# EI-CoreBioinformatics/portcullis

Measured on AMD Instinct MI355X. Metric: junc_reads_per_sec, higher is better.
Workload: dtype int32; 1 GPU; BASELINE configs[2]: synthetic 199999998 paired-end 150-bp reads, 25 contigs of GRCh38 lengths (3088286401 bp), 249999 junctions, orientation FR; reads_total=199999998, junctions_total=249999, contigs=25, reads_rank0=199999998, pairs_rank0=66692850

## Files before the change

### portcullis_amd/csrc/pjb_api.hip

```cpp
#include "pjb_host.hip.h"
#include "pjb_kernels.hip.h"

static int slot_init(pjb_ctx *c, int k);
static void aux_streams(pjb_ctx *c) {
    if (!c->stream3) (void)hipStreamCreateWithFlags(&c->stream3, hipStreamNonBlocking);
    if (!c->stream4) (void)hipStreamCreateWithFlags(&c->stream4, hipStreamNonBlocking);
}

extern "C" {

namespace {
std::mutex g_host_mu;
std::map<void *, size_t> g_host_registered;
}
void *pjb_host_alloc(size_t bytes) {
    if (bytes >= ((size_t)8 << 20)) {
        const size_t huge = (size_t)2 << 20, len = (bytes + huge - 1) & ~(huge - 1);
        void *p = mmap(nullptr, len, PROT_READ | PROT_WRITE, MAP_PRIVATE | MAP_ANONYMOUS, -1, 0);
        if (p != MAP_FAILED) {
            (void)madvise(p, len, MADV_HUGEPAGE);
            const size_t nt = std::min<size_t>(4, len >> 24);
            auto touch = [&](size_t t) {
                const size_t per = ((len / std::max<size_t>(nt, 1)) + huge - 1) & ~(huge - 1), a = std::min(len, per * t), b = std::min(len, a + per);
                for (size_t o = a; o < b; o += 4096) ((volatile uint8_t *)p)[o] = 0;
// ... 489 lines not shown
    c->mirror_acc[0] += (int64_t)R.spliced;
    c->mirror_acc[1] += (int64_t)R.unspliced;
    c->mirror_acc[2] += (int64_t)R.sum_len;
    c->mirror_acc[3] = std::min<int64_t>(c->mirror_acc[3], R.min_len);
    c->mirror_acc[4] = std::max<int64_t>(c->mirror_acc[4], R.max_len);
    int64_t *h = c->mirror_hdr;
    h[0] = (int64_t)c->mirror_rows;
    for (int k = 0; k < 5; k++) h[1 + k] = c->mirror_acc[k];
    h[6] = h[7] = 0;
}
static void mirror_reset(pjb_ctx *c) {
    c->mirror_rows = 0;
    c->mirror_acc[0] = c->mirror_acc[1] = c->mirror_acc[2] = 0;
    c->mirror_acc[3] = INT32_MAX;
    c->mirror_acc[4] = 0;
}
static int mirror_header_only(pjb_ctx *c, const pjb_region_result &R) {
    if (!c->mirror) return PJB_OK;
    aux_streams(c);
    mirror_fold(c, R, 0);
    HIP_TRY(c, hipMemcpyAsync(c->mirror, c->mirror_hdr, PJB_MIRROR_HEADER_BYTES, hipMemcpyHostToDevice, c->stream4));
    HIP_TRY(c, hipStreamSynchronize(c->stream4));
    return PJB_OK;
}

static void wait_flight(pjb_ctx *c, Flight &f);


static int rows_pinned_reserve(pjb_ctx *c, size_t need) {
    if (need <= c->rows_pinned_cap && c->rows_pinned) return PJB_OK;
    int rc = rows_sync(c);
    if (rc) return rc;
    const size_t ncap = std::max<size_t>(need * 3 / 2, 1024);
    pjb_junction_row *np = nullptr;
    const hipError_t e = hipHostMalloc((void **)&np, ncap * sizeof(pjb_junction_row), hipHostMallocPortable);
    if (e != hipSuccess) return fail(c, PJB_ERR_NOMEM, "hipHostMalloc(rows): %s", hipGetErrorString(e));
    if (c->rows_pinned && c->rows_n) memcpy(np, c->rows_pinned, std::min(c->rows_n, c->rows_pinned_cap) * sizeof(pjb_junction_row));
    if (c->rows_pinned) (void)hipHostFree(c->rows_pinned);
    c->rows_pinned = np;
    c->rows_pinned_cap = ncap;
    return PJB_OK;
}

static size_t rows_upper_bound(const pjb_ctx *c) {
    size_t n = c->rows_n;
    for (int k = 0; k < c->n_fl; k++)
        if (c->fl[k].queued) n += c->fl[k].lim.junc_limit;
    return n;
}

constexpr unsigned K6_BLOCKS = 128;
static int queue_contig(pjb_ctx *c, Flight &f) {
    std::vector<DevBatch> &batches = f.batches;
    CtlSlot &S = c->sl[f.slot];
    const hipStream_t service = c->stream, st = c->side_stream ? S.main : c->stream;
    struct ChainScope {
        pjb_ctx *c;
        hipStream_t service;
        ~ChainScope() {
            c->stream = service;
            c->scan_tiles = &c->b_scan_tiles;
        }
    } chain_scope{c, service};
    c->stream = st;
    c->scan_tiles = &S.scan_tiles;
    const u32 n_tiles = f.n_tiles;
    const ContigLimits &lim = f.lim;
    const int n_members = (int)f.tids.size();
    const bool group = n_members > 1;
    const int32_t ref_len = group ? (int32_t)f.vlen : c->ref_len[(size_t)f.tid];
    GroupTab GT;
    memset(&GT, 0, sizeof GT);
    GT.n = n_members;
    bool all_codes = true, any_x = false;
    for (int m = 0; m < n_members; m++) {
        const Contig &g = c->contigs[(size_t)f.tids[(size_t)m]];
        GT.voff[m] = f.voff[(size_t)m];
        GT.len[m] = (int32_t)g.len;
        GT.tid[m] = f.tids[(size_t)m];
        GT.d[m] = g.d;
        GT.codes[m] = g.codes;
        GT.codes2[m] = g.codes2;
        if (g.any_exc) GT.exc_members |= 1u << m;
        all_codes = all_codes && g.codes != nullptr;
        any_x = any_x || g.has_x;
    }
    const KeyFmt kf = lim.kf;
    const u32 PL = lim.pair_limit, JL = lim.junc_limit;
    const u32 SL = lim.sort_limit && lim.sort_limit < JL ? lim.sort_limit : JL;
    int rc;
    bool ahead = false;
    for (int k = 0; k < c->n_fl; k++) ahead |= c->fl[k].queued && &c->fl[k] != &f;
    const int64_t row_base = ahead ? -1 : (int64_t)c->rows_n, mirror_base = ahead ? -1 : (int64_t)c->mirror_rows;
    struct PoolScope {
        pjb_ctx *c;
        ~PoolScope() { c->cur_pool = MISC_POOL; }
    } pool_scope{c};
    c->cur_pool = f.slot;
    c->cur_slot = f.slot;
    ev_drop(c, f.slot);
    if ((rc = ensure(c, S.batches, batches.size() * sizeof(DevBatch)))) return rc;
    if (batches.size() + 2 > S.batches_pinned_cap) {
        if (S.batches_pinned) (void)hipHostFree(S.batches_pinned);
        S.batches_pinned = nullptr;
        S.batches_pinned_cap = 0;
        const size_t cap = std::max<size_t>(batches.size() * 2 + 2, 16);
        HIP_TRY(c, hipHostMalloc((void **)&S.batches_pinned, cap * sizeof(DevBatch), hipHostMallocDefault));
        S.batches_pinned_cap = cap;
    }
    memcpy(S.batches_pinned, batches.data(), batches.size() * sizeof(DevBatch));
    if ((rc = ensure(c, S.cstats, sizeof(ContigStats)))) return rc;
    if (!S.scan_parts.p) {
        if ((rc = ensure(c, S.scan_parts, sizeof(ScanPart) * K1S_BLOCKS))) return rc;
        HIP_TRY(c, hipMemset(S.scan_parts.p, 0, sizeof(ScanPart) * K1S_BLOCKS));
        HIP_TRY(c, hipStreamSynchronize(nullptr));
    }
    if ((rc = ensure(c, S.err, 8))) return rc;
    if (!c->b_cursor.p) {
        if ((rc = ensure(c, c->b_cursor, sizeof(RowCursor)))) return rc;
        HIP_TRY(c, hipMemset(c->b_cursor.p, 0, sizeof(RowCursor)));
        HIP_TRY(c, hipStreamSynchronize(nullptr));
    }
    if ((rc = ensure(c, S.tile_cnt, (size_t)n_tiles * 4))) return rc;
    if ((rc = ensure(c, S.tile_stats, (size_t)n_tiles * sizeof(TileStats)))) return rc;
    if ((rc = ensure(c, S.tile_soff, ((size_t)n_tiles + 1) * 4))) return rc;
    if ((rc = ensure(c, S.chunk_tile, ((size_t)n_tiles * (K1_TILE / 256) + 4) * 4))) return rc;
    if ((rc = ensure(c, S.splidx, (size_t)n_tiles * K1_TILE * 4))) return rc;
    if ((rc = ensure(c, S.splpoff, (size_t)n_tiles * K1_TILE * 4))) return rc;
    if ((rc = ensure(c, S.splrec, (size_t)n_tiles * K1_TILE * 16))) return rc;
    if (!S.members.p) {
        if ((rc = ensure(c, S.members, GROUP_MAX * sizeof(MemberStats) + GROUP_MAX * 4 + (GROUP_MAX + 1) * 4))) return rc;
        HIP_TRY(c, hipMemset(S.members.p, 0, S.members.cap));
        HIP_TRY(c, hipStreamSynchronize(nullptr));
    }
    MemberStats *d_members = (MemberStats *)S.members.p;
    u32 *d_member_junc = (u32 *)(d_members + GROUP_MAX);
    u32 *d_tile_lo = d_member_junc + GROUP_MAX;
    if ((rc = ensure(c, S.total, 8))) return rc;
    if ((rc = ensure(c, S.okey, ((size_t)PL + RS_TILE) * 8))) return rc;
    if ((rc = ensure(c, S.key[0], ((size_t)PL + RS_TILE) * 8))) return rc;
    if ((rc = ensure(c, S.key[1], ((size_t)PL + RS_TILE) * 8))) return rc;
    if ((rc = ensure(c, S.idx[0], ((size_t)PL + RS_TILE) * 4))) return rc;
    if ((rc = ensure(c, S.idx[1], ((size_t)PL + RS_TILE) * 4))) return rc;
    if ((rc = ensure(c, S.rec, ((size_t)PL + 1) * sizeof(PairRec)))) return rc;
    if ((rc = ensure(c, S.jid, (size_t)PL * 4 + 16))) return rc;
    if ((rc = ensure(c, S.jidbam, ((size_t)PL + RS_TILE) * 4))) return rc;
    if (c->extra && (rc = ensure(c, S.g, (size_t)PL * 4 + 16))) return rc;
    if ((rc = ensure(c, S.seg, ((size_t)PL + 1) * 4))) return rc;
    if ((rc = ensure(c, S.runfirst, ((size_t)PL + 1) * 4))) return rc;
    if ((rc = ensure(c, S.runstart, ((size_t)PL + 1) * 4))) return rc;
    if ((rc = ensure(c, S.ent, (size_t)PL * 8 + 16))) return rc;
    const u32 pair_blocks = std::max<u32>(1, (PL + 255) / 256);
    const u32 gen_cap = lim.list_cap ? lim.list_cap : (c->list_cap_forced ? c->list_cap_forced : gen_list_cap(PL));
    const u32 pack_nn = (u64)f.n_reads < (1ull << 28) ? 1u : 0u;
    if ((rc = ensure(c, S.genlist, (size_t)gen_cap * GEN_SHARDS * 8 * 3))) return rc;
    if ((rc = ensure(c, S.gencount, GEN_SHARDS * GEN_CNT_STRIDE * 4))) return rc;
    const u32 slots_lim = JL + (PL + 63) / 64 + 1;
    if ((rc = ensure(c, S.frag, (size_t)slots_lim * F_WORDS * 4))) return rc;
    if ((rc = ensure(c, S.fragj, (size_t)slots_lim * 4))) return rc;
    if ((rc = ensure(c, S.acc, (size_t)JL * F_WORDS * 4 + 16))) return rc;
    if ((rc = ensure(c, S.ancl, (size_t)JL * 4 + 16))) return rc;
    if ((rc = ensure(c, S.ancr, (size_t)JL * 4 + 16))) return rc;
    if ((rc = ensure(c, S.jkey, (size_t)JL * 8 + 16))) return rc;
    if ((rc = ensure(c, S.rows, (size_t)JL * sizeof(pjb_junction_row) + 16))) return rc;
    size_t old = rows_upper_bound(c);
    if (old + JL > c->rows_cap) {
        for (int k = 0; k < c->n_fl; k++)
            if (c->fl[k].queued && &c->fl[k] != &f) wait_flight(c, c->fl[k]);
        if ((rc = rows_sync(c))) return rc;
        old = std::min(old, c->rows_cap);
        const size_t ncap = std::max<size_t>((old + JL) * 3 / 2, 1024);
        pjb_junction_row *nd = nullptr;
        hipError_t e = hipMalloc((void **)&nd, ncap * sizeof(pjb_junction_row));
        if (e != hipSuccess) return fail(c, PJB_ERR_NOMEM, "hipMalloc(row table): %s", hipGetErrorString(e));
        if (old) {
            HIP_TRY(c, hipMemcpyAsync(nd, c->rows_table, old * sizeof(pjb_junction_row), hipMemcpyDeviceToDevice, c->stream4));
            HIP_TRY(c, hipStreamSynchronize(c->stream4));
        }
        if (c->rows_table) bury(c, c->rows_table);
        c->rows_table = nd;
        c->rows_cap = ncap;
    }
    if (!S.pub) {
        HIP_TRY(c, hipHostMalloc((void **)&S.pub, PUB_BYTES, hipHostMallocMapped | hipHostMallocPortable));
        void *dp = nullptr;
        if (hipHostGetDevicePointer(&dp, S.pub, 0) != hipSuccess || !dp) return fail(c, PJB_ERR_HIP, "hipHostGetDevicePointer(control block) failed");
        S.pub_dev = (uint8_t *)dp;
    }

    const hipStream_t front = st;
    {
        bool on_service = false;
        for (int32_t t : f.tids) {
            auto oit = c->open.find(t);
            on_service = on_service || (oit != c->open.end() && oit->second.on_main_stream);
        }
        if (st != service && on_service) {
            HIP_TRY(c, hipEventRecord(c->ev_front, service));
            HIP_TRY(c, hipStreamWaitEvent(st, c->ev_front, 0));
        }
    }
    HIP_TRY(c, hipMemcpyAsync(S.batches.p, S.batches_pinned, batches.size() * sizeof(DevBatch), hipMemcpyHostToDevice, front));
    if (group) {
        u32 *h_lo = (u32 *)(S.batches_pinned + batches.size());
        for (int m = 0; m <= n_members; m++) h_lo[m] = f.tile_lo[(size_t)m];
        HIP_TRY(c, hipMemcpyAsync(d_tile_lo, h_lo, (size_t)(n_members + 1) * 4, hipMemcpyHostToDevice, front));
    }
    if (!S.at_rest) {
        HIP_TRY(c, hipMemsetAsync(S.err.p, 0xff, 8, front));
        HIP_TRY(c, hipMemsetAsync(S.gencount.p, 0, GEN_SHARDS * GEN_CNT_STRIDE * 4, front));
        HIP_TRY(c, hipMemsetAsync(d_member_junc, 0, GROUP_MAX * 4, front));
    }
    S.at_rest = false;
    u64 *d_err = (u64 *)S.err.p;
    ContigStats *d_cs = (ContigStats *)S.cstats.p;
    const u32 *d_P = &d_cs->P, *d_J = &d_cs->J, *d_slots = &d_cs->n_slots;
    const bool stage_events = c->ktime && c->ktime_only.empty();
#define STAGE_EVENT(k)                                            \
    do {                                                          \
        if (stage_events) HIP_TRY(c, hipEventRecord(S.ev[k], st));  \
    } while (0)
    HIP_TRY(c, hipEventRecord(S.ev[0], front));
    const size_t n_words = ((size_t)std::max(ref_len, 1) + 63) / 64;
    if (lim.dense) {
        const void *was[2] = {S.bitmap.p, S.ends.p};
        if ((rc = ensure(c, S.bitmap, n_words * 8 + 16))) return rc;
        if ((rc = ensure(c, S.wrank, n_words * 4 + 16))) return rc;
        const void *was_pc = S.pagecnt.p;
        if ((rc = ensure(c, S.pagecnt, ((n_words >> KD_PAGE_SHIFT) + 1) * 4 + 16))) return rc;
        if ((rc = ensure(c, S.pagerank, ((n_words >> KD_PAGE_SHIFT) + 1) * 4 + 16))) return rc;
        if ((rc = ensure(c, S.ends, (size_t)JL * DENSE_ENDS * 4 + 32))) return rc;
        if ((rc = ensure(c, S.firstid, (size_t)JL * 4 + 16))) return rc;
        if (!S.dense_at_rest || was[0] != S.bitmap.p || was[1] != S.ends.p || was_pc != S.pagecnt.p) {
            HIP_TRY(c, hipMemsetAsync(S.bitmap.p, 0, S.bitmap.cap, front));
            HIP_TRY(c, hipMemsetAsync(S.pagecnt.p, 0, S.pagecnt.cap, front));
            HIP_TRY(c, hipMemsetAsync(S.ends.p, 0xff, S.ends.cap, front));
        }
        S.dense_at_rest = false;
    }
    Pairs pr;
    pr.key = (u64 *)S.okey.p;
    pr.rec = (PairRec *)S.rec.p;
    pr.g = c->extra ? (u32 *)S.g.p : (u32 *)nullptr;
    f.pr = pr;
    u32 *d_gen_cnt = (u32 *)S.gencount.p;
    const bool fast_codes = all_codes && !any_x;
    {
        const bool xk1 = c->extra && !c->extra_dense_only && !group && !f.x_k1 && !f.x_pre;
        XOut xo = {nullptr, nullptr, nullptr, nullptr, 0, nullptr};
        if (xk1) {
            const size_t N = (size_t)f.n_reads;
            if ((rc = ensure(c, S.x_q, N + 16)) || (rc = ensure(c, S.x_spos, N * 4 + 16)) || (rc = ensure(c, S.x_send, N * 4 + 16)) ||
                (rc = ensure(c, S.x_zlist, (size_t)X_ZCAP * 4)) || (rc = ensure(c, S.x_scnt, X_SCNT_BYTES)))
                return rc;
            HIP_TRY(c, hipMemsetAsync((uint8_t *)S.x_q.p + N, 0, 1, c->stream));
            HIP_TRY(c, hipMemsetAsync(S.x_scnt.p, 0, sizeof(SparseCounters) + sizeof(ExtraCounters), c->stream));
            xo = XOut{(int32_t *)S.x_spos.p, (int32_t *)S.x_send.p, (uint8_t *)S.x_q.p, (u32 *)S.x_zlist.p, X_ZCAP, (SparseCounters *)S.x_scnt.p};
        }
        if (c->k1_serial && c->last_k1_ev) HIP_TRY(c, hipStreamWaitEvent(st, c->last_k1_ev, 0));
        if (xk1)
            LAUNCH(c, "k1_count", k1_count<true>, dim3(n_tiles), dim3(K1C_T), (const DevBatch *)S.batches.p, (int)batches.size(), (u32 *)S.tile_cnt.p, (TileStats *)S.tile_stats.p,
                   (u32 *)S.splidx.p, (u32 *)S.splpoff.p, (uint4 *)S.splrec.p, d_err, GT, 0, xo);
        else
            LAUNCH(c, "k1_count", k1_count<false>, dim3(n_tiles), dim3(K1C_T), (const DevBatch *)S.batches.p, (int)batches.size(), (u32 *)S.tile_cnt.p, (TileStats *)S.tile_stats.p,
                   (u32 *)S.splidx.p, (u32 *)S.splpoff.p, (uint4 *)S.splrec.p, d_err, GT, group ? 1 : 0, xo);
        if (xk1) {
            HIP_TRY(c, hipEventRecord(S.ev_xk1, c->stream));
            f.x_k1 = true;
        }
        LAUNCH(c, "k1_scan_tiles", k1_scan_tiles, dim3(c->k1s_blocks_forced ? (u32)c->k1s_blocks_forced : k1s_blocks(n_tiles)), dim3(K1S_THREADS), (u32 *)S.tile_cnt.p, (const TileStats *)S.tile_stats.p,
               n_tiles, d_cs, PL, kf, group ? INT32_MAX - 1 : ref_len, (const u64 *)nullptr, (u32 *)S.tile_soff.p, (u32 *)S.chunk_tile.p,
               (ScanPart *)S.scan_parts.p, ++S.scan_epoch);
        EmitLists el;
        el.cand = lim.dense ? (u64 *)S.key[1].p : (u64 *)nullptr;
        el.bitmap = lim.dense ? (u64 *)S.bitmap.p : (u64 *)nullptr;
        el.page_cnt = lim.dense ? (u32 *)S.pagecnt.p : (u32 *)nullptr;
        el.cand_anc = (u64 *)S.ent.p;
        el.gen_list = (u64 *)S.genlist.p;
        el.gen_cnt = d_gen_cnt;
        el.gen_cap = gen_cap;
        el.pack_nn = pack_nn;
        for (size_t b0 = 0; b0 < batches.size(); b0 += K1E_MAXB) {
            const size_t nb = std::min<size_t>(K1E_MAXB, batches.size() - b0);
            u64 reads = 0;
            for (size_t bi = b0; bi < b0 + nb; bi++) reads += (u64)batches[bi].n;
            const u32 nt = (u32)std::min<u64>((reads + K1_TILE - 1) / K1_TILE + nb, 0x7fffffffu);
            static const u32 tiles_per_block = getenv("PJB_K1E_TILES") ? (u32)std::max(1, atoi(getenv("PJB_K1E_TILES"))) : 8u;
            const u32 grid = std::max<u32>(1, std::min<u32>(nt, std::max<u32>(1024, nt / tiles_per_block)));
            LAUNCH(c, "k1_emit", k1_emit, dim3(grid), dim3(256), (const DevBatch *)S.batches.p + b0, (int)nb, n_tiles, (const u32 *)S.tile_cnt.p,
                   (const u32 *)S.tile_soff.p, (const u32 *)S.chunk_tile.p, (const u32 *)S.splidx.p, (const u32 *)S.splpoff.p, (const uint4 *)S.splrec.p, pr, el, kf,
                   GT, fast_codes ? 1 : 0, (int)c->cfg.orientation, d_err, d_cs);
        }
        if (c->k1_serial && !getenv("PJB_K1_SERIAL_LATE")) {
            HIP_TRY(c, hipEventRecord(S.ev_k1, st));
            c->last_k1_ev = S.ev_k1;
        }
        if (group)
            LAUNCH(c, "kg_member_stats", kg_member_stats, dim3((unsigned)n_members), dim3(256), (const u32 *)S.tile_cnt.p, (const TileStats *)S.tile_stats.p,
                   (const u32 *)d_tile_lo, n_members, d_members, n_tiles, (const ContigStats *)d_cs);
        LAUNCH(c, "k1_generic", k1_generic, dim3(std::min<u32>(std::max<u32>(1, (u32)(((u64)gen_cap * GEN_SHARDS + K1E_T - 1) / K1E_T)), 1536u )), dim3(K1E_T),
               (const DevBatch *)S.batches.p, (int)batches.size(), (const u32 *)S.splidx.p, (const uint4 *)S.splrec.p, pr, el, kf, GT, fast_codes ? 1 : 0,
               (int)c->cfg.orientation, d_err, d_cs);
    }
    if (c->k1_serial && getenv("PJB_K1_SERIAL_LATE")) {
        HIP_TRY(c, hipEventRecord(S.ev_k1, st));
        c->last_k1_ev = S.ev_k1;
    }
    STAGE_EVENT(1);
    const u32 gen_grid = std::min<u32>(2 * (u32)(((u64)gen_cap * GEN_SHARDS + 255) / 256), 2560u);
    auto launch_k4b = [&]() -> int {
        LAUNCH(c, "k4b_generic", k4b_generic, dim3(gen_grid), dim3(256), (const u64 *)S.genlist.p, (const u32 *)d_gen_cnt, gen_cap, (const u64 *)pr.key,
               pr.rec, (const u32 *)S.jidbam.p, kf, (const DevBatch *)S.batches.p, (int)batches.size(), (const int32_t *)S.ancl.p, (const int32_t *)S.ancr.p,
               GT, any_x ? 1 : 0, any_x ? 0 : 1, d_err, (const ContigStats *)d_cs, pack_nn);
        return PJB_OK;
    };
    auto fork_k4b = [&]() -> int {
        if (!c->side_stream) return launch_k4b();
        HIP_TRY(c, hipEventRecord(S.ev_fork, st));
        HIP_TRY(c, hipStreamWaitEvent(S.side, S.ev_fork, 0));
        c->stream = S.side;
        f.forked = true;
        const int rc2 = launch_k4b();
        c->stream = st;
        if (rc2) return rc2;
        HIP_TRY(c, hipEventRecord(S.ev_join, S.side));
        return PJB_OK;
    };

    int sort_bits = kf.total_bits;
    const u32 rs_tiles = std::max<u32>(1, (PL + RS_TILE - 1) / RS_TILE);
    int n_pass = 1;
    std::vector<int> pass_bits;
    bool first_hist_done = false;
    auto plan_passes = [&]() -> int {
        n_pass = (sort_bits + c->radix_max_bits - 1) / c->radix_max_bits;
        if (n_pass < 1) n_pass = 1;
        pass_bits.assign((size_t)n_pass, sort_bits / n_pass);
        for (int p = 0; p < sort_bits % n_pass; p++) pass_bits[(size_t)p]++;
        const int dbits = pass_bits[0];
        int rc2;
        if ((rc2 = ensure(c, S.hist, (size_t)rs_tiles * (1u << dbits) * 4))) return rc2;
        if ((rc2 = ensure(c, S.hist_scan, (size_t)rs_tiles * (1u << dbits) * 4))) return rc2;
        if ((rc2 = ensure(c, S.bintotal, (size_t)4 << dbits))) return rc2;
        if ((rc2 = ensure(c, S.hist_part, (size_t)((rs_tiles + RSP_TILES - 1) / RSP_TILES) * (1u << dbits) * 4))) return rc2;
        return PJB_OK;
    };
    if (lim.dense) {
        const u32 cand_blocks = std::min<u32>(pair_blocks, 1024u);
        const u64 *okey = (const u64 *)pr.key;
        u64 *cand = (u64 *)S.key[1].p;
        const u32 n_pages = (u32)((n_words + ((size_t)1 << KD_PAGE_SHIFT) - 1) >> KD_PAGE_SHIFT);
        if ((rc = run_scan(c, "kd_rank", ArrU32Fn{(const u32 *)S.pagecnt.p}, ExclusiveU32Sink{(u32 *)S.pagerank.p}, (u64)n_pages, (u64 *)S.total.p)))
            return rc;
        LAUNCH(c, "kd_rank_pages", kd_rank_pages, dim3((n_pages + 3) / 4), dim3(256), (const u64 *)S.bitmap.p, (const u32 *)S.pagecnt.p, (const u32 *)S.pagerank.p,
               (u32 *)S.wrank.p, n_pages, (u32)n_words);
        u32 *cand_rank = (u32 *)S.idx[1].p;
        LAUNCH(c, "kd_ends", kd_ends, dim3(cand_blocks), dim3(256), (const u64 *)cand, kf, (const u64 *)S.bitmap.p, (const u32 *)S.wrank.p, JL,
               (u32 *)S.ends.p, cand_rank, d_cs);
        if ((rc = run_scan(c, "kd_first", EndsCountFn{(const u32 *)S.ends.p}, FirstIdSink{(u32 *)S.firstid.p, (int32_t *)S.ancl.p, (int32_t *)S.ancr.p},
                           (u64)JL, (u64 *)S.total.p)))
            return rc;
        LAUNCH(c, "kd_table", kd_table, dim3(cand_blocks), dim3(256), (const u64 *)cand, (const u64 *)S.ent.p, (const u32 *)cand_rank, kf, JL,
               (const u32 *)S.ends.p, (const u32 *)S.firstid.p, (const u64 *)S.total.p, (u64 *)S.jkey.p, (int32_t *)S.ancl.p, (int32_t *)S.ancr.p, d_cs,
               (const u32 *)d_gen_cnt, gen_cap, SL);
        sort_bits = std::max(1, bits_of((uint64_t)SL));
        if ((rc = plan_passes())) return rc;
        LAUNCH(c, "kd_assign", kd_assign, dim3(rs_tiles), dim3(256), okey, d_P, kf, (const u64 *)S.bitmap.p, (const u32 *)S.wrank.p,
               (const u32 *)S.ends.p, (const u32 *)S.firstid.p, JL, (const u64 *)S.total.p, (u32 *)S.jidbam.p, (u32 *)S.acc.p, (const u64 *)S.jkey.p,
               (const int32_t *)S.ancl.p, (const int32_t *)S.ancr.p, d_err, d_cs, pass_bits[0], (u32 *)S.hist.p);
        first_hist_done = true;
        if ((rc = fork_k4b())) return rc;
        LAUNCH(c, "kd_reset", kd_reset, dim3(cand_blocks), dim3(256), (const u64 *)cand, (const u32 *)cand_rank, kf, JL, (const ContigStats *)d_cs,
               (u64 *)S.bitmap.p, (u32 *)S.ends.p, (u32 *)S.pagecnt.p);
        S.dense_at_rest = true;
    } else if ((rc = plan_passes()))
        return rc;
    int cur = 0, shift = 0;
    auto sort_pass = [&](auto key_tag, const void *kin_v, void *kout_v, const u32 *vin, u32 *vout, int bits) -> int {
        using K = decltype(key_tag);
        const K *kin = (const K *)kin_v;
        K *kout = (K *)kout_v;
        if (!(shift == 0 && first_hist_done))
            LAUNCH(c, "rs_hist", rs_hist<K>, dim3(rs_tiles), dim3(256), kin, d_P, shift, bits, (u32 *)S.hist.p, rs_tiles);
        {
            const u32 nb = 1u << bits, n_panels = (rs_tiles + RSP_TILES - 1) / RSP_TILES;
            LAUNCH(c, "rs_panel_sums", rs_panel_sums, dim3(n_panels, (nb + 255) / 256), dim3(256), (const u32 *)S.hist.p, rs_tiles, nb, (u32 *)S.hist_part.p);
            LAUNCH(c, "rs_panel_scan", rs_panel_scan, dim3(n_panels, (nb + 255) / 256), dim3(256), (const u32 *)S.hist.p, (const u32 *)S.hist_part.p, rs_tiles, nb,
                   (u32 *)S.hist_scan.p, (u32 *)S.bintotal.p);
        }
#define RS_SCATTER(B)                                                                                                                          \
    LAUNCH_LDS(c, "rs_scatter", (rs_scatter<B, K>), dim3(rs_tiles), dim3(256), rs_scatter_lds_bytes(bits, sizeof(K)), kin, vin, kout, vout, d_P, \
               shift, bits, (const u32 *)S.hist_scan.p, (const u32 *)S.bintotal.p, rs_tiles)
        switch (bits) {
        case 9: RS_SCATTER(9); break;
        case 10: RS_SCATTER(10); break;
        case 11: RS_SCATTER(11); break;
        default: RS_SCATTER(0); break;
        }
#undef RS_SCATTER
        return PJB_OK;
    };
    for (int p = 0; p < n_pass; p++) {
        const int bits = pass_bits[(size_t)p];
        if (bits <= 0) break;
        const u32 *vin = p == 0 ? nullptr : (const u32 *)S.idx[cur].p;
        u32 *vout = (u32 *)S.idx[cur ^ 1].p;
        if (lim.dense) rc = sort_pass((u32)0, p == 0 ? S.jidbam.p : S.key[cur].p, S.key[cur ^ 1].p, vin, vout, bits);
        else rc = sort_pass((u64)0, p == 0 ? S.okey.p : S.key[cur].p, S.key[cur ^ 1].p, vin, vout, bits);
        if (rc) return rc;
        cur ^= 1;
        shift += bits;
    }
    f.n_pass = n_pass;
    const u32 *sidx = (const u32 *)S.idx[cur].p;
    f.sidx = sidx;
    const u32 *jid_sorted = lim.dense ? (const u32 *)S.key[cur].p : (const u32 *)S.jid.p;
    f.jid_sorted = jid_sorted;
    STAGE_EVENT(2);
    if ((rc = ensure(c, S.entsum, (size_t)JL * 8 + 16))) return rc;
    const u32 n_slices_lim = (PL + 63) / 64 + 1;
    const hipStream_t tl = st;
    auto entropy_kernels = [&]() -> int {
        LAUNCH(c, "k5_entropy_sum", k5_entropy_sum, dim3(std::max<u32>(1, (JL + 15) / 16)), dim3(256), (const u32 *)S.seg.p, (const u32 *)S.runfirst.p,
               (const u32 *)S.runstart.p, d_J, (double *)S.entsum.p);
        return PJB_OK;
    };
    bool entropy_forked = false;
    auto fork_entropy = [&]() -> int {
        if (!c->side_stream) return entropy_kernels();
        HIP_TRY(c, hipEventRecord(S.ev_fork2, st));
        HIP_TRY(c, hipStreamWaitEvent(S.side, S.ev_fork2, 0));
        c->stream = S.side;
        entropy_forked = true;
        const int rc2 = entropy_kernels();
        c->stream = st;
        if (rc2) return rc2;
        HIP_TRY(c, hipEventRecord(S.ev_join2, S.side));
        return PJB_OK;
    };
    if (lim.dense) {
        if ((rc = ensure(c, S.masks, (size_t)n_slices_lim * 8 * 2 + (size_t)n_slices_lim * 4))) return rc;
        u64 *head_mask = (u64 *)S.masks.p, *run_mask = head_mask + n_slices_lim;
        u32 *run_base = (u32 *)(run_mask + n_slices_lim);
        STAGE_EVENT(3);
        STAGE_EVENT(4);
        if (f.forked) HIP_TRY(c, hipStreamWaitEvent(tl, S.ev_join, 0));
#ifdef PJB_DEBUG_LAUNCH
        fprintf(stderr, "[k4_pairs] tid %d PL %u JL %u slots_lim %u n_slices_lim %u frag cap %zu fragj cap %zu masks cap %zu rec cap %zu idx cap %zu key cap %zu jkey cap %zu cur %d n_pass %d\n",
                f.tid, PL, JL, slots_lim, n_slices_lim, S.frag.cap, S.fragj.cap, S.masks.cap, S.rec.cap, S.idx[cur].cap, S.key[cur].cap, S.jkey.cap, cur, n_pass);
        {
            ContigStats hcs;
            (void)hipDeviceSynchronize();
            (void)hipMemcpy(&hcs, d_cs, sizeof hcs, hipMemcpyDeviceToHost);
            u64 htot = 0;
            (void)hipMemcpy(&htot, S.total.p, 8, hipMemcpyDeviceToHost);
            fprintf(stderr, "[k4_pairs] cs: P %u n_pairs %llu J %u n_junc %u n_slots %u n_slices %u n_cand %u overflow %u R %u total %llu slot %d attempt %d\n", hcs.P,
                    (unsigned long long)hcs.n_pairs, hcs.J, hcs.n_junc, hcs.n_slots, hcs.n_slices, hcs.n_cand, hcs.overflow, hcs.R, (unsigned long long)htot, f.slot, f.attempt);
            std::vector<u32> hs(hcs.P), hj(hcs.P), hb(hcs.P);
            (void)hipMemcpy(hs.data(), sidx, (size_t)hcs.P * 4, hipMemcpyDeviceToHost);
            (void)hipMemcpy(hj.data(), jid_sorted, (size_t)hcs.P * 4, hipMemcpyDeviceToHost);
            (void)hipMemcpy(hb.data(), S.jidbam.p, (size_t)hcs.P * 4, hipMemcpyDeviceToHost);
            std::vector<char> seen(hcs.P, 0);
            size_t bad_idx = 0, dup = 0, bad_order = 0, bad_in = 0, mism = 0;
            long first_bad = -1;
            for (size_t i = 0; i < hcs.P; i++) {
                if (hb[i] >= hcs.J) bad_in++;
// ... 521 lines not shown

int pjb_collect_device(pjb_ctx *c, const pjb_junction_row **rows, int64_t *n) {
    if (!c || !rows || !n) return PJB_ERR_ARG;
    *rows = (const pjb_junction_row *)c->sl[c->last_slot].rows.p;
    *n = (int64_t)c->last_rows_n;
    return PJB_OK;
}

int pjb_set_row_mirror(pjb_ctx *c, void *device_buffer, int64_t cap_bytes) {
    if (!c) return PJB_ERR_ARG;
    if (device_buffer && cap_bytes < PJB_MIRROR_HEADER_BYTES) return fail(c, PJB_ERR_ARG, "set_row_mirror: buffer smaller than its header");
    if (c->n_fl) return fail(c, PJB_ERR_STATE, "set_row_mirror: target %d is still queued", c->fl[0].tid);
    c->mirror = (uint8_t *)device_buffer;
    c->mirror_cap = device_buffer ? (size_t)cap_bytes : 0;
    mirror_reset(c);
    if (c->mirror && !c->mirror_hdr) {
        HIP_TRY(c, hipSetDevice(c->cfg.device));
        HIP_TRY(c, hipHostMalloc((void **)&c->mirror_hdr, PJB_MIRROR_HEADER_BYTES, hipHostMallocDefault));
    }
    return PJB_OK;
}

int pjb_plan_groups(const int32_t *ref_len, const int32_t *tids, int32_t n_tids, int64_t max_bases, int32_t *group_of) {
    if (n_tids < 0 || (n_tids > 0 && (!ref_len || !tids || !group_of))) return PJB_ERR_ARG;
    if (max_bases <= 0) max_bases = (int64_t)1 << 30;
    auto span = [&](int32_t k) { return (((int64_t)std::max(ref_len[tids[k]], 1) + GROUP_GAP) + 63) & ~(int64_t)63; };
    auto plan = [&](int64_t cap) {
        int32_t g = 0, members = 0;
        int64_t tot = 0;
        for (int32_t k = 0; k < n_tids; k++) {
            const int64_t s = span(k);
            if (members && (tot + s > cap || members >= GROUP_MAX)) g++, members = 0, tot = 0;
            group_of[k] = g;
            members++;
            tot += s;
        }
        return n_tids ? g + 1 : 0;
    };
    for (int32_t k = 0; k < n_tids; k++)
        if (tids[k] < 0) return PJB_ERR_ARG;
    int32_t n = plan(max_bases);
    if (n == 1 && n_tids > 1) {
        int64_t total = 0;
        for (int32_t k = 0; k < n_tids; k++) total += span(k);
        if (total > 600000000) n = plan((int64_t)((double)total * 0.55));
    }
    return n;
}

int pjb_merge_rows(const void *gathered, int32_t n_ranks, int64_t slot_stride_bytes, pjb_junction_row *rows_out, int64_t cap_rows, int64_t *n_rows,
                   pjb_region_result *totals) {
    if (n_rows) *n_rows = 0;
    if (!gathered || n_ranks < 1 || slot_stride_bytes < PJB_MIRROR_HEADER_BYTES || !n_rows || !totals || cap_rows < 0 || (cap_rows > 0 && !rows_out))
        return PJB_ERR_ARG;
    struct Run {
        int32_t refid;
        const pjb_junction_row *first;
        int64_t n;
    };
    std::vector<Run> runs;
    pjb_region_result T;
    memset(&T, 0, sizeof T);
    T.min_len = INT32_MAX;
    int64_t total = 0;
    for (int32_t r = 0; r < n_ranks; r++) {
        const uint8_t *slot = (const uint8_t *)gathered + (size_t)r * (size_t)slot_stride_bytes;
        int64_t h[6];
        memcpy(h, slot, sizeof h);
        if (h[0] < 0 || h[0] > (slot_stride_bytes - PJB_MIRROR_HEADER_BYTES) / (int64_t)sizeof(pjb_junction_row)) return PJB_ERR_ARG;
        T.spliced += (uint64_t)h[1];
        T.unspliced += (uint64_t)h[2];
        T.sum_len += (uint64_t)h[3];
        T.min_len = std::min<int32_t>(T.min_len, (int32_t)std::min<int64_t>(h[4], INT32_MAX));
        T.max_len = std::max<int32_t>(T.max_len, (int32_t)h[5]);
        const pjb_junction_row *rows = (const pjb_junction_row *)(slot + PJB_MIRROR_HEADER_BYTES);
        for (int64_t i = 0; i < h[0];) {
            int64_t j = i + 1;
            while (j < h[0] && rows[j].refid == rows[i].refid) j++;
            runs.push_back(Run{rows[i].refid, rows + i, j - i});
            i = j;
        }
        total += h[0];
    }
    T.n_reads = (int64_t)(T.spliced + T.unspliced);
    T.n_junctions = total;
    *totals = T;
    *n_rows = total;
    if (total > cap_rows) return PJB_ERR_ARG;
    std::stable_sort(runs.begin(), runs.end(), [](const Run &a, const Run &b) { return a.refid < b.refid; });
    pjb_junction_row *out = rows_out;
    for (const Run &u : runs) {
        memcpy(out, u.first, (size_t)u.n * sizeof(pjb_junction_row));
        out += u.n;
    }
    return PJB_OK;
}

int pjb_clear_rows(pjb_ctx *c) {
    if (!c) return PJB_ERR_ARG;
    if (c->n_fl) return fail(c, PJB_ERR_STATE, "clear_rows: target %d is still queued", c->fl[0].tid);
    (void)rows_sync(c);
    c->rows_n = 0;
    (void)exhume(c);
    mirror_reset(c);
    if (c->extra) {
        (void)hipSetDevice(c->cfg.device);
        (void)hipStreamSynchronize(c->stream);
        extra_clear(c);
    }
    return PJB_OK;
}

int pjb_get_kernel_timing(const pjb_ctx *c, pjb_kernel_time *out, int32_t cap, int32_t *n) {
    if (!c || !n) return PJB_ERR_ARG;
    *n = (int32_t)c->knames.size();
    for (int32_t i = 0; out && i < cap && i < *n; i++) {
        memset(&out[i], 0, sizeof out[i]);
        strncpy(out[i].name, c->knames[(size_t)i].c_str(), sizeof(out[i].name) - 1);
        out[i].launches = c->kcount[(size_t)i];
        out[i].total_ms = c->kms[(size_t)i];
    }
    return PJB_OK;
}

int pjb_select_timed_kernels(pjb_ctx *c, const char *comma_separated_names) {
    if (!c) return PJB_ERR_ARG;
    c->ktime_only.clear();
    std::string s = comma_separated_names ? comma_separated_names : "";
    size_t a = 0;
    while (a < s.size()) {
        size_t b = s.find(',', a);
        if (b == std::string::npos) b = s.size();
        if (b > a) c->ktime_only.push_back(s.substr(a, b - a));
        a = b + 1;
    }
    return PJB_OK;
}

int pjb_reset_kernel_timing(pjb_ctx *c) {
    if (!c) return PJB_ERR_ARG;
    std::fill(c->kcount.begin(), c->kcount.end(), 0);
    std::fill(c->kms.begin(), c->kms.end(), 0.0);
    return PJB_OK;
}

int pjb_set_option(pjb_ctx *c, const char *name, int64_t value) {
    if (!c || !name) return PJB_ERR_ARG;
    if (c->n_fl) return fail(c, PJB_ERR_STATE, "set_option: target %d is still queued", c->fl[0].tid);
    const std::string n = name;
    if (n == "overlap") c->side_stream = value != 0;
    else if (n == "dense_ids") c->dense_ids = value != 0;
    else if (n == "extra_dense") c->extra_dense_only = value != 0;
    else if (n == "sort_floor") c->sort_floor = (u32)std::max<int64_t>(1, std::min<int64_t>(value, 1 << 30));
    else if (n == "list_cap") c->list_cap_forced = (u32)std::max<int64_t>(0, std::min<int64_t>(value, 1 << 30));
    else return fail(c, PJB_ERR_ARG, "set_option: unknown option '%s'", name);
    return PJB_OK;
}

int pjb_get_timing(const pjb_ctx *c, pjb_timing *out) {
    if (!c || !out) return PJB_ERR_ARG;
    if (c->cfg.abi_version >= 4) *out = c->timing;
    else memcpy(out, &c->timing, offsetof(pjb_timing, repeats));
    return PJB_OK;
}

}
```

### portcullis_amd/csrc/pjb_device.hip.h

```cpp
#pragma once

#include <hip/hip_runtime.h>
#include <stdint.h>

#include "../../include/portcullis_amd.h"

namespace pjb {

typedef unsigned long long u64;
typedef unsigned int u32;

struct DevBatch {
    const int32_t *pos;
    const uint16_t *flag;
    const uint8_t *mapq;
    const uint8_t *xs;
    const int32_t *l_qseq;
    const int32_t *mtid;
    const int32_t *mpos;
    const uint32_t *cig_off;
    const uint32_t *cigar;
    const uint32_t *seq_off;
    const uint8_t *seq4;
    const u64 *name_hash;
    int64_t n;
    uint32_t base;
    uint32_t tile_base;
    int32_t prev_pos;
    int32_t member;
    const int32_t *prev_pos_ptr;
    const uint32_t *seq2;
    const uint32_t *seq_exc;
};

__device__ inline void set_error(u64 *err, u32 ordinal, int code) {
    atomicMin(err, ((u64)ordinal << 8) | (u64)(u32)(-code));
}

struct TileStats {
    u32 spliced, unspliced;
    u64 sum_len;
    int32_t min_len, max_len;
    int32_t max_end;
    int32_t max_nlen;
    int32_t min_pos;
    int32_t _pad;
};

enum : u32 { OVF_PAIRS = 1u, OVF_KEYFMT = 2u, OVF_JUNC = 4u, OVF_DENSE = 8u, OVF_LISTS = 16u };
struct ContigStats {
    u64 spliced, unspliced, sum_len;
    int32_t min_len, max_len;
    int32_t max_end, max_nlen, min_pos;
    u32 n_tiles;
    u64 n_pairs;
    u64 err;
    u32 n_junc, n_runs;
    u32 P;
    u32 J, R;
    u32 n_slots;
    u32 overflow;
    u32 n_cand;
    u32 n_slices;
    u32 list_need;
};

struct __attribute__((aligned(16))) PairRec {
    u64 aux;
    int32_t lstart;
    int32_t rend;
    int32_t pos;
    int32_t aend;
    u32 meta;
    u32 updown;
};
static_assert(sizeof(PairRec) == 32, "PairRec is one 32-byte sector");
struct Pairs {
    u64 *key;
    PairRec *rec;
    u32 *g;
};
__device__ __forceinline__ void rec_store(PairRec *dst, const PairRec &r) {
    uint4 *q = reinterpret_cast<uint4 *>(dst);
    q[0] = make_uint4((u32)r.aux, (u32)(r.aux >> 32), (u32)r.lstart, (u32)r.rend);
    q[1] = make_uint4((u32)r.pos, (u32)r.aend, r.meta, r.updown);
}
__device__ __forceinline__ PairRec rec_load(const PairRec *src) {
    const uint4 *q = reinterpret_cast<const uint4 *>(src);
    const uint4 a = q[0], b = q[1];
    PairRec r;
    r.aux = (u64)a.x | ((u64)a.y << 32);
    r.lstart = (int32_t)a.z;
    r.rend = (int32_t)a.w;
    r.pos = (int32_t)b.x;
    r.aend = (int32_t)b.y;
    r.meta = b.z;
    r.updown = b.w;
    return r;
}

enum : u32 {
    META_CAT_MASK = 3u,
    META_MULTI = 1u << 2,
    META_XS_SHIFT = 3,
    META_UM = 1u << 5,
    META_BPP = 1u << 6,
    META_PPP = 1u << 7,
    META_REL = 1u << 8,
    META_SIMPLE = 1u << 9,
};
__device__ __forceinline__ u64 pack_res(u32 minMatch, u32 mmes, u32 mis) {
    return (u64)(minMatch & 0xfffffu) | ((u64)(mmes & 0xfffffu) << 20) | ((u64)mis << 40);
}
constexpr u32 RES_FIELD_MAX = 0xfffffu;

constexpr int GROUP_MAX = 32;
constexpr int32_t GROUP_GAP = 4096;
struct GroupTab {
    int32_t n;
    int32_t voff[GROUP_MAX];
    int32_t len[GROUP_MAX];
    int32_t tid[GROUP_MAX];
    const uint8_t *d[GROUP_MAX];
    const u32 *codes[GROUP_MAX];
    const u32 *codes2[GROUP_MAX];
    u32 exc_members;
};
struct Member {
    int32_t idx, voff, len, tid;
    const uint8_t *d;
    const u32 *codes;
};
__device__ __forceinline__ Member member_of(const GroupTab &T, int32_t vpos) {
    int m = 0;
    if (T.n > 1) {
#pragma unroll
        for (int s = GROUP_MAX / 2; s >= 1; s >>= 1)
            if (m + s < T.n && T.voff[m + s] <= vpos) m += s;
    }
    Member M;
    M.idx = m;
    M.voff = T.voff[m];
    M.len = T.len[m];
    M.tid = T.tid[m];
    M.d = T.d[m];
    M.codes = T.codes[m];
    return M;
}
struct MemberStats {
    u64 spliced, unspliced, sum_len, n_pairs;
    int32_t min_len, max_len;
    u32 n_junc, _pad;
};

struct KeyFmt {
    int raw;
    int lbits;
    int total_bits;
};
__device__ __host__ inline u64 make_key(const KeyFmt &f, int32_t istart, int32_t iend) {
    if (f.raw) return ((u64)(u32)istart << 32) | (u64)(u32)iend;
    return ((u64)(u32)istart << f.lbits) | (u64)(u32)(iend - istart + 1);
}
__device__ __host__ inline void unpack_key(const KeyFmt &f, u64 k, int32_t &istart, int32_t &iend) {
    if (f.raw) {
        istart = (int32_t)(u32)(k >> 32);
        iend = (int32_t)(u32)k;
    } else {
        istart = (int32_t)(u32)(k >> f.lbits);
        iend = istart + (int32_t)(u32)(k & ((1ull << f.lbits) - 1)) - 1;
    }
}

__device__ __forceinline__ bool op_consumes_ref(u32 op) { return (0x18Du >> op) & 1u; }
__device__ __forceinline__ bool op_consumes_query(u32 op) { return (0x193u >> op) & 1u; }
enum : u32 { OP_M = 0, OP_I = 1, OP_D = 2, OP_N = 3, OP_S = 4, OP_H = 5, OP_P = 6, OP_EQ = 7, OP_X = 8 };

__device__ __forceinline__ int lane_id() { return threadIdx.x & 63; }
__device__ __forceinline__ void lds_barrier() {
    asm volatile("s_waitcnt lgkmcnt(0)" ::: "memory");
    __builtin_amdgcn_s_barrier();
    asm volatile("" ::: "memory");
}

template <class T>
__device__ __forceinline__ T gload(const T *p) {
    T v;
    __builtin_memcpy(&v, (const __attribute__((address_space(1))) void *)p, sizeof(T));
    return v;
}
#define PJB_GLOBAL __attribute__((address_space(1)))
template <class T>
__device__ __forceinline__ const PJB_GLOBAL T *as_global(const T *p) {
    return (const PJB_GLOBAL T *)p;
}
template <class T, class U>
__device__ __forceinline__ T gload_as(const PJB_GLOBAL U *p) {
    T v;
    __builtin_memcpy(&v, (const PJB_GLOBAL void *)p, sizeof(T));
    return v;
}
struct GBatch {
    const PJB_GLOBAL int32_t *pos;
    const PJB_GLOBAL uint16_t *flag;
    const PJB_GLOBAL uint8_t *mapq;
    const PJB_GLOBAL uint8_t *xs;
    const PJB_GLOBAL int32_t *l_qseq;
    const PJB_GLOBAL int32_t *mtid;
    const PJB_GLOBAL int32_t *mpos;
    const PJB_GLOBAL uint32_t *cig_off;
    const PJB_GLOBAL uint32_t *cigar;
    const PJB_GLOBAL uint32_t *seq_off;
    const PJB_GLOBAL uint8_t *seq4;
    int64_t n;
    uint32_t base, tile_base;
    int32_t prev_pos, member;
    const PJB_GLOBAL int32_t *prev_pos_ptr;
    const PJB_GLOBAL uint32_t *seq2, *seq_exc;
// ... 324 lines not shown
```

### portcullis_amd/csrc/pjb_host.hip.h

```cpp
#pragma once
#include "pjb_device.hip.h"
#include "pjb_extra_types.hip.h"

#include <algorithm>
#include <sys/mman.h>
#include <thread>
#include <chrono>
#include <cstdarg>
#include <cstdio>
#include <cstdlib>
#include <cstring>
#include <map>
#include <memory>
#include <mutex>
#include <string>
#include <thread>
#include <vector>

using namespace pjb;


inline thread_local std::string g_create_error;
inline thread_local std::string g_thread_error;
inline thread_local const void *g_thread_error_ctx = nullptr;
// ... 71 lines not shown
    int32_t tid = -1;
    int32_t len = 0;
    u32 *cover = nullptr;
    bool has_unspliced = false;
    size_t row_base = 0, n_rows = 0;
    ExtraRow *xr = nullptr;
    u64 *pair_code = nullptr;
    u32 *pair_row = nullptr;
    u32 n_pairs = 0;
    u64 *spl_codes = nullptr;
    u32 n_spl = 0;
    bool dense = false;
    bool codes_in_table = false;
    SparseDepth sparse = {nullptr, nullptr, nullptr, nullptr, 0, 0, 0, 0};
    int32_t voff = 0;
};

struct XArena {
    struct Chunk {
        uint8_t *p;
        size_t cap;
    };
    std::vector<Chunk> chunks;
    size_t cur = 0, used = 0;
};

struct ContigLimits {
    u32 pair_limit = 0, junc_limit = 0;
    u32 list_cap = 0;
    u32 sort_limit = 0;
    KeyFmt kf;
    bool dense = false;
};

struct CtlSlot {
    Buf cstats, err, gencount, batches, rows;
    Buf x_q, x_spos, x_send, x_gapoff, x_zlist, x_scnt, x_codes;
    Buf tile_cnt, tile_stats, splidx, splpoff, splrec, tile_soff, chunk_tile;
    Buf scan_parts;
    u32 scan_epoch = 0;
    Buf members;
    Buf okey, rec, g, jidbam;
    hipEvent_t ev_k1 = nullptr;
    hipEvent_t ev_xk1 = nullptr;
    Buf total, bitmap, wrank, ends, firstid, key[2], idx[2], hist, hist_scan, hist_part, bintotal, scan_tiles;
    Buf pagecnt, pagerank;
    Buf jid, seg, runfirst, runstart, ent, entsum, frag, fragj, acc, ancl, ancr, jkey, genlist, masks;
    bool dense_at_rest = false;
    hipStream_t main = nullptr, side = nullptr;
    hipEvent_t ev_fork = nullptr, ev_join = nullptr, ev_fork2 = nullptr, ev_join2 = nullptr;
    uint8_t *pub = nullptr, *pub_dev = nullptr;
    DevBatch *batches_pinned = nullptr;
    size_t batches_pinned_cap = 0;
    bool at_rest = false;
    hipEvent_t ev[PJB_N_STAGES + 2] = {};
    hipEvent_t ev_rows = nullptr, ev_done = nullptr;
};
struct EvPool {
    std::vector<hipEvent_t> ev;
    size_t used = 0;
    std::vector<int> name;
};
constexpr int MISC_POOL = PJB_MAX_QUEUED;

struct Flight {
    int32_t tid = -1;
    std::vector<int32_t> tids;
    std::vector<int32_t> voff;
    int64_t vlen = 0;
    std::vector<u32> tile_lo;
    std::vector<int64_t> m_reads;
    std::vector<DevBatch> batches;
    std::vector<int> batch_member;
    int slot = 0;
    bool queued = false;
    bool empty = false;
    bool forked = false;
    ContigLimits lim;
    int64_t n_reads = 0;
    u32 n_tiles = 0;
    int attempt = 0, list_attempt = 0;
    int n_pass = 0;
    const u32 *sidx = nullptr;
    const u32 *jid_sorted = nullptr;
    Pairs pr;
    bool x_pre = false;
    bool x_k1 = false;
    int32_t *x_spos = nullptr, *x_send = nullptr;
    u32 *x_gapoff = nullptr;
    Gap *x_gaps = nullptr;
    u32 x_gap_cap = 0;
};

constexpr size_t PJB_UP_EVENTS = 64;
struct pjb_ctx {
    pjb_config cfg;
    hipStream_t stream = nullptr;
    hipStream_t stream3 = nullptr;
    hipStream_t stream4 = nullptr;
    hipEvent_t ev_front = nullptr;
    CtlSlot sl[PJB_MAX_QUEUED];
    bool slot_busy[PJB_MAX_QUEUED] = {};
    Flight fl[PJB_MAX_QUEUED];
    int n_fl = 0;
    int cur_slot = 0;
    EvPool pools[PJB_MAX_QUEUED + 1];
    int cur_pool = MISC_POOL;
    Buf b_cursor;
    std::map<int32_t, struct BamStage *> bam_stage;
    std::mutex bam_mu, err_mu;
    std::vector<Buf> genome_pool;
    std::vector<Buf> stage_pool;
    std::vector<Buf> out_pool, misc_pool;
    hipStream_t inf_streams[4] = {};
    unsigned inf_next = 0;
    hipStream_t stream_up = nullptr;
    hipEvent_t ev_up = nullptr;
    hipEvent_t up_events[64] = {};
    int64_t up_ticket = 0, up_done = 0;
    std::string err;
    std::vector<int32_t> ref_len;
    std::vector<Contig> contigs;
    int32_t cur_tid = -1;
    std::map<int32_t, OpenContig> open;
    std::vector<Slab> slab_pool;
    uint8_t *stage[2] = {nullptr, nullptr};
    size_t stage_cap[2] = {0, 0};
    hipEvent_t stage_ev[2] = {nullptr, nullptr};
    bool stage_busy[2] = {false, false};
    unsigned stage_next = 0;
    pjb_junction_row *rows_pinned = nullptr;
    pjb_junction_row *rows_table = nullptr;
    bool rows_copy_pending = false;
    int last_slot = 0;
    int inflate_lanes = 512 * 64;
    bool side_stream = true;
    bool dense_ids = true;
    u32 junc_seen = 0;
    int lbits_seen = 18;
    size_t rows_n = 0, rows_cap = 0;
    size_t rows_pinned_cap = 0;
    std::vector<void *> graveyard;
    std::mutex grave_mu;
    size_t last_rows_n = 0;
    uint8_t *mirror = nullptr;
    size_t mirror_cap = 0;
    int64_t *mirror_hdr = nullptr;
    size_t mirror_rows = 0;
    int64_t mirror_acc[5] = {0, 0, 0, INT32_MAX, 0};
    pjb_timing timing;
    int radix_max_bits = 11;
    double junc_per_read = 0;
    u32 sort_floor = 1u << 16;
    u32 list_cap_forced = 0;
    bool k1_serial = true;
    hipEvent_t last_k1_ev = nullptr;
    int k1s_blocks_forced = 0;
    bool ktime = false;
    std::vector<std::string> knames;
    std::vector<int64_t> kcount;
    std::vector<double> kms;
    std::vector<std::string> ktime_only;
    Buf *scan_tiles = nullptr;
    Buf b_scan_tiles;
    Buf b_inf_comp, b_inf_out, b_inf_blocks, b_inf_status, b_inf_scratch, b_inf_bitmap;
    Buf b_dfl_in, b_dfl_sym, b_dfl_slots, b_dfl_size, b_dfl_off, b_dfl_packed;
    Buf b_bam_seg, b_bam_rec, b_bam_ctl;
    bool extra = false;
    std::vector<ExtraContig> xc;
    std::map<int32_t, std::pair<u64 *, u32>> filter_keys;
    Buf f_pos, f_cigoff, f_cigar, f_codes;
    Buf g_rows, g_models, g_refs, g_out, g_bad;
    Buf x_pos, x_endx, x_q, x_prefq, x_ce, x_bound, x_de, x_dropped, x_zlist, x_cnt, x_tabk, x_tabc, x_rs, x_re, x_rr, x_tileoff;
    Buf x_xrall, x_tab;
    size_t x_tab_slots = 0, x_tab_n = 0;
    XArena xarena;
    pjb_extra_row *xrows_pinned = nullptr;
    size_t xrows_pinned_cap = 0;
    bool extra_dense_only = false;
    Buf b_hasx, b_xtotal;
    Buf b_fasta_raw;
};


inline int fail(pjb_ctx *c, int code, const char *fmt, ...) {
    char tmp[1024];
    va_list ap;
    va_start(ap, fmt);
    vsnprintf(tmp, sizeof tmp, fmt, ap);
    va_end(ap);
    if (c) {
        g_thread_error = tmp;
        g_thread_error_ctx = c;
        std::lock_guard<std::mutex> lk(c->err_mu);
        c->err = tmp;
    } else
        g_create_error = tmp;
    return code;
}

#define HIP_TRY(c, call)                                                                                   \
    do {                                                                                                   \
        hipError_t e_ = (call);                                                                            \
        if (e_ != hipSuccess)                                                                              \
            return fail((c), PJB_ERR_HIP, "%s failed: %s (%s:%d)", #call, hipGetErrorString(e_), __FILE__, \
                        __LINE__);                                                                         \
    } while (0)

inline void bury(pjb_ctx *c, void *p) {
    std::lock_guard<std::mutex> lk(c->grave_mu);
    c->graveyard.push_back(p);
}
inline bool exhume(pjb_ctx *c) {
    std::vector<void *> g;
    {
        std::lock_guard<std::mutex> lk(c->grave_mu);
        g.swap(c->graveyard);
    }
    for (void *p : g) (void)hipFree(p);
    return !g.empty();
}
#ifdef PJB_DEBUG_ALLOC
#define ensure(c, b, bytes) ensure_named((c), (b), (bytes), #b, __LINE__)
inline int ensure_named(pjb_ctx *c, Buf &b, size_t bytes, const char *what, int line);
inline int ensure_impl(pjb_ctx *c, Buf &b, size_t bytes);
inline int ensure_named(pjb_ctx *c, Buf &b, size_t bytes, const char *what, int line) {
    const void *was = b.p;
    const int rc = ensure_impl(c, b, bytes);
    if (b.p != was) fprintf(stderr, "[alloc] %s (line %d): %p .. %p (%zu bytes, asked %zu)\n", what, line, b.p, (void *)((char *)b.p + b.cap), b.cap, bytes);
    return rc;
}
inline int ensure_impl(pjb_ctx *c, Buf &b, size_t bytes) {
#else
inline int ensure(pjb_ctx *c, Buf &b, size_t bytes) {
#endif
    if (bytes <= b.cap && b.p) return PJB_OK;
    if (b.p) bury(c, b.p);
    b.p = nullptr;
    b.cap = 0;
    size_t want = std::max<size_t>(bytes + bytes / 4, 256);
    hipError_t e = hipMalloc(&b.p, want);
    if (e != hipSuccess) {
        (void)hipGetLastError();
        if (exhume(c)) e = hipMalloc(&b.p, want);
    }
    if (e != hipSuccess) {
        want = std::max<size_t>(bytes, 256);
        e = hipMalloc(&b.p, want);
        if (e != hipSuccess) return fail(c, PJB_ERR_NOMEM, "hipMalloc(%zu) failed: %s", want, hipGetErrorString(e));
    }
    b.cap = want;
    static const bool poison = getenv("PJB_POISON") != nullptr && strcmp(getenv("PJB_POISON"), "0") != 0;
    if (poison) {
        (void)hipMemset(b.p, 0xCD, want);
        (void)hipDeviceSynchronize();
    }
    return PJB_OK;
}

inline void release(Buf &b) {
    if (b.p) (void)hipFree(b.p);
    b.p = nullptr;
    b.cap = 0;
}

inline const char *err_text(int code) {
    switch (code) {
    case PJB_ERR_BAD_XS: return "Unknown strand: XS tag is not one of + - ? .";
    case PJB_ERR_NO_PRESENCE: return "Found an alignment that does not have a presence in the requested region";
    case PJB_ERR_ZERO_LEN_OP: return "Can't extract cigar op sequence from query string when length has been calculated as 0";
    case PJB_ERR_QUERY_RANGE: return "Can't extract cigar op sequence from query string";
    case PJB_ERR_GENOME_RANGE: return "Can't extract cigar op sequence from extracted genome region";
    case PJB_ERR_QREGION: return "Query region is outside the genomic region";
    case PJB_ERR_ANCHOR_MISMATCH: return "Anchor region for query and genome are not the same size";
    case PJB_ERR_SPLICE_SITE_LEN: return "Retrieved sequence for splice site of junction is not the expected length";
    case PJB_ERR_ANCHOR_LEN: return "Retrieved sequence for anchor of junction is not the expected length";
    case PJB_ERR_INTRON_FLANK_LEN: return "Retrieved sequence for intron region of junction is not the expected length";
    case PJB_ERR_MIN_ANCHOR: return "The intron must lie inside its anchors (Intron::minAnchorLength)";
    case PJB_ERR_HAMMING_LEN: return "Can't find hamming distance of strings that are not the same length";
    case PJB_ERR_CLIP_RANGE: return "Soft clip longer than the read (basic_string::substr)";
    case PJB_ERR_UNSORTED: return "Alignments are not coordinate sorted";
    case PJB_ERR_DIVERGENT: return "Malformed CIGAR: padded query and genome walks disagree";
    case PJB_ERR_NO_SEQ: return "A spliced alignment was submitted without its sequence";
    default: return "unknown error";
    }
}

inline int check_device_error(pjb_ctx *c, u64 e) {
    if (e == ~0ull) return PJB_OK;
    const int code = -(int)(e & 0xff);
    const unsigned long long ord = e >> 8;
    return fail(c, code, "%s (alignment ordinal %llu on target %d)", err_text(code), ord, c->cur_tid);
}

inline void parallel_copy(void *dst, const void *src, size_t bytes) {
    const size_t MIN_SLICE = (size_t)4 << 20;
    const unsigned hw = std::max(1u, std::thread::hardware_concurrency());
    const size_t nthr = std::min<size_t>(std::min<size_t>(8, hw), bytes / MIN_SLICE);
    if (nthr <= 1) {
        memcpy(dst, src, bytes);
        return;
    }
    std::vector<std::thread> th;
    const size_t per = ((bytes + nthr - 1) / nthr + 63) & ~(size_t)63;
    for (size_t t = 0; t < nthr; t++) {
        const size_t a = std::min(bytes, per * t), b = std::min(bytes, a + per);
// ... 201 lines not shown
```

### portcullis_amd/csrc/pjb_kernels.hip.h

```cpp
#pragma once

#include "pjb_device.hip.h"

namespace pjb {

__global__ __launch_bounds__(256) void k0_upper(uint8_t *g, int64_t n, int do_upper, int *has_x) {
    int64_t i = ((int64_t)blockIdx.x * 256 + threadIdx.x) * 16;
    bool x = false;
    for (int64_t j = i; j < n && j < i + 16; j++) {
        uint8_t c = g[j];
        x |= (c == 'X' || (do_upper && c == 'x'));
    }
    if (__ballot(x) && lane_id() == 0) atomicOr(has_x, 1);
    if (!do_upper) return;
    if (i + 16 <= n && ((uintptr_t)(g + i) & 15) == 0) {
        uint4 v = *reinterpret_cast<uint4 *>(g + i);
        u32 *w = reinterpret_cast<u32 *>(&v);
#pragma unroll
        for (int k = 0; k < 4; k++) {
            u32 x = w[k], r = 0;
#pragma unroll
            for (int b = 0; b < 4; b++) {
                u32 c = (x >> (8 * b)) & 0xff;
                if (c >= 'a' && c <= 'z') c -= 32;
                r |= c << (8 * b);
            }
            w[k] = r;
        }
        *reinterpret_cast<uint4 *>(g + i) = v;
    } else {
        for (int64_t j = i; j < n && j < i + 16; j++) {
            uint8_t c = g[j];
            if (c >= 'a' && c <= 'z') g[j] = c - 32;
        }
    }
}

__global__ __launch_bounds__(256) void k0_fasta(const uint8_t *raw, int64_t raw_bytes, int64_t n, int32_t line_blen, int32_t line_len,
                                                 uint8_t *out, int *bad) {
    const int64_t i0 = ((int64_t)blockIdx.x * 256 + threadIdx.x) * 16;
    if (i0 >= n) return;
    int64_t line = i0 / line_blen;
    int32_t col = (int32_t)(i0 - line * line_blen);
    int64_t src = line * line_len + col;
    bool wrong = false;
    const int64_t i1 = i0 + 16 < n ? i0 + 16 : n;
    for (int64_t i = i0; i < i1; i++) {
        uint8_t ch = 0;
        if (src < raw_bytes) ch = raw[src];
        else wrong = true;
        wrong |= ch <= 32 || ch >= 127;
        out[i] = ch;
        src++;
        if (++col == line_blen) {
            if (i + 1 < n)
                for (int32_t k = 0; k < line_len - line_blen; k++) {
                    const uint8_t t = src + k < raw_bytes ? raw[src + k] : (uint8_t)'?';
                    wrong |= t > 32 && t < 127;
                }
            src += line_len - line_blen;
            col = 0;
        }
    }
    if (__ballot(wrong) && lane_id() == 0) atomicOr(bad, 1);
}

__device__ __forceinline__ u32 nt16_code(u32 c, bool &exotic) {
    switch (c) {
    case '=': return 0;
    case 'A': return 1;
    case 'C': return 2;
    case 'M': return 3;
    case 'G': return 4;
    case 'R': return 5;
    case 'S': return 6;
    case 'V': return 7;
    case 'T': return 8;
    case 'W': return 9;
    case 'Y': return 10;
    case 'H': return 11;
    case 'K': return 12;
    case 'D': return 13;
    case 'B': return 14;
    case 'N': return 15;
    default: exotic = true; return 0;
    }
}
__global__ __launch_bounds__(256) void k0_encode(const uint8_t *g, int64_t n, u32 *codes, int64_t n_words, int *exotic_flag) {
    const int64_t w = (int64_t)blockIdx.x * 256 + threadIdx.x;
    bool exotic = false;
    if (w < n_words) {
        u32 out = 0;
        const int64_t b0 = w * 8;
#pragma unroll
        for (int k = 0; k < 8; k++) {
            const int64_t i = b0 + k;
            if (i < n) out |= nt16_code(g[i], exotic) << (4 * k);
        }
        codes[w] = out;
    }
    if (__ballot(exotic) && lane_id() == 0) atomicOr(exotic_flag, 1);
}

constexpr int K0_CODES2_PAD = 8, K0_GEXC_PAD = 4;
__host__ __device__ inline int64_t codes2_words(int64_t n) { return ((n + 63) / 64) * 4; }
__host__ __device__ inline int64_t gexc_words(int64_t n) { return (((n + 63) / 64 + 63) / 64) * 2; }
__host__ __device__ inline int64_t codes2_alloc_words(int64_t n) { return codes2_words(n) + K0_CODES2_PAD + gexc_words(n) + K0_GEXC_PAD; }
__global__ __launch_bounds__(256) void k0_encode2(const uint8_t *g, int64_t n, u32 *codes2, u32 *gexc, int *any_exc) {
    const int64_t s = (int64_t)blockIdx.x * 256 + threadIdx.x;
    const int64_t n_str = (n + 63) / 64;
    bool exc = false;
    if (s < n_str) {
        u32 w[4] = {0, 0, 0, 0};
        const int64_t b0 = s * 64;
        if (b0 + 64 <= n && ((uintptr_t)(g + b0) & 15) == 0) {
#pragma unroll
            for (int q = 0; q < 4; q++) {
                const uint4 v = *reinterpret_cast<const uint4 *>(g + b0 + 16 * q);
                const u32 x[4] = {v.x, v.y, v.z, v.w};
#pragma unroll
                for (int k = 0; k < 16; k++) {
                    const u32 c = (x[k >> 2] >> (8 * (k & 3))) & 0xffu;
                    const u32 code = c == 'C' ? 1u : c == 'G' ? 2u : c == 'T' ? 3u : 0u;
                    exc |= !(c == 'A' || c == 'C' || c == 'G' || c == 'T');
                    w[q] |= code << (2 * k);
                }
            }
        } else {
            for (int k = 0; k < 64; k++) {
                const int64_t i = b0 + k;
                if (i < n) {
                    const u32 c = g[i];
                    const u32 code = c == 'C' ? 1u : c == 'G' ? 2u : c == 'T' ? 3u : 0u;
                    exc |= !(c == 'A' || c == 'C' || c == 'G' || c == 'T');
                    w[k >> 4] |= code << (2 * (k & 15));
                }
            }
        }
        *reinterpret_cast<uint4 *>(codes2 + 4 * s) = make_uint4(w[0], w[1], w[2], w[3]);
    }
    const u64 m = __ballot(exc);
    if (lane_id() == 0 && s < ((n_str + 63) / 64) * 64) reinterpret_cast<u64 *>(gexc)[s >> 6] = m;
    if (m && lane_id() == 0) atomicOr(any_exc, 1);
}


__device__ __forceinline__ u32 spl_nlq(u32 n, bool seq_ok, int32_t lq) {
    return (n < 0x7fffu ? n : 0x7fffu) | (seq_ok ? 0x8000u : 0u) | ((u32)lq < 0xffffu ? (u32)lq << 16 : 0xffff0000u);
}
#ifndef K1C_T
#define K1C_T 256
#endif
#ifndef K1C_WAVES
#define K1C_WAVES 7
#endif
__device__ __forceinline__ int batch_of_tile(const DevBatch *batches, int n_batches, u32 tile) {
    int found = 0;
    for (int base = 0; base < n_batches; base += 64) {
        const int k = base + lane_id();
        const u32 tb = k < n_batches ? gload(&batches[k].tile_base) : 0xffffffffu;
        const u64 m = __ballot(tb <= tile);
        if (m == 0) break;
        found = base + 63 - __clzll((long long)m);
    }
    return __builtin_amdgcn_readfirstlane(found);
}
template <int CTRL, int ROW_MASK, int BANK_MASK>
__device__ __forceinline__ u32 dpp_shift0(u32 v) {
    return (u32)__builtin_amdgcn_update_dpp(0, (int)v, CTRL, ROW_MASK, BANK_MASK, false);
}
__device__ __forceinline__ u32 wave_iscan_dpp(u32 v) {
    u32 o = v + dpp_shift0<0x111, 0xf, 0xf>(v) + dpp_shift0<0x112, 0xf, 0xf>(v) + dpp_shift0<0x113, 0xf, 0xf>(v);
    o += dpp_shift0<0x114, 0xf, 0xe>(o);
    o += dpp_shift0<0x118, 0xf, 0xc>(o);
    o += dpp_shift0<0x142, 0xa, 0xf>(o);
    o += dpp_shift0<0x143, 0xc, 0xf>(o);
    return o;
}
#define PJB_LDS __attribute__((address_space(3)))
#ifndef K1C_OPSW
#define K1C_OPSW 3072
#endif
template <bool EXTRA>
__device__ __forceinline__ void k1_count_rows(const GBatch &b, const u32 tile_local, const u32 cA, const u32 n_ops, u32 *tile_cnt, TileStats *tile_stats, u32 *spl_idx,
                                              u32 *spl_poff, uint4 *spl_rec, u64 *err, const int32_t chk_ref_len, const XOut &X) {
    constexpr int NW = K1C_T / 64;
    static_assert(K1C_T * 4 == K1_TILE, "four reads a thread");
    __shared__ __attribute__((aligned(16))) u32 s_ops[K1C_OPSW + 8];
    __shared__ u32 s_scan[2][NW];
    __shared__ u64 r64[NW][2];
    __shared__ int32_t r32[NW][6];
    const int t = threadIdx.x, w = t >> 6;
    const int64_t r0 = (int64_t)tile_local * K1_TILE + 4 * t;
    const uintptr_t a0 = (uintptr_t)(b.cigar + cA);
    const u32 shift = (u32)(a0 >> 2) & 3u;
    {
        const PJB_GLOBAL uint4 *p = (const PJB_GLOBAL uint4 *)(a0 - 4u * shift);
        const u32 total = n_ops + shift;
        const u32 exist = b.cig_off[b.n] - cA + shift;
#pragma unroll
        for (int it = 0; it < (K1C_OPSW + 3 + K1C_T * 4 - 1) / (K1C_T * 4); it++) {
            if ((u32)it * (K1C_T * 4) < total) {
                const u32 i = (u32)it * (K1C_T * 4) + (u32)t * 4u;
                if (i + 4u <= exist) {
                    if (i < total) __builtin_amdgcn_global_load_lds(p + (i >> 2), (PJB_LDS void *)(s_ops + it * (K1C_T * 4) + w * 256), 16, 0, 0);
                } else if (i < exist) {
                    const PJB_GLOBAL u32 *q = (const PJB_GLOBAL u32 *)p + i;
                    s_ops[i] = q[0];
                    if (i + 1u < exist) s_ops[i + 1] = q[1];
                    if (i + 2u < exist) s_ops[i + 2] = q[2];
                }
            }
        }
    }
    const Words4 co = gload_as<Words4>(b.cig_off + r0);
    const u32 co4 = b.cig_off[r0 + 4];
    const Words4 po = gload_as<Words4>(b.pos + r0);
    const int32_t pprev = r0 > 0 ? b.pos[r0 - 1] : (b.prev_pos_ptr ? *b.prev_pos_ptr : b.prev_pos);
    const Words4 lqv = gload_as<Words4>(b.l_qseq + r0);
    const Words4 sov = gload_as<Words4>(b.seq_off + r0);
    const u32 so4 = b.seq_off[r0 + 4];
    const u32 xs4 = gload_as<u32>(b.xs + r0);
    u64 fl4 = 0;
    if (EXTRA) fl4 = gload_as<u64>(b.flag + r0);
    const u32 c[5] = {co.x, co.y, co.z, co.w, co4}, so[5] = {sov.x, sov.y, sov.z, sov.w, so4};
    const int32_t pos[4] = {(int32_t)po.x, (int32_t)po.y, (int32_t)po.z, (int32_t)po.w}, lq[4] = {(int32_t)lqv.x, (int32_t)lqv.y, (int32_t)lqv.z, (int32_t)lqv.w};
    asm volatile("s_waitcnt vmcnt(0)" ::: "memory");
    __syncthreads();
    u32 cnt = 0, spl = 0, uns = 0;
    u64 sum = 0;
    int32_t mn = INT32_MAX, mx = 0, max_end = 0, max_nlen = 0, min_pos = INT32_MAX;
    u32 cN[4], nlq[4];
    u32 xspan = 0, xgapmax = 0;
    bool xmany = false;
#pragma unroll
    for (int i = 0; i < 4; i++) {
        const int64_t r = r0 + i;
        const int32_t p = pos[i], lenv = lq[i];
        const int32_t prv = i == 0 ? pprev : pos[i > 0 ? i - 1 : 0];
        if (p < prv) set_error(err, b.base + (u32)r, PJB_ERR_UNSORTED);
        if (((xs4 >> (8 * i)) & 0xffu) > 2u) set_error(err, b.base + (u32)r, PJB_ERR_BAD_XS);
        mn = lenv < mn ? lenv : mn;
        mx = lenv > mx ? lenv : mx;
        sum += (u64)(int64_t)lenv;
        const u32 n = c[i + 1] - c[i];
        nlq[i] = spl_nlq(n, (u64)(so[i + 1] - so[i]) * 8ull >= (u64)(int64_t)lenv, lenv);
        const u32 *ops = s_ops + (c[i] - cA + shift);
        u32 cc = 0, ngap = 0, gmax = 0;
        int32_t al = 0;
        auto count_op = [&](u32 op) {
            const u32 ty = op & 15u;
            const int32_t ln = (int32_t)(op >> 4);
            if (op_consumes_ref(ty)) al += ln;
            if (ty == OP_N) {
                cc++;
                max_nlen = ln > max_nlen ? ln : max_nlen;
            }
            if (EXTRA && ty == OP_D && ln) {
                ngap++;
                gmax = max(gmax, (u32)ln);
            }
        };
        const u32 o0 = ops[0], o1 = ops[1], o2 = ops[2], o3 = ops[3];
        count_op(0u < n ? o0 : 0u);
        count_op(1u < n ? o1 : 0u);
        count_op(2u < n ? o2 : 0u);
        count_op(3u < n ? o3 : 0u);
        for (u32 k = 4; k < n; k++) count_op(ops[k]);
        cnt += cc;
        if (cc) {
            spl++;
            const int32_t e = p + al;
            max_end = e > max_end ? e : max_end;
            min_pos = p < min_pos ? p : min_pos;
        } else
            uns++;
        cN[i] = cc;
        if (EXTRA) {
            const u32 g = b.base + (u32)r;
            const u32 fv = (u32)(fl4 >> (16 * i)) & 0xffffu;
            const bool unspliced = cc == 0 && !(fv & 0x4u);
            const bool spans = unspliced && al > 0 && p >= 0;
            X.s_pos[g] = p;
            X.s_end[g] = spans ? p + al : p;
            if (!spans) ngap = 0, gmax = 0;
            if (ngap > SPARSE_GAP_MAX) xmany = true, ngap = SPARSE_GAP_MAX;
            X.q[g] = (uint8_t)((spans ? 1u : 0u) | (ngap << 1));
            if (spans) xspan = max(xspan, (u32)al);
            xgapmax = max(xgapmax, gmax);
            if (unspliced && al == 0) {
                const u32 z = atomicAdd(&X.cnt->n_zero, 1u);
                if (z < X.zcap) X.zlist[z] = (u32)p;
            }
        }
    }
    if (EXTRA) {
        xspan = wave_max(xspan);
        xgapmax = wave_max(xgapmax);
        if (lane_id() == 0) {
            if (xspan > X.cnt->max_span) atomicMax(&X.cnt->max_span, xspan);
            if (xgapmax > X.cnt->max_gap) atomicMax(&X.cnt->max_gap, xgapmax);
        }
        if (xmany) atomicOr(&X.cnt->need_dense, 2u);
    }
    {
        const u32 inc_s = wave_iscan_dpp(spl), inc_p = wave_iscan_dpp(cnt);
        if (lane_id() == 63) {
            s_scan[0][w] = inc_s;
            s_scan[1][w] = inc_p;
        }
        __syncthreads();
        u32 ex_s = inc_s - spl, ex_p = inc_p - cnt;
#pragma unroll
        for (int k = 0; k < NW; k++)
            if (k < w) {
                ex_s += s_scan[0][k];
                ex_p += s_scan[1][k];
            }
#pragma unroll
        for (int i = 0; i < 4; i++)
            if (cN[i]) {
                const size_t slot = (size_t)blockIdx.x * K1_TILE + ex_s;
                spl_idx[slot] = (u32)(r0 + i);
                spl_poff[slot] = ex_p;
                spl_rec[slot] = make_uint4(c[i], (u32)pos[i], so[i], nlq[i]);
                ex_s++;
                ex_p += cN[i];
            }
    }
    const u32 w_cnt = wave_total<DppAdd>(cnt), w_su = wave_total<DppAdd>((spl << 16) | uns);
    sum = (u64)wave_total<DppAdd>((u32)(sum & 0xffffu)) + ((u64)wave_total<DppAdd>((u32)((sum >> 16) & 0xffffu)) << 16) +
          ((u64)wave_total<DppAdd>((u32)(sum >> 32)) << 32);
    auto smin = [](int32_t v) { return (int32_t)(wave_total<DppMin>((u32)v ^ 0x80000000u) ^ 0x80000000u); };
    auto smax = [](int32_t v) { return (int32_t)(wave_total<DppMax>((u32)v ^ 0x80000000u) ^ 0x80000000u); };
    mn = smin(mn);
    mx = smax(mx);
    max_end = smax(max_end);
    max_nlen = smax(max_nlen);
    min_pos = smin(min_pos);
    if (lane_id() == 0) {
        r64[w][0] = ((u64)w_cnt << 32) | w_su;
        r64[w][1] = sum;
        r32[w][0] = mn;
        r32[w][1] = mx;
        r32[w][2] = max_end;
        r32[w][3] = max_nlen;
        r32[w][4] = min_pos;
    }
    __syncthreads();
    if (threadIdx.x == 0) {
        u64 pk = 0;
        TileStats ts;
        ts.sum_len = 0;
        ts.min_len = INT32_MAX, ts.max_len = 0, ts.max_end = 0, ts.max_nlen = 0, ts.min_pos = INT32_MAX;
        for (int i = 0; i < NW; i++) {
            pk += r64[i][0];
            ts.sum_len += r64[i][1];
            ts.min_len = min(ts.min_len, r32[i][0]);
            ts.max_len = max(ts.max_len, r32[i][1]);
            ts.max_end = max(ts.max_end, r32[i][2]);
            ts.max_nlen = max(ts.max_nlen, r32[i][3]);
            ts.min_pos = min(ts.min_pos, r32[i][4]);
        }
        ts.spliced = (u32)((pk >> 16) & 0xffff);
        ts.unspliced = (u32)(pk & 0xffff);
        if (chk_ref_len > 0 && ts.max_end > chk_ref_len) ts.max_end = INT32_MAX;
        ts._pad = 0;
        tile_stats[blockIdx.x] = ts;
        tile_cnt[blockIdx.x] = (u32)(pk >> 32);
    }
}
template <bool EXTRA>
__global__ __launch_bounds__(K1C_T) __attribute__((amdgpu_waves_per_eu(K1C_WAVES, K1C_WAVES))) void k1_count(const DevBatch *batches, int n_batches, u32 *tile_cnt, TileStats *tile_stats, u32 *spl_idx,
                                                 u32 *spl_poff, uint4 *spl_rec, u64 *err, GroupTab G, int chk_members, XOut X) {
    constexpr int NW = K1C_T / 64, RPT = K1_TILE / K1C_T;
    __shared__ u64 sm64[NW];
    __shared__ u64 sm_scan4[RPT][NW];
    __shared__ int32_t smi[NW][6];
    const GBatch b = load_batch(batches + batch_of_tile(batches, n_batches, blockIdx.x));
    const u32 tile_local = blockIdx.x - b.tile_base;
    const int32_t chk_ref_len = chk_members ? max(G.len[b.member], 1) : 0;
    int64_t base = (int64_t)tile_local * K1_TILE;
    if (base + K1_TILE <= b.n) {
        const u32 cA = b.cig_off[base], cB = b.cig_off[base + K1_TILE];
        if (cB - cA + 3u <= (u32)K1C_OPSW) {
            k1_count_rows<EXTRA>(b, tile_local, cA, cB - cA, tile_cnt, tile_stats, spl_idx, spl_poff, spl_rec, err, chk_ref_len, X);
            return;
        }
    }
    u32 cnt = 0, spl = 0, uns = 0;
    u64 sum = 0;
    int32_t mn = INT32_MAX, mx = 0, max_end = 0, max_nlen = 0, min_pos = INT32_MAX;
    constexpr int K1_OPS = 4;
    u32 c0[RPT], nop[RPT], ops[RPT][K1_OPS];
    int32_t pos4[RPT];
    u32 c4[RPT], so4[RPT], nlq4[RPT];
    u32 bad = 0;
    u32 xflag4[RPT] = {}, xspan = 0, xgapmax = 0;
    bool xmany = false;
#pragma unroll
    for (int it = 0; it < RPT; it++) {
        const int64_t r = base + it * K1C_T + threadIdx.x;
        const bool on = r < b.n;
        const int64_t rr = on ? r : b.n - 1, rp = rr > 0 ? rr - 1 : 0;
        const u32 c0v = b.cig_off[rr], c1v = b.cig_off[rr + 1];
        const int32_t posv = b.pos[rr], prevv = b.pos[rp], lenv = b.l_qseq[rr];
        const u32 xsv = (u32)b.xs[rr], sov = b.seq_off[rr], so1v = b.seq_off[rr + 1];
        so4[it] = sov;
        c0[it] = on ? c0v : 0u;
        nop[it] = on ? c1v - c0v : 0u;
        pos4[it] = on ? posv : 0;
        const int32_t prv = r > 0 ? prevv : (b.prev_pos_ptr ? *b.prev_pos_ptr : b.prev_pos);
        if (on && posv < prv) bad |= 1u << it;
        if (on && xsv > 2) bad |= 16u << it;
        if (on) {
            mn = lenv < mn ? lenv : mn;
            mx = lenv > mx ? lenv : mx;
            sum += (u64)(int64_t)lenv;
        }
        nlq4[it] = spl_nlq(c1v - c0v, (u64)(so1v - sov) * 8ull >= (u64)(int64_t)lenv, lenv);
        if (EXTRA) {
            const u32 fv = (u32)b.flag[rr];
            xflag4[it] = on ? fv : 0u;
        }
    }
#pragma unroll
    for (int it = 0; it < RPT; it++)
#pragma unroll
        for (int k = 0; k < K1_OPS; k++) {
            const bool has = (u32)k < nop[it];
            const u32 v = *(has ? b.cigar + c0[it] + k : b.cig_off);
            ops[it][k] = has ? v : 0u;
        }
#pragma unroll
    for (int it = 0; it < RPT; it++) {
        const int64_t r = base + it * K1C_T + threadIdx.x;
        u32 cthis = 0;
        if (r < b.n) {
            const int32_t p = pos4[it];
            if (bad & (1u << it)) set_error(err, b.base + (u32)r, PJB_ERR_UNSORTED);
            if (bad & (16u << it)) set_error(err, b.base + (u32)r, PJB_ERR_BAD_XS);
            u32 c = 0, ngap = 0, gmax = 0;
            int32_t al = 0;
            auto count_op = [&](u32 op) {
                const u32 ty = op & 15u;
                const int32_t ln = (int32_t)(op >> 4);
                if (op_consumes_ref(ty)) al += ln;
                if (ty == OP_N) {
                    c++;
                    max_nlen = ln > max_nlen ? ln : max_nlen;
                }
                if (EXTRA && ty == OP_D && ln) {
                    ngap++;
                    gmax = max(gmax, (u32)ln);
                }
            };
#pragma unroll
            for (int k = 0; k < K1_OPS; k++) count_op(ops[it][k]);
            for (u32 k = K1_OPS; k < nop[it]; k++) count_op(b.cigar[c0[it] + k]);
            cnt += c;
            if (c) {
                spl++;
                int32_t e = p + al;
                max_end = e > max_end ? e : max_end;
                min_pos = p < min_pos ? p : min_pos;
            } else
                uns++;
            cthis = c;
            if (EXTRA) {
                const u32 g = b.base + (u32)r;
                const bool unspliced = c == 0 && !(xflag4[it] & 0x4u);
                const bool spans = unspliced && al > 0 && p >= 0;
                X.s_pos[g] = p;
                X.s_end[g] = spans ? p + al : p;
                if (!spans) ngap = 0, gmax = 0;
                if (ngap > SPARSE_GAP_MAX) xmany = true, ngap = SPARSE_GAP_MAX;
                X.q[g] = (uint8_t)((spans ? 1u : 0u) | (ngap << 1));
                if (spans) xspan = max(xspan, (u32)al);
                xgapmax = max(xgapmax, gmax);
                if (unspliced && al == 0) {
                    const u32 z = atomicAdd(&X.cnt->n_zero, 1u);
                    if (z < X.zcap) X.zlist[z] = (u32)p;
                }
            }
        }
        c4[it] = cthis;
    }
    if (EXTRA) {
        xspan = wave_max(xspan);
        xgapmax = wave_max(xgapmax);
        if (lane_id() == 0) {
            if (xspan > X.cnt->max_span) atomicMax(&X.cnt->max_span, xspan);
            if (xgapmax > X.cnt->max_gap) atomicMax(&X.cnt->max_gap, xgapmax);
        }
        if (xmany) atomicOr(&X.cnt->need_dense, 2u);
    }
    {
        u64 inc[RPT];
        const int w = threadIdx.x >> 6;
#pragma unroll
        for (int it = 0; it < RPT; it++) {
            inc[it] = wave_iscan<u64>(((u64)c4[it] << 16) | (u64)(c4[it] ? 1u : 0u));
            if (lane_id() == 63) sm_scan4[it][w] = inc[it];
        }
        __syncthreads();
        u64 run = 0;
#pragma unroll
        for (int it = 0; it < RPT; it++) {
            u64 before = run;
#pragma unroll
            for (int i = 0; i < NW; i++) {
                const u64 t = sm_scan4[it][i];
                if (i < w) before += t;
                run += t;
            }
            if (c4[it]) {
                const u64 ex = before + inc[it] - (((u64)c4[it] << 16) | 1u);
                const size_t slot = (size_t)blockIdx.x * K1_TILE + (u32)(ex & 0xffffu);
                spl_idx[slot] = (u32)(base + it * K1C_T + threadIdx.x);
                spl_poff[slot] = (u32)(ex >> 16);
                spl_rec[slot] = make_uint4(c0[it], (u32)pos4[it], so4[it], nlq4[it]);
            }
        }
    }
    u64 packed = ((u64)wave_total<DppAdd>(cnt) << 32) | (u64)wave_total<DppAdd>((spl << 16) | uns);
    sum = (u64)wave_total<DppAdd>((u32)(sum & 0xffffu)) + ((u64)wave_total<DppAdd>((u32)((sum >> 16) & 0xffffu)) << 16) +
          ((u64)wave_total<DppAdd>((u32)(sum >> 32)) << 32);
    auto smin = [](int32_t v) { return (int32_t)(wave_total<DppMin>((u32)v ^ 0x80000000u) ^ 0x80000000u); };
    auto smax = [](int32_t v) { return (int32_t)(wave_total<DppMax>((u32)v ^ 0x80000000u) ^ 0x80000000u); };
    mn = smin(mn);
    mx = smax(mx);
    max_end = smax(max_end);
    max_nlen = smax(max_nlen);
    min_pos = smin(min_pos);
    int w = threadIdx.x >> 6;
    __shared__ u64 smp[NW];
    if (lane_id() == 0) {
        smp[w] = packed;
        sm64[w] = sum;
        smi[w][0] = mn;
        smi[w][1] = mx;
        smi[w][2] = max_end;
        smi[w][3] = max_nlen;
        smi[w][4] = min_pos;
    }
    __syncthreads();
    if (threadIdx.x == 0) {
        u64 p = 0;
        TileStats t;
        t.sum_len = 0;
        t.min_len = INT32_MAX, t.max_len = 0, t.max_end = 0, t.max_nlen = 0, t.min_pos = INT32_MAX;
        for (int i = 0; i < NW; i++) {
            p += smp[i];
            t.sum_len += sm64[i];
            t.min_len = min(t.min_len, smi[i][0]);
            t.max_len = max(t.max_len, smi[i][1]);
            t.max_end = max(t.max_end, smi[i][2]);
            t.max_nlen = max(t.max_nlen, smi[i][3]);
            t.min_pos = min(t.min_pos, smi[i][4]);
        }
        t.spliced = (u32)((p >> 16) & 0xffff);
        t.unspliced = (u32)(p & 0xffff);
        if (chk_ref_len > 0 && t.max_end > chk_ref_len) t.max_end = INT32_MAX;
        t._pad = 0;
        tile_stats[blockIdx.x] = t;
        tile_cnt[blockIdx.x] = (u32)(p >> 32);
    }
}

constexpr int K1S_THREADS = 256, K1S_PER = 16, K1S_BLOCKS = 64;
struct ScanPart {
    u64 pairs, spl, uns, sum;
    int32_t mn, mx, max_end, max_nlen, min_pos;
    u32 flag;
    u32 _pad[2];
};
static_assert(sizeof(ScanPart) == 64, "ScanPart layout");
__host__ __device__ inline u32 k1s_blocks(u32 n_tiles) {
    const u32 g = (n_tiles + 1023u) / 1024u;
    return g < 1u ? 1u : (g > (u32)K1S_BLOCKS ? (u32)K1S_BLOCKS : g);
}
__global__ __launch_bounds__(K1S_THREADS) void k1_scan_tiles(u32 *tile_cnt, const TileStats *ts, u32 n_tiles, ContigStats *out, u32 pair_limit,
                                                              KeyFmt kf, int32_t ref_len, const u64 *tile_desc, u32 *tile_soff, u32 *chunk_tile,
                                                              ScanPart *parts, u32 epoch) {
    constexpr int NW = K1S_THREADS / 64;
    __shared__ u64 wsum[NW];
    __shared__ u32 wsum2[NW];
    __shared__ u32 carry2_s;
    __shared__ u64 carry_s;
    __shared__ u64 r_pairs[NW], r_spl[NW], r_uns[NW], r_sum[NW];
    __shared__ int32_t r_i[NW][5];
    __shared__ ScanPart total_s;
    const u32 nblk = gridDim.x, blk = blockIdx.x;
    const u32 per_blk = ((n_tiles + nblk - 1) / nblk + (u32)K1S_PER - 1) / (u32)K1S_PER * (u32)K1S_PER;
    const u32 lo = min(n_tiles, blk * per_blk), hi = min(n_tiles, lo + per_blk);
    const int w = threadIdx.x >> 6;
    u64 pairs = 0, spl = 0, uns = 0, sum = 0;
    int32_t mn = INT32_MAX, mx = 0, max_end = 0, max_nlen = 0, min_pos = INT32_MAX;
    for (u32 base = lo; base < hi; base += K1S_THREADS * K1S_PER) {
        const u32 i0 = base + K1S_PER * threadIdx.x;
#pragma unroll 4
        for (int q = 0; q < K1S_PER; q++) {
            const u32 i = i0 + q, ic = i < hi ? i : hi - 1;
            const u64 cnt = tile_desc ? (tile_desc[ic] & ((1ull << 40) - 1)) : (u64)tile_cnt[ic];
            const TileStats t = ts[ic];
            if (i < hi) {
                pairs += cnt;
                spl += t.spliced;
                uns += t.unspliced;
                sum += t.sum_len;
                mn = min(mn, t.min_len);
                mx = max(mx, t.max_len);
                max_end = max(max_end, t.max_end);
                max_nlen = max(max_nlen, t.max_nlen);
                min_pos = min(min_pos, t.min_pos);
            }
        }
    }
    pairs = wave_sum(pairs);
    spl = wave_sum(spl);
    uns = wave_sum(uns);
    sum = wave_sum(sum);
    mn = wave_min(mn);
    mx = wave_max(mx);
    max_end = wave_max(max_end);
    max_nlen = wave_max(max_nlen);
    min_pos = wave_min(min_pos);
    if (lane_id() == 0) {
        r_pairs[w] = pairs;
        r_spl[w] = spl;
        r_uns[w] = uns;
        r_sum[w] = sum;
        r_i[w][0] = mn;
        r_i[w][1] = mx;
        r_i[w][2] = max_end;
        r_i[w][3] = max_nlen;
        r_i[w][4] = min_pos;
    }
    __syncthreads();
    ScanPart mine;
    mine.pairs = mine.spl = mine.uns = mine.sum = 0;
    mine.mn = INT32_MAX, mine.mx = 0, mine.max_end = 0, mine.max_nlen = 0, mine.min_pos = INT32_MAX;
    for (int k = 0; k < NW; k++) {
        mine.pairs += r_pairs[k];
        mine.spl += r_spl[k];
        mine.uns += r_uns[k];
        mine.sum += r_sum[k];
        mine.mn = min(mine.mn, r_i[k][0]);
        mine.mx = max(mine.mx, r_i[k][1]);
        mine.max_end = max(mine.max_end, r_i[k][2]);
        mine.max_nlen = max(mine.max_nlen, r_i[k][3]);
        mine.min_pos = min(mine.min_pos, r_i[k][4]);
    }
    if (threadIdx.x == 0 && blk + 1 < nblk) {
        ScanPart *o = parts + blk;
        o->pairs = mine.pairs;
        o->spl = mine.spl;
        o->uns = mine.uns;
        o->sum = mine.sum;
        o->mn = mine.mn;
        o->mx = mine.mx;
        o->max_end = mine.max_end;
        o->max_nlen = mine.max_nlen;
        o->min_pos = mine.min_pos;
        __hip_atomic_store(&o->flag, epoch, __ATOMIC_RELEASE, __HIP_MEMORY_SCOPE_AGENT);
    }
    if (w == 0) {
        const u32 l = lane_id();
        ScanPart b;
        b.pairs = b.spl = b.uns = b.sum = 0;
        b.mn = INT32_MAX, b.mx = 0, b.max_end = 0, b.max_nlen = 0, b.min_pos = INT32_MAX;
        if (l < blk) {
            const ScanPart *o = parts + l;
            while (__hip_atomic_load(&o->flag, __ATOMIC_ACQUIRE, __HIP_MEMORY_SCOPE_AGENT) != epoch) __builtin_amdgcn_s_sleep(1);
            b.pairs = __hip_atomic_load(&o->pairs, __ATOMIC_RELAXED, __HIP_MEMORY_SCOPE_AGENT);
            b.spl = __hip_atomic_load(&o->spl, __ATOMIC_RELAXED, __HIP_MEMORY_SCOPE_AGENT);
            if (blk + 1 == nblk) {
                b.uns = __hip_atomic_load(&o->uns, __ATOMIC_RELAXED, __HIP_MEMORY_SCOPE_AGENT);
                b.sum = __hip_atomic_load(&o->sum, __ATOMIC_RELAXED, __HIP_MEMORY_SCOPE_AGENT);
                b.mn = __hip_atomic_load(&o->mn, __ATOMIC_RELAXED, __HIP_MEMORY_SCOPE_AGENT);
                b.mx = __hip_atomic_load(&o->mx, __ATOMIC_RELAXED, __HIP_MEMORY_SCOPE_AGENT);
                b.max_end = __hip_atomic_load(&o->max_end, __ATOMIC_RELAXED, __HIP_MEMORY_SCOPE_AGENT);
                b.max_nlen = __hip_atomic_load(&o->max_nlen, __ATOMIC_RELAXED, __HIP_MEMORY_SCOPE_AGENT);
                b.min_pos = __hip_atomic_load(&o->min_pos, __ATOMIC_RELAXED, __HIP_MEMORY_SCOPE_AGENT);
            }
        }
        b.pairs = wave_sum(b.pairs);
        b.spl = wave_sum(b.spl);
        if (blk + 1 == nblk) {
            b.uns = wave_sum(b.uns);
            b.sum = wave_sum(b.sum);
            b.mn = wave_min(b.mn);
            b.mx = wave_max(b.mx);
            b.max_end = wave_max(b.max_end);
            b.max_nlen = wave_max(b.max_nlen);
            b.min_pos = wave_min(b.min_pos);
        }
        if (l == 0) {
            carry_s = b.pairs;
            carry2_s = (u32)b.spl;
            total_s = b;
        }
    }
    __syncthreads();
    for (u32 base = lo; base < hi; base += K1S_THREADS * K1S_PER) {
        const u32 i0 = base + K1S_PER * threadIdx.x;
        u64 v[K1S_PER];
        u32 v2[K1S_PER];
        u64 vs = 0;
        u32 vs2 = 0;
#pragma unroll
        for (int q = 0; q < K1S_PER; q++) {
            const u32 i = i0 + q, ic = i < hi ? i : hi - 1;
            const u64 cnt = tile_desc ? (tile_desc[ic] & ((1ull << 40) - 1)) : (u64)tile_cnt[ic];
            const u32 sp = ts[ic].spliced;
            v[q] = i < hi ? cnt : 0;
            v2[q] = i < hi ? sp : 0u;
            vs += v[q];
            vs2 += v2[q];
        }
        const u64 inc = wave_iscan(vs);
        const u32 inc2 = wave_iscan(vs2);
        if (lane_id() == 63) {
            wsum[w] = inc;
            wsum2[w] = inc2;
        }
        __syncthreads();
        u64 wb = 0, tot = 0;
        u32 wb2 = 0, tot2 = 0;
        for (int k = 0; k < NW; k++) {
            const u64 s = wsum[k];
            const u32 s2 = wsum2[k];
            if (k < w) {
                wb += s;
                wb2 += s2;
            }
            tot += s;
            tot2 += s2;
        }
        const u64 carry = carry_s;
        const u32 carry2 = carry2_s;
        u64 ex = carry + wb + inc - vs;
        u32 so = carry2 + wb2 + inc2 - vs2;
#pragma unroll
        for (int q = 0; q < K1S_PER; q++) {
            const u32 i = i0 + q;
            if (i < hi) {
                if (!tile_desc) tile_cnt[i] = (u32)ex;
                if (tile_soff) {
                    tile_soff[i] = so;
                    for (u32 c = (so + 255u) >> 8; (c << 8) < so + v2[q]; c++) chunk_tile[c] = i;
                }
            }
            ex += v[q];
            so += v2[q];
        }
        __syncthreads();
        if (threadIdx.x == 0) {
            carry_s = carry + tot;
            carry2_s = carry2 + tot2;
        }
        __syncthreads();
    }
    if (blk + 1 != nblk) return;
    if (threadIdx.x == 0) {
        if (tile_soff) tile_soff[n_tiles] = carry2_s;
        const ScanPart b = total_s;
        const u64 n_pairs = carry_s;
        const int32_t m0 = min(b.mn, mine.mn), m1 = max(b.mx, mine.mx), m2 = max(b.max_end, mine.max_end), m3 = max(b.max_nlen, mine.max_nlen),
                      m4 = min(b.min_pos, mine.min_pos);
        out->spliced = b.spl + mine.spl;
        out->unspliced = b.uns + mine.uns;
        out->sum_len = b.sum + mine.sum;
        out->min_len = m0;
        out->max_len = m1;
        out->max_end = m2;
        out->max_nlen = m3;
        out->min_pos = m4;
        out->n_tiles = n_tiles;
        out->n_pairs = n_pairs;
        u32 ovf = 0;
        if (n_pairs > (u64)pair_limit) ovf |= OVF_PAIRS;
        if (n_pairs > 0) {
            const bool weird = m4 < 0 || m2 > ref_len || m2 < 0;
            if (!kf.raw) {
                int need = 0;
                for (u32 v = (u32)m3; v; v >>= 1) need++;
                if (weird || need > kf.lbits) ovf |= OVF_KEYFMT;
            }
        }
        out->overflow = ovf;
        out->P = ovf ? 0u : (u32)n_pairs;
        out->J = out->R = out->n_slots = out->n_slices = 0;
        out->n_junc = out->n_runs = 0;
        out->list_need = 0;
        out->n_cand = 0;
    }
}

__device__ __forceinline__ u32 nt16_ascii(u32 c) {
    const u64 t0 = 0x565352474D43413DULL;
    const u64 t1 = 0x4E42444B48595754ULL;
    const u64 t = (c & 8u) ? t1 : t0;
    return (u32)(t >> ((c & 7u) * 8)) & 0xffu;
}

__device__ __forceinline__ u32 swap_nibbles(u32 x) { return ((x & 0x0F0F0F0Fu) << 4) | ((x >> 4) & 0x0F0F0F0Fu); }
template <int NW>
struct CmpChunkT {
    u32 qw[NW], gg[NW];
};
template <int NW>
__device__ __forceinline__ void load_words(u32 (&d)[NW], const u32 *p, int32_t first, int32_t last) {
    static_assert(NW == 9 || NW == 8 || NW == 5, "chunk width");
    if (first >= 0 && first + NW - 1 <= last) {
        const Words4 a = gload(reinterpret_cast<const Words4 *>(p + first));
        d[0] = a.x, d[1] = a.y, d[2] = a.z, d[3] = a.w;
        if constexpr (NW >= 8) {
            const Words4 b = gload(reinterpret_cast<const Words4 *>(p + first + 4));
            d[4] = b.x, d[5] = b.y, d[6] = b.z, d[7] = b.w;
        }
        if constexpr (NW != 8) d[NW - 1] = gload(p + first + NW - 1);
    } else {
#pragma unroll
        for (int k = 0; k < NW; k++) d[k] = (first + k >= 0 && first + k <= last) ? gload(p + first + k) : 0u;
    }
}
template <int NW, bool TO_BUFFER_END = false>
__device__ __forceinline__ void chunk_load(CmpChunkT<NW> &C, const u32 *seqw, int32_t qi, int32_t q_last, const u32 *gw, int32_t gi, int32_t g_words,
                                           int32_t l, int32_t t) {
    const int32_t lastg = (gi + l - 1) >> 3;
    load_words<NW>(C.qw, seqw, (qi + t) >> 3, q_last);
    load_words<NW>(C.gg, gw, (gi + t) >> 3, !TO_BUFFER_END && lastg < g_words - 1 ? lastg : g_words - 1);
}
template <int NW>
__device__ __forceinline__ void chunk_cmp(CmpChunkT<NW> &C, int32_t qi, int32_t gi, int32_t l, int32_t t, int32_t out_base, int32_t &mism,
                                          int32_t &first_mis, int32_t &last_mis) {
    const u32 shq = (u32)(qi & 7) * 4u, shg = (u32)(gi & 7) * 4u;
#pragma unroll
    for (int k = 0; k < NW; k++) C.qw[k] = swap_nibbles(C.qw[k]);
#pragma unroll
    for (int c = 0; c < NW - 1; c++) {
        const int32_t rem = l - t - 8 * c;
        if (rem > 0) {
            const u32 q = __builtin_amdgcn_alignbit(C.qw[c + 1], C.qw[c], shq);
            const u32 g = __builtin_amdgcn_alignbit(C.gg[c + 1], C.gg[c], shg);
            const u32 x = q ^ g;
            u32 m = (((x & 0x77777777u) + 0x77777777u) | x) & 0x88888888u;
            if (rem < 8) m &= (1u << (4 * rem)) - 1u;
            if (m) {
                mism += __popc(m);
                if (first_mis < 0) first_mis = out_base + t + 8 * c + ((__ffs((int)m) - 1) >> 2);
                last_mis = out_base + t + 8 * c + ((31 - __clz((int)m)) >> 2);
            }
        }
    }
}
__device__ __forceinline__ u32 ffbl_hw(u32 x) {
    u32 r;
    asm("v_ffbl_b32 %0, %1" : "=v"(r) : "v"(x));
    return r;
}
__device__ __forceinline__ u32 ffbh_hw(u32 x) {
    u32 r;
    asm("v_ffbh_u32 %0, %1" : "=v"(r) : "v"(x));
    return r;
}
template <int NW>
__device__ __forceinline__ void chunk_cmp_bits(CmpChunkT<NW> &C, int32_t qi, int32_t gi, int32_t l, int32_t t, u32 &mism, u32 &fbit, u32 &lbit1) {
    const u32 shq = (u32)(qi & 7) * 4u, shg = (u32)(gi & 7) * 4u;
#pragma unroll
    for (int k = 0; k < NW; k++) C.qw[k] = swap_nibbles(C.qw[k]);
    const int32_t rem2 = 2 * (l - t);
    u32 fw = 0xffffffffu, lw = 0;
#pragma unroll
    for (int c = 0; c < NW - 1; c++) {
        int32_t w2 = rem2 - 16 * c;
        w2 = w2 < 0 ? 0 : (w2 > 16 ? 16 : w2);
        const u32 inval = (0xffffffffu << (u32)w2) << (u32)w2;
        const u32 q = __builtin_amdgcn_alignbit(C.qw[c + 1], C.qw[c], shq);
        const u32 g = __builtin_amdgcn_alignbit(C.gg[c + 1], C.gg[c], shg);
        const u32 x = q ^ g;
        const u32 m = (((x & 0x77777777u) + 0x77777777u) | x) & (0x88888888u & ~inval);
        mism += (u32)__popc(m);
        fw = min(fw, __builtin_elementwise_add_sat(ffbl_hw(m), 32u * (u32)c));
        lw = max(lw, __builtin_elementwise_sub_sat(32u * (u32)c + 32u, ffbh_hw(m)));
    }
    fbit = min(fbit, __builtin_elementwise_add_sat(fw, 4u * (u32)t));
    lbit1 = lw ? lw + 4u * (u32)t : lbit1;
}
template <int NW, bool TO_BUFFER_END = false>
__device__ __forceinline__ void cmp_words(const u32 *seqw, int32_t qi, int32_t q_last, const u32 *gw, int32_t gi, int32_t g_words, int32_t l,
                                          int32_t out_base, int32_t &mism, int32_t &first_mis, int32_t &last_mis) {
    for (int32_t t = 0; t < l; t += 8 * (NW - 1)) {
        CmpChunkT<NW> C;
        chunk_load<NW, TO_BUFFER_END>(C, seqw, qi, q_last, gw, gi, g_words, l, t);
        chunk_cmp<NW>(C, qi, gi, l, t, out_base, mism, first_mis, last_mis);
    }
}

constexpr int OPS_LDS = 8;
template <int STRIDE, int NLDS>
struct OpsViewT {
    const uint32_t *g;
    const u32 *lds;
    __device__ __forceinline__ u32 operator[](u32 k) const { return k < (u32)NLDS ? lds[k * STRIDE] : gload(g + k); }
};
typedef OpsViewT<256, OPS_LDS> OpsView;

struct NCursor {
    u32 i;
    int32_t acc;
    bool has;
    int32_t peek;
};
template <typename Ops>
__device__ __forceinline__ void ncursor_advance(NCursor &c, const Ops cig, u32 n) {
    c.has = false;
    while (c.i < n) {
        u32 op = cig[c.i++];
        u32 ty = op & 15u;
        if (op_consumes_ref(ty)) c.acc += (int32_t)(op >> 4);
        if (ty == OP_N) {
            c.has = true;
            c.peek = c.acc;
            return;
        }
    }
}

constexpr int SIMPLE_NW = 8;
struct CmpBlock {
    int32_t len, mism, first, last;
};
__device__ __forceinline__ u64 cmp_blocks_res(const CmpBlock &L, const CmpBlock &R) {
    const u32 upM = L.last < 0 ? (u32)L.len : (u32)(L.len - 1 - L.last);
    const u32 downM = R.first < 0 ? (u32)R.len : (u32)R.first;
    const u32 tu = (u32)(L.len - L.mism), td = (u32)(R.len - R.mism);
    return pack_res(upM < downM ? upM : downM, tu < td ? tu : td, (u32)(L.mism + R.mism));
}
struct EmitRead {
    u32 n;
    int32_t pos;
    u32 g;
    u32 meta;
    u32 nN;
    int32_t aend;
    int32_t lq;
    bool seq_ok;
    u32 off;
    const u32 *closed_seqw;
    int32_t q_limit;
    const u32 *gcodes;
    int32_t glen, voff;
};
template <typename Ops, typename PairFn>
__device__ __forceinline__ void emit_read_pairs(const Ops cig, const EmitRead R, const Pairs P, const KeyFmt kf, const int32_t ref_len,
                                                u64 *err, PairFn &&on_pair) {
    const u32 n = R.n, g = R.g, nN = R.nN;
    const int32_t pos = R.pos, aend = R.aend;
    u32 meta = R.meta;
    NCursor U = {0, pos, false, 0}, D = {0, pos, false, 0};
    ncursor_advance(U, cig, n);
    ncursor_advance(D, cig, n);
    u32 cntU = 0, cntD = 0;
    int32_t lStart = pos, lEndExc = pos, sumAfter = 0, prevRStartU = 0, prevIend = 0, prevIstart = 0;
    int32_t qAcc = 0, prevQ = 0;
    int64_t prev = -1;
    u64 prev_key = 0;
    const bool closed = R.closed_seqw != nullptr;
    PairRec pend;
    pend.aux = 0;
    pend.lstart = pend.rend = 0;
    pend.pos = pos;
    pend.aend = aend;
    pend.meta = closed ? meta | META_SIMPLE : meta;
    pend.updown = 0;
    typedef CmpBlock Block;
    Block blkL = {0, 0, -1, -1}, blk = {0, 0, -1, -1};
    auto closed_stats = [&]() { return cmp_blocks_res(blkL, blk); };
    (void)prevIstart;
    (void)prevQ;
    u32 k = 0;
    for (u32 i = 0; i < n; i++) {
        const u32 op = cig[i];
        const u32 ty = op & 15u;
        const int32_t ln = (int32_t)(op >> 4);
        if (ty == OP_N) {
            if (prev >= 0) {
                int32_t rEndExc = prevRStartU + sumAfter;
                if (rEndExc - 1 >= ref_len) rEndExc = ref_len;
                pend.rend = rEndExc - 1;
                if (closed) pend.aux = closed_stats();
                rec_store(P.rec + prev, pend);
                on_pair(prev_key, pend.lstart, pend.rend);
                if (rEndExc - 1 < prevIend) set_error(err, g, PJB_ERR_MIN_ANCHOR);
            }
            const int32_t istart = lEndExc;
            const int32_t rStartU = lEndExc + ln;
            int32_t rStart = rStartU;
            if (rStart - 1 >= ref_len) rStart = ref_len - 1;
            const int32_t iend = rStart - 1;
            while (U.has && U.peek < istart) {
                cntU++;
                ncursor_advance(U, cig, n);
            }
            while (D.has && D.peek <= iend + 1) {
                cntD++;
                ncursor_advance(D, cig, n);
            }
            const int64_t idx = (int64_t)R.off + k;
            const u64 key = make_key(kf, istart, iend);
            P.key[idx] = key;
            if (P.g) P.g[idx] = g;
            pend.lstart = lStart;
            pend.updown = cntU | ((nN - cntD) << 16);
            if (lStart > istart) set_error(err, g, PJB_ERR_MIN_ANCHOR);
            prev = idx;
            prev_key = key;
            blkL = blk;
            blk = Block{0, 0, -1, -1};
            prevIstart = istart;
            prevQ = qAcc;
            prevIend = iend;
            prevRStartU = rStartU;
            sumAfter = 0;
            lStart = rStart;
            lEndExc = rStart;
            k++;
        } else {
            if (closed && ty != OP_S) {
                const bool cq = op_consumes_query(ty), cr = op_consumes_ref(ty);
                if (cq && cr)
                    cmp_words<SIMPLE_NW, true>(R.closed_seqw, qAcc, R.q_limit, R.gcodes, lEndExc - R.voff, (R.glen + 7) / 8 + 1, ln, blk.len, blk.mism, blk.first, blk.last);
                else {
                    blk.mism += ln;
                    if (blk.first < 0) blk.first = blk.len;
                    blk.last = blk.len + ln - 1;
                }
                blk.len += ln;
            }
            if (op_consumes_ref(ty)) {
                lEndExc += ln;
                sumAfter += ln;
            }
        }
        if (op_consumes_query(ty)) qAcc += ln;
    }
    if (prev >= 0) {
        int32_t rEndExc = prevRStartU + sumAfter;
        if (rEndExc - 1 >= ref_len) rEndExc = ref_len;
        pend.rend = rEndExc - 1;
        if (closed) pend.aux = closed_stats();
        rec_store(P.rec + prev, pend);
        on_pair(prev_key, pend.lstart, pend.rend);
        if (rEndExc - 1 < prevIend) set_error(err, g, PJB_ERR_MIN_ANCHOR);
    }
}

__device__ __forceinline__ u32 read_meta(u32 flag, u32 xs, u32 mapq, int32_t pos, int32_t mtid, int32_t mpos, int32_t tid, int orientation) {
    const bool pp_check = orientation == PJB_OR_FR || orientation == PJB_OR_RF || orientation == PJB_OR_FF;
// ... 86 lines not shown
                old = atomicCAS((unsigned long long *)&sh.set[h], (unsigned long long)KD_EMPTY, (unsigned long long)k);
                if (old == KD_EMPTY) {
                    atomicAdd(&sh.set_n, 1u);
                    old = k;
                }
            }
            if (old == k) {
                if (lstart < sh.lo[h]) atomicMin(&sh.lo[h], lstart);
                if (rend > sh.hi[h]) atomicMax(&sh.hi[h], rend);
                return;
            }
            h = (h + 1) & (KC_SLOTS - 1);
        }
        const u32 at = atomicAdd(&cs->n_cand, 1u);
        E.cand[at] = k;
        E.cand_anc[at] = (u64)(u32)lstart | ((u64)(u32)rend << 32);
        cand_mark(E, k);
    }
    __device__ __forceinline__ u32 list_reserve(u32 kind, bool mine, u32 pairs, u32 shard) const {
        const u64 gm2 = __ballot(mine);
        if (!gm2) return 0u;
        const u32 pairs_w = pairs * (u32)__popcll(gm2);
        const int leader = __ffsll((long long)gm2) - 1;
        const u32 w0 = shard * GEN_CNT_STRIDE + (kind - 1) * 2;
        u32 base = 0;
        if (lane_id() == leader) {
            base = atomicAdd(&E.gen_cnt[w0], (u32)__popcll(gm2));
            if (pairs_w) atomicAdd(&E.gen_cnt[w0 + 1], pairs_w);
        }
        return base;
    }
    __device__ __forceinline__ void list_write(u32 kind, bool mine, u32 base, u64 entry, u32 shard) const {
        const u64 gm2 = __ballot(mine);
        if (!gm2) return;
        base = (u32)__builtin_amdgcn_readlane((int)base, __ffsll((long long)gm2) - 1);
        const u32 at = base + (u32)__popcll(gm2 & ((1ull << lane_id()) - 1));
        if (mine && at < E.gen_cap) E.gen_list[((size_t)(kind - 1) * GEN_SHARDS + shard) * E.gen_cap + at] = entry;
    }
    __device__ __forceinline__ void list_append(u32 kind, bool mine, u32 pairs, u64 entry, u32 shard) const {
        const u64 gm2 = __ballot(mine);
        if (!gm2) return;
        const u32 pairs_w = wave_total<DppAdd>(mine ? pairs : 0u);
        const int leader = __ffsll((long long)gm2) - 1;
        const u32 w0 = shard * GEN_CNT_STRIDE + (kind - 1) * 2;
        u32 base = 0;
        if (lane_id() == leader) {
            base = atomicAdd(&E.gen_cnt[w0], (u32)__popcll(gm2));
            atomicAdd(&E.gen_cnt[w0 + 1], pairs_w);
        }
        base = (u32)__builtin_amdgcn_readlane((int)base, leader);
        const u32 at = base + (u32)__popcll(gm2 & ((1ull << lane_id()) - 1));
        if (mine && at < E.gen_cap) E.gen_list[((size_t)(kind - 1) * GEN_SHARDS + shard) * E.gen_cap + at] = entry;
    }
    __device__ __forceinline__ void cand_flush(bool force) const {
        if (!want_cand) return;
        lds_barrier();
        if (sh.set_n > (u32)KC_SLOTS / 4 || force) {
            u64 mine[KC_SLOTS / K1E_T], anc[KC_SLOTS / K1E_T];
            u32 cnt = 0;
#pragma unroll
            for (int i = 0; i < KC_SLOTS / K1E_T; i++) {
                const int at = i * K1E_T + threadIdx.x;
                mine[i] = sh.set[at];
                anc[i] = (u64)(u32)sh.lo[at] | ((u64)(u32)sh.hi[at] << 32);
                cnt += mine[i] != KD_EMPTY;
                sh.set[at] = KD_EMPTY;
                sh.lo[at] = INT32_MAX;
                sh.hi[at] = INT32_MIN;
            }
            u32 total;
            const u32 excl = block_escan<K1E_T / 64, u32, true>(cnt, sh.scan, &total);
            if (threadIdx.x == 0) {
                sh.base = total ? atomicAdd(&cs->n_cand, total) : 0u;
                sh.set_n = 0;
            }
            lds_barrier();
            u32 o = sh.base + excl;
#pragma unroll
            for (int i = 0; i < KC_SLOTS / K1E_T; i++)
                if (mine[i] != KD_EMPTY) {
                    E.cand[o] = mine[i];
                    E.cand_anc[o++] = anc[i];
                    cand_mark(E, mine[i]);
                }
        }
    }
};

struct __attribute__((packed, aligned(4))) Words2 {
    u32 x, y;
};
constexpr int C2_NW = 8;
constexpr int32_t C2_ROUND = 16 * (C2_NW - 1);
constexpr int32_t C2_MAX_BLOCK = 1900;
template <int NW>
__device__ __forceinline__ void chunk2_cmp_bits(const u32 (&qw)[NW], const u32 (&gw)[NW], u32 shq, u32 shg, int32_t l, int32_t t, u32 &mism, u32 &fbit,
                                                u32 &lbit1) {
    const int32_t rem = l - t;
    u32 fw = 0xffffffffu, lw = 0;
#pragma unroll
    for (int c = 0; c < NW - 1; c++) {
        int32_t v = rem - 16 * c;
        v = v < 0 ? 0 : (v > 16 ? 16 : v);
        const u32 inval = (0xffffffffu << (u32)v) << (u32)v;
        const u32 x = __builtin_amdgcn_alignbit(qw[c + 1], qw[c], shq) ^ __builtin_amdgcn_alignbit(gw[c + 1], gw[c], shg);
        const u32 m = (x | (x >> 1)) & (0x55555555u & ~inval);
        mism += (u32)__popc(m);
        fw = min(fw, __builtin_elementwise_add_sat(ffbl_hw(m), 32u * (u32)c));
        lw = max(lw, __builtin_elementwise_sub_sat(32u * (u32)c + 32u, ffbh_hw(m)));
    }
    fbit = min(fbit, __builtin_elementwise_add_sat(fw, 2u * (u32)t));
    lbit1 = lw ? lw + 2u * (u32)t : lbit1;
}

#ifdef K1E_PROF
__device__ unsigned long long g_k1e_prof[16];
#define K1E_T0() unsigned long long prof_t = __builtin_amdgcn_s_memtime()
#define K1E_MARK(i)                                                                  \
    do {                                                                             \
        const unsigned long long now_ = __builtin_amdgcn_s_memtime();                \
        if (lane_id() == 0) atomicAdd(&g_k1e_prof[i], now_ - prof_t);                \
        prof_t = now_;                                                               \
    } while (0)
#else
#define K1E_T0() do {} while (0)
#define K1E_MARK(i) do {} while (0)
#endif
constexpr int K1E_MAXB = 64;
struct EmitRec {
    bool on;
    u32 slot, r, toff, poff;
    uint4 sr;
};
struct EmitOps {
    u32 op[OPS_LDS];
    u32 n, flag, xs, mapq;
    u32 excw;
    int32_t mtid, mpos, lq;
};
struct EmitTrip {
    int bi;
    u32 chunk, s_begin, s_end;
};
__global__ __launch_bounds__(K1E_T) __attribute__((amdgpu_waves_per_eu(K1E_WAVES, K1E_WAVES))) void k1_emit(const DevBatch *batches, int n_batches, u32 n_tiles_total, const u32 *tile_off, const u32 *tile_soff,
                                                const u32 *chunk_tile, const u32 *spl_idx, const u32 *spl_poff, const uint4 *spl_rec, Pairs P, EmitLists E, KeyFmt kf,
                                                GroupTab G, int use_codes, int orientation, u64 *err, ContigStats *cs) {
    __shared__ u32 s_soff[K1E_LOOK];
    __shared__ EmitShared sh;
    __shared__ u32 s_cfirst[K1E_MAXB + 1];
    __shared__ u32 s_sbegin[K1E_MAXB + 1];
    __shared__ u32 s_seqw[K1E_MAXB], s_cigw[K1E_MAXB], s_tbase[K1E_MAXB];
    __shared__ u32 s_wsum[4];
    if (cs->P == 0) return;
    K1E_T0();
    const bool want_g = P.g != nullptr;
    const bool want_cand = E.cand != nullptr;
    EmitCtx ctx{sh, E, kf, cs, want_cand};
    ctx.init();
    auto cand_insert = [&](u64 k, int32_t lstart, int32_t rend) { ctx.cand_insert(k, lstart, rend); };
    {
        u32 trips = 0;
        if ((int)threadIdx.x < n_batches) {
            const PJB_GLOBAL DevBatch *d = as_global(batches + threadIdx.x);
            const u32 tb = d->tile_base, nt = (u32)((d->n + K1_TILE - 1) / K1_TILE);
            const u32 sb = tile_soff[tb], se = tile_soff[tb + nt];
            trips = sb == se ? 0u : ((se + (u32)K1E_T - 1u) >> K1E_SHIFT) - (sb >> K1E_SHIFT);
            s_sbegin[threadIdx.x] = sb;
            if ((int)threadIdx.x == n_batches - 1) s_sbegin[n_batches] = se;
            s_seqw[threadIdx.x] = as_global(d->seq_off)[d->n];
            s_cigw[threadIdx.x] = as_global(d->cig_off)[d->n];
            s_tbase[threadIdx.x] = tb;
        }
        u32 total;
        const u32 ex = block_escan<K1E_T / 64>(trips, s_wsum, &total);
        if (threadIdx.x < (u32)K1E_MAXB) s_cfirst[threadIdx.x] = ex;
        if (threadIdx.x == K1E_T - 1) s_cfirst[K1E_MAXB] = total;
        __syncthreads();
    }
    const u32 n_trips = s_cfirst[K1E_MAXB];
    const u32 per_block = (n_trips + gridDim.x - 1) / gridDim.x;
    const u32 v_lo = min(n_trips, blockIdx.x * per_block), v_hi = min(n_trips, v_lo + per_block);
    if (v_lo >= v_hi) return;
    u32 win_t0 = 0xffffffffu;
    int win_bi = -1;
    auto locate = [&](u32 v) {
        static_assert(K1E_MAXB <= 64, "one ballot");
        const int k = lane_id();
        const u64 m = __ballot(k < n_batches && s_cfirst[k] <= v);
        EmitTrip T;
        T.bi = __builtin_amdgcn_readfirstlane(63 - __clzll((long long)m));
        T.s_begin = s_sbegin[T.bi];
        T.s_end = s_sbegin[T.bi + 1];
        T.chunk = (T.s_begin >> K1E_SHIFT) + (v - s_cfirst[T.bi]);
        return T;
    };
    auto fetch_rec = [&](const EmitTrip &T) {
        const u32 s_last = min((T.chunk + 1u) << K1E_SHIFT, T.s_end) - 1u;
        const bool reload = win_bi != T.bi || win_t0 == 0xffffffffu || s_last >= s_soff[K1E_LOOK - 1];
        if (reload) {
            win_t0 = (T.chunk << K1E_SHIFT) < T.s_begin ? s_tbase[T.bi] : chunk_tile[T.chunk >> (8 - K1E_SHIFT)];
            win_bi = T.bi;
            const u32 mine = threadIdx.x < K1E_LOOK && win_t0 + threadIdx.x <= n_tiles_total ? tile_soff[win_t0 + threadIdx.x] : 0xffffffffu;
            lds_barrier();
            if (threadIdx.x < K1E_LOOK) s_soff[threadIdx.x] = mine;
            lds_barrier();
        }
        const u32 s = (T.chunk << K1E_SHIFT) + threadIdx.x;
        EmitRec R;
        R.on = s >= T.s_begin && s < T.s_end;
        R.slot = R.r = R.toff = R.poff = 0;
        R.sr = make_uint4(0, 0, 0, 0);
        const u32 w_first = (T.chunk << K1E_SHIFT) + (threadIdx.x & ~63u);
        const u32 off_m = lane_id() < K1E_LOOK ? s_soff[lane_id() & (K1E_LOOK - 1)] : 0xffffffffu;
        const u32 m_lo = (u32)__popcll(__ballot(off_m <= w_first)), m_hi = (u32)__popcll(__ballot(off_m <= w_first + 63u));
        if (R.on) {
            u32 k = m_lo ? m_lo - 1u : 0u;
            for (u32 m = m_lo ? m_lo : 1u; m < m_hi; m++) k += s >= (u32)__builtin_amdgcn_readlane((int)off_m, (int)m) ? 1u : 0u;
            u32 tile = win_t0 + k, soff = s_soff[k];
            if (k + 1 == (u32)K1E_LOOK && s >= soff) {
                u32 lo = tile, hi = n_tiles_total;
                while (hi - lo > 1) {
                    const u32 mid = (lo + hi) >> 1;
                    if (tile_soff[mid] <= s) lo = mid;
                    else hi = mid;
                }
                tile = lo;
                soff = tile_soff[lo];
            }
            R.slot = tile * (u32)K1_TILE + (s - soff);
            R.sr = spl_rec[R.slot];
            R.r = spl_idx[R.slot];
            R.toff = tile_off[tile];
            R.poff = spl_poff[R.slot];
        }
        return R;
    };
    auto fetch_ops = [&](const EmitTrip &T, const EmitRec &R) {
        EmitOps O;
#pragma unroll
        for (int q = 0; q < OPS_LDS; q++) O.op[q] = 0;
        O.n = O.flag = O.xs = O.mapq = 0;
        O.excw = 0xffffffffu;
        O.mtid = O.mpos = O.lq = 0;
        if (R.on) {
            const GBatch b = load_batch(batches + T.bi);
            const u32 c0 = R.sr.x, cig_words = s_cigw[T.bi];
            const int64_t r = R.r;
            u32 n = R.sr.w & 0x7fffu;
            if (n == 0x7fffu) n = b.cig_off[r + 1] - c0;
            O.n = n;
            O.flag = b.flag[r];
            O.xs = b.xs[r];
            O.mapq = b.mapq[r];
            O.mtid = b.mtid[r];
            O.mpos = b.mpos[r];
            if (b.seq2 != nullptr) O.excw = b.seq_exc[r >> 5];
            O.lq = (int32_t)(R.sr.w >> 16);
            if (O.lq == 0xffff) O.lq = b.l_qseq[r];
            static_assert(OPS_LDS == 8, "two 16-byte loads");
            if (cig_words >= (u32)OPS_LDS) {
                const u32 c0c = c0 + (u32)OPS_LDS <= cig_words ? c0 : cig_words - (u32)OPS_LDS;
                const Words4 lo4 = gload_as<Words4>(b.cigar + c0c), hi4 = gload_as<Words4>(b.cigar + c0c + 4);
                u32 w[OPS_LDS] = {lo4.x, lo4.y, lo4.z, lo4.w, hi4.x, hi4.y, hi4.z, hi4.w};
                if (c0c != c0) {
                    const u32 sh = c0 - c0c;
#pragma unroll
                    for (int q = 0; q < OPS_LDS; q++) {
                        u32 v = 0;
#pragma unroll
                        for (int j = q; j < OPS_LDS; j++) v = (u32)(j - q) == sh ? w[j] : v;
                        w[q] = v;
                    }
                }
#pragma unroll
                for (int q = 0; q < OPS_LDS; q++) O.op[q] = w[q];
            } else {
#pragma unroll
                for (int q = 0; q < OPS_LDS; q++) O.op[q] = c0 + (u32)q < cig_words ? b.cigar[c0 + (u32)q] : 0u;
            }
        }
        return O;
    };
    K1E_MARK(0);
    EmitTrip T = locate(v_lo);
    EmitRec R = fetch_rec(T);
    EmitOps O = fetch_ops(T, R);
    EmitTrip T1 = T;
    EmitRec R1 = R;
    if (v_lo + 1 < v_hi) {
        T1 = locate(v_lo + 1);
        R1 = fetch_rec(T1);
    }
    K1E_MARK(1);
    for (u32 v = v_lo; v < v_hi; v++) {
        const GBatch b = load_batch(batches + T.bi);
        const int mem = b.member;
        const int32_t voff = G.voff[mem], ref_len = G.len[mem], tid = G.tid[mem];
        const PJB_GLOBAL u32 *gcodes = use_codes ? as_global(G.codes[mem]) : (const PJB_GLOBAL u32 *)nullptr;
        const PJB_GLOBAL u32 *gcodes2 = use_codes && b.seq2 != nullptr ? as_global(G.codes2[mem]) : (const PJB_GLOBAL u32 *)nullptr;
        const int32_t vlen = voff + ref_len;
        const u32 seq_words = s_seqw[T.bi];
        const int32_t g_words = (ref_len + 7) / 8 + 1;
        const u32 chunk = T.chunk;
        const bool on = R.on;
        const u32 so = R.sr.z;
        const int32_t pos = (int32_t)R.sr.y, lq = O.lq;
        bool generic = false, simple = false, two = false;
        u32 dS = 0, a = 0, nl = 0, b2 = 0, nl2 = 0, b3 = 0, meta = 0, off = 0, g = 0;
        if (on) {
            const u32 n = O.n;
            const u32 (&op)[OPS_LDS] = O.op;
            g = b.base + R.r;
            off = R.toff + R.poff;
            meta = read_meta(O.flag, O.xs, O.mapq, pos, O.mtid, O.mpos, tid, orientation);
            const bool seq_ok = (R.sr.w & 0x8000u) != 0;
            if (gcodes != nullptr && n >= 3 && n <= 7) {
                const bool clipF = (op[0] & 15u) == OP_S;
                const u32 i0 = clipF ? 1u : 0u;
                const u32 oa = clipF ? op[1] : op[0], on_ = clipF ? op[2] : op[1], ob = clipF ? op[3] : op[2];
                const u32 o3 = clipF ? op[4] : op[3], o4 = clipF ? op[5] : op[4], o5 = clipF ? op[6] : op[5];
                two = n >= i0 + 5u && (o3 & 15u) == OP_N;
                const u32 body = i0 + (two ? 5u : 3u);
                const u32 oL = two ? o5 : o3;
                const bool clipL = n == body + 1u && (oL & 15u) == OP_S;
                if (n == body || clipL) {
                    dS = clipF ? op[0] >> 4 : 0u;
                    const u32 dE = clipL ? oL >> 4 : 0u;
                    a = oa >> 4;
                    nl = on_ >> 4;
                    b2 = ob >> 4;
                    nl2 = two ? o3 >> 4 : 0u;
                    b3 = two ? o4 >> 4 : 0u;
                    simple = (oa & 15u) == OP_M && (on_ & 15u) == OP_N && (ob & 15u) == OP_M && a > 0 && b2 > 0 && a <= RES_FIELD_MAX && b2 <= RES_FIELD_MAX &&
                             dS <= RES_FIELD_MAX && lq > 1 && (u64)lq == (u64)dS + a + b2 + b3 + dE && seq_ok;
                    if (two)
                        simple = simple && (o4 & 15u) == OP_M && b3 > 0 && b3 <= RES_FIELD_MAX && nl > 0 && nl2 > 0 && pos >= 0 &&
                                 (int64_t)pos + a + nl + b2 + nl2 + b3 <= (int64_t)ref_len;
                }
            }
            two = two && simple;
            generic = !simple;
        }
        const u32 shard = (chunk >> (8 - K1E_SHIFT)) % GEN_SHARDS;
        const u32 base2 = ctx.list_reserve(2, two, 2u, shard), base3 = ctx.list_reserve(3, generic, 0u, shard);
        K1E_MARK(2);
        bool use2 = simple && gcodes2 != nullptr && !((O.excw >> (R.r & 31u)) & 1u) && pos >= 0 && (int64_t)pos + a + nl + b2 + nl2 + b3 <= (int64_t)ref_len &&
                    a <= (u32)C2_MAX_BLOCK && b2 <= (u32)C2_MAX_BLOCK && b3 <= (u32)C2_MAX_BLOCK;
        const int64_t n2w = codes2_words(ref_len);
        const bool any_exc = (G.exc_members >> mem) & 1u;
        Words2 x0 = {0, 0}, x1 = {0, 0}, x2 = {0, 0};
        if (use2 && any_exc) {
            const PJB_GLOBAL u32 *gexc = gcodes2 + n2w + K0_CODES2_PAD;
            const u32 g1 = (u32)pos + a + nl;
            x0 = gload_as<Words2>(gexc + ((u32)pos >> 11));
            x1 = gload_as<Words2>(gexc + (g1 >> 11));
            if (two) x2 = gload_as<Words2>(gexc + ((g1 + b2 + nl2) >> 11));
        }
        const bool more = v + 1 < v_hi, more2 = v + 2 < v_hi;
        EmitTrip T2 = T1;
        EmitRec R2 = R1;
        EmitOps On = O;
        if (more2) {
            T2 = locate(v + 2);
            R2 = fetch_rec(T2);
        }
        K1E_MARK(4);
        if (more) On = fetch_ops(T1, R1);
        K1E_MARK(6);
        const u32 *seqw = (const u32 *)b.seq4 + so;
        const int32_t q_limit = (int32_t)min(seq_words - 1u - so, 0x7fffffffu);
        if (simple) {
            const int32_t vpos = pos + voff;
            const int32_t aend_all = vpos + (int32_t)(a + nl + b2 + nl2 + b3) - 1;
            const u32 npairs = two ? 2u : 1u;
            int32_t ist_[2], lst_[2], rend_[2], iend_[2];
            u32 ud_[2];
            {
                int32_t lst = vpos;
                u32 la = a, ln_ = nl, lb = b2;
#pragma unroll
                for (u32 pr = 0; pr < 2; pr++) {
                    const int32_t istart = lst + (int32_t)la;
                    const int32_t rStartU = istart + (int32_t)ln_;
                    int32_t rStart = rStartU;
                    if (rStart - 1 >= vlen) rStart = vlen - 1;
                    const int32_t iend = rStart - 1;
                    int32_t rEndExc = rStartU + (int32_t)lb;
                    if (rEndExc - 1 >= vlen) rEndExc = vlen;
                    if (pr < npairs && rEndExc - 1 < iend) set_error(err, g, PJB_ERR_MIN_ANCHOR);
                    ist_[pr] = istart;
                    lst_[pr] = lst;
                    rend_[pr] = rEndExc - 1;
                    iend_[pr] = iend;
                    ud_[pr] = two ? (pr == 0 ? (1u << 16) : 1u) : (rStartU <= iend + 1 ? 0u : (1u << 16));
                    lst = rStart;
                    la = lb;
                    ln_ = nl2;
                    lb = b3;
                }
            }
            const int32_t bq[3] = {(int32_t)dS, (int32_t)(dS + a), (int32_t)(dS + a + b2)};
            const int32_t bg[3] = {lst_[0] - voff, iend_[0] + 1 - voff, iend_[1] + 1 - voff};
            const int32_t bl[3] = {(int32_t)a, rend_[0] - iend_[0], rend_[1] - iend_[1]};
            CmpBlock res[3] = {{bl[0], 0, -1, -1}, {bl[1], 0, -1, -1}, {bl[2], 0, -1, -1}};
            const int nb = two ? 3 : 2;
            {
                auto hit = [&](const Words2 &w, int32_t gi, int32_t l) {
                    const u32 b0 = (u32)gi >> 6, cnt = (((u32)(gi + l - 1)) >> 6) - b0 + 1u;
                    const u64 bits = (((u64)1 << cnt) - 1u) << (b0 & 31u);
                    return (((u64)w.x | ((u64)w.y << 32)) & bits) != 0;
                };
                if (any_exc && use2 && (hit(x0, bg[0], bl[0]) || hit(x1, bg[1], bl[1]) || (two && hit(x2, bg[2], bl[2])))) use2 = false;
            }
            if (__ballot(use2)) {
                const u32 *seq2w = (const u32 *)b.seq2 + (so >> 1);
                const int32_t q2_last = (int32_t)min(((seq_words + 1u) >> 1) - 1u - (so >> 1), 0x7fffffffu);
                const int32_t g2_last = (int32_t)(n2w + K0_CODES2_PAD - 1);
                const u32 qodd = (so & 1u) * 16u;
                int k = use2 ? 0 : nb;
                int32_t t = 0;
                u32 mism = 0, fbit = 0xffffffffu, lbit1 = 0;
                for (;;) {
                    const int32_t l = k == 0 ? bl[0] : k == 1 ? bl[1] : bl[2];
                    const bool act = k < nb && t < l;
                    if (act) {
                        const int32_t qi = k == 0 ? bq[0] : k == 1 ? bq[1] : bq[2], gi = k == 0 ? bg[0] : k == 1 ? bg[1] : bg[2];
                        const u32 qbit = qodd + 2u * (u32)(qi + t), gbit = 2u * (u32)(gi + t);
                        u32 qw[C2_NW], gw[C2_NW];
                        const int32_t qf = (int32_t)(qbit >> 5), gf = (int32_t)(gbit >> 5);
                        if (qf + C2_NW - 1 <= q2_last) {
                            const Words4 qa = gload(reinterpret_cast<const Words4 *>(seq2w + qf)), ga = gload_as<Words4>(gcodes2 + gf);
                            Words4 qb = {0, 0, 0, 0}, gb = {0, 0, 0, 0};
                            if (l - t > 48) {
                                qb = gload(reinterpret_cast<const Words4 *>(seq2w + qf + 4));
                                gb = gload_as<Words4>(gcodes2 + gf + 4);
                            }
                            qw[0] = qa.x, qw[1] = qa.y, qw[2] = qa.z, qw[3] = qa.w, qw[4] = qb.x, qw[5] = qb.y, qw[6] = qb.z, qw[7] = qb.w;
                            gw[0] = ga.x, gw[1] = ga.y, gw[2] = ga.z, gw[3] = ga.w, gw[4] = gb.x, gw[5] = gb.y, gw[6] = gb.z, gw[7] = gb.w;
                        } else {
                            load_words<C2_NW>(qw, seq2w, qf, q2_last);
                            load_words<C2_NW>(gw, (const u32 *)gcodes2, gf, g2_last);
                        }
                        chunk2_cmp_bits<C2_NW>(qw, gw, qbit & 31u, gbit & 31u, l, t, mism, fbit, lbit1);
                        t += C2_ROUND;
                    }
                    if (k < nb && t >= l) {
                        const int32_t first = (int32_t)fbit >> 1, last = ((int32_t)lbit1 - 1) >> 1;
                        if (k == 0) res[0].mism = (int32_t)mism, res[0].first = first, res[0].last = last;
                        if (k == 1) res[1].mism = (int32_t)mism, res[1].first = first, res[1].last = last;
                        if (k == 2) res[2].mism = (int32_t)mism, res[2].first = first, res[2].last = last;
                        k++;
                        t = 0, mism = 0, fbit = 0xffffffffu, lbit1 = 0;
                    }
                    if (!__ballot(k < nb)) break;
                }
            }
            if (__ballot(!use2)) {
                int k = use2 ? nb : 0;
                int32_t t = 0;
                u32 mism = 0, fbit = 0xffffffffu, lbit1 = 0;
                for (;;) {
                    const int32_t l = k == 0 ? bl[0] : k == 1 ? bl[1] : bl[2];
                    const bool act = k < nb && t < l;
                    if (act) {
                        const int32_t qi = k == 0 ? bq[0] : k == 1 ? bq[1] : bq[2], gi = k == 0 ? bg[0] : k == 1 ? bg[1] : bg[2];
                        CmpChunkT<SIMPLE_NW> C;
                        chunk_load<SIMPLE_NW, true>(C, seqw, qi, q_limit, (const u32 *)gcodes, gi, g_words, l, t);
                        chunk_cmp_bits<SIMPLE_NW>(C, qi, gi, l, t, mism, fbit, lbit1);
                        t += 8 * (SIMPLE_NW - 1);
                    }
                    if (k < nb && t >= l) {
                        const int32_t first = (int32_t)fbit >> 2, last = ((int32_t)lbit1 - 1) >> 2;
                        if (k == 0) res[0].mism = (int32_t)mism, res[0].first = first, res[0].last = last;
                        if (k == 1) res[1].mism = (int32_t)mism, res[1].first = first, res[1].last = last;
                        if (k == 2) res[2].mism = (int32_t)mism, res[2].first = first, res[2].last = last;
                        k++;
                        t = 0, mism = 0, fbit = 0xffffffffu, lbit1 = 0;
                    }
                    if (!__ballot(k < nb)) break;
                }
            }
#pragma unroll
            for (u32 pr = 0; pr < 2; pr++) {
                if (pr >= npairs) break;
                PairRec Q;
                Q.lstart = lst_[pr];
                Q.rend = rend_[pr];
                Q.pos = vpos;
                Q.aend = aend_all;
                Q.meta = meta | META_SIMPLE | (two ? META_MULTI : 0u);
                Q.updown = ud_[pr];
                Q.aux = cmp_blocks_res(res[pr], res[pr + 1]);
                const u64 key = make_key(kf, ist_[pr], iend_[pr]);
                P.key[off + pr] = key;
                if (want_g) P.g[off + pr] = g;
                rec_store(P.rec + off + pr, Q);
                if (want_cand) cand_insert(key, Q.lstart, Q.rend);
            }
        }
        const u64 p1_entry = (u64)(E.pack_nn ? g | (2u << 28) : g) | ((u64)off << 32);
        K1E_MARK(7);
        ctx.list_write(2, two, base2, p1_entry, shard);
        ctx.list_write(3, generic, base3, (u64)R.slot | ((u64)off << 32), shard);
        K1E_MARK(8);
        if (!more) ctx.cand_flush(true);
        K1E_MARK(9);
        T = T1;
        R = R1;
        O = On;
        T1 = T2;
        R1 = R2;
    }
}

__device__ __forceinline__ const DevBatch &find_batch_by_tile(const DevBatch *batches, int n_batches, u32 tile) {
    int lo = 0, hi = n_batches - 1;
    while (lo < hi) {
        const int mid = (lo + hi + 1) >> 1;
        if (batches[mid].tile_base <= tile) lo = mid;
        else hi = mid - 1;
    }
    return batches[lo];
}
__global__ __launch_bounds__(K1E_T) void k1_generic(const DevBatch *batches, int n_batches, const u32 *spl_idx, const uint4 *spl_rec, Pairs P, EmitLists E, KeyFmt kf,
                                                    GroupTab G, int use_codes, int orientation, u64 *err, ContigStats *cs) {
    __shared__ EmitShared sh;
    __shared__ u32 s_ops[OPS_LDS][K1E_T];
    __shared__ u32 s_first[GEN_SHARDS + 1];
    __shared__ u32 s_wsum[4];
    if (cs->P == 0) return;
    const bool want_cand = E.cand != nullptr;
    EmitCtx ctx{sh, E, kf, cs, want_cand};
    ctx.init();
    static_assert(GEN_SHARDS == K1E_T, "a sub-list per thread");
    {
        const u32 c = E.gen_cnt[threadIdx.x * GEN_CNT_STRIDE + 4];
        u32 total;
        const u32 ex = block_escan<K1E_T / 64>(c < E.gen_cap ? c : E.gen_cap, s_wsum, &total);
        s_first[threadIdx.x] = ex;
        if (threadIdx.x == K1E_T - 1) s_first[GEN_SHARDS] = total;
        __syncthreads();
    }
    const u32 n_items = s_first[GEN_SHARDS];
    for (u32 item0 = blockIdx.x * K1E_T; item0 < n_items; item0 += gridDim.x * K1E_T) {
        const u32 item = item0 + threadIdx.x;
        u32 gen_pairs = 0, gen_kind = 0;
        u64 gen_entry = 0;
        if (item < n_items) {
            u32 sub = 0;
#pragma unroll
            for (u32 step = GEN_SHARDS / 2; step > 0; step >>= 1)
                if (sub + step < GEN_SHARDS && s_first[sub + step] <= item) sub += step;
            const u64 e3 = E.gen_list[((size_t)2 * GEN_SHARDS + sub) * E.gen_cap + (item - s_first[sub])];
            const u32 slot = (u32)e3;
            const DevBatch &b = find_batch_by_tile(batches, n_batches, slot / (u32)K1_TILE);
            const u32 r = spl_idx[slot];
            const uint4 sr = spl_rec[slot];
            const int m = b.member;
            const int32_t voff = G.voff[m], ref_len = G.len[m], vlen = voff + ref_len;
            const u32 *gcodes = use_codes ? G.codes[m] : (const u32 *)nullptr;
            EmitRead R;
            R.n = sr.w & 0x7fffu;
            if (R.n == 0x7fffu) R.n = gload(b.cig_off + r + 1) - sr.x;
            R.lq = (int32_t)(sr.w >> 16);
            if (R.lq == 0xffff) R.lq = gload(b.l_qseq + r);
            const int32_t pos = (int32_t)sr.y;
            R.pos = pos + voff;
            R.g = b.base + r;
            R.meta = read_meta(gload(b.flag + r), (u32)gload(b.xs + r), gload(b.mapq + r), pos, gload(b.mtid + r), gload(b.mpos + r), G.tid[m], orientation);
            R.seq_ok = (sr.w & 0x8000u) != 0;
            R.off = (u32)(e3 >> 32);
            OpsViewT<K1E_T, OPS_LDS> cig;
            cig.g = b.cigar + sr.x;
            cig.lds = &s_ops[0][threadIdx.x];
#pragma unroll
            for (int q = 0; q < OPS_LDS; q++) {
                const bool has = (u32)q < R.n;
                const u32 v = gload(has ? cig.g + q : b.cig_off);
                s_ops[q][threadIdx.x] = has ? v : 0u;
            }
            u32 nN = 0, shape = 0;
            int32_t aligned = 0;
            int64_t qsum = 0, bsum = 0;
            for (u32 q = 0; q < R.n; q++) {
                const u32 o = cig[q], ty = o & 15u, ln = o >> 4;
                nN += (ty == OP_N);
                if (op_consumes_ref(ty)) aligned += (int32_t)ln;
                if (op_consumes_query(ty)) qsum += ln;
                const bool len_ok = ln > 0 && ln <= RES_FIELD_MAX;
                if (ty == OP_M || ty == OP_EQ || ty == OP_X) shape = (shape == 0 || shape == 5 || shape == 2 || shape == 1 || shape == 6) && len_ok ? 1u : 4u;
                else if (ty == OP_I || ty == OP_D) shape = shape == 1 && len_ok ? 6u : 4u;
                else if (ty == OP_N) shape = shape == 1 && ln > 0 ? 2u : 4u;
                else if (ty == OP_S) shape = shape == 0 && len_ok ? 5u : shape == 1 && q + 1 == R.n ? 3u : 4u;
                else shape = 4;
                bsum = ty == OP_N ? 0 : ty == OP_S ? bsum : bsum + ln;
                if (bsum > (int64_t)RES_FIELD_MAX) shape = 4;
            }
            if (nN > 1) R.meta |= META_MULTI;
            R.nN = nN;
            R.aend = R.pos + aligned - 1;
            const bool closed = gcodes != nullptr && (shape == 1 || shape == 3) && nN > 0 && R.seq_ok && R.lq > 1 && qsum == (int64_t)R.lq &&
                                R.pos >= voff && R.aend < vlen;
            R.closed_seqw = closed ? reinterpret_cast<const u32 *>(b.seq4) + sr.z : nullptr;
            R.q_limit = (int32_t)min(gload(b.seq_off + b.n) - 1u - sr.z, 0x7fffffffu);
            R.gcodes = gcodes;
            R.glen = ref_len;
            R.voff = voff;
            emit_read_pairs(cig, R, P, kf, vlen, err, [&](u64 key, int32_t lstart, int32_t rend) { ctx.cand_insert(key, lstart, rend); });
            gen_pairs = nN;
            gen_kind = closed ? 2u : 1u;
            gen_entry = (u64)(closed && E.pack_nn ? R.g | ((nN < 15u ? nN : 15u) << 28) : R.g) | ((u64)R.off << 32);
        }
        const u32 shard = (item0 >> K1E_SHIFT) % GEN_SHARDS;
        ctx.list_append(1, gen_kind == 1, gen_pairs, gen_entry, shard);
        ctx.list_append(2, gen_kind == 2, gen_pairs, gen_entry, shard);
        ctx.cand_flush(item0 + gridDim.x * K1E_T >= n_items);
    }
}

__global__ __launch_bounds__(256) void kg_member_stats(const u32 *tile_off, const TileStats *ts, const u32 *tile_lo, int n_members, MemberStats *out, u32 n_tiles,
                                                       const ContigStats *cs) {
    __shared__ u64 sm[4][4];
    __shared__ int32_t smi[4][2];
    const int m = blockIdx.x;
    if (m >= n_members) return;
    u64 spl = 0, uns = 0, sum = 0, pairs = 0;
    int32_t mn = INT32_MAX, mx = 0;
    for (u32 t = tile_lo[m] + threadIdx.x; t < tile_lo[m + 1]; t += 256) {
        const TileStats x = ts[t];
        spl += x.spliced;
        uns += x.unspliced;
        sum += x.sum_len;
        mn = min(mn, x.min_len);
        mx = max(mx, x.max_len);
    }
    spl = wave_sum(spl);
    uns = wave_sum(uns);
    sum = wave_sum(sum);
    {
        const u32 t0 = tile_lo[m], t1 = tile_lo[m + 1], total = (u32)cs->n_pairs;
        pairs = threadIdx.x == 0 ? (u64)((t1 < n_tiles ? tile_off[t1] : total) - (t0 < n_tiles ? tile_off[t0] : total)) : 0ull;
    }
    mn = wave_min(mn);
    mx = wave_max(mx);
    const int w = threadIdx.x >> 6;
    if (lane_id() == 0) {
        sm[w][0] = spl;
        sm[w][1] = uns;
        sm[w][2] = sum;
        sm[w][3] = pairs;
        smi[w][0] = mn;
        smi[w][1] = mx;
    }
    __syncthreads();
    if (threadIdx.x == 0) {
        MemberStats S;
        S.spliced = sm[0][0] + sm[1][0] + sm[2][0] + sm[3][0];
        S.unspliced = sm[0][1] + sm[1][1] + sm[2][1] + sm[3][1];
        S.sum_len = sm[0][2] + sm[1][2] + sm[2][2] + sm[3][2];
        S.n_pairs = sm[0][3] + sm[1][3] + sm[2][3] + sm[3][3];
        S.min_len = min(min(smi[0][0], smi[1][0]), min(smi[2][0], smi[3][0]));
        S.max_len = max(max(smi[0][1], smi[1][1]), max(smi[2][1], smi[3][1]));
        S.n_junc = 0;
        S._pad = 0;
        out[m] = S;
    }
}

constexpr int DENSE_ENDS = 8;
constexpr u32 DENSE_EMPTY = 0xffffffffu;

__device__ __forceinline__ u32 start_rank(const u64 *bitmap, const u32 *wrank, int32_t start) {
    const u32 w = (u32)start >> 6;
    return wrank[w] + (u32)__popcll(bitmap[w] & ((1ull << (start & 63)) - 1ull));
}
struct PopcFn {
    const u64 *words;
    __device__ u64 operator()(u64 i) const { return (u64)__popcll(words[i]); }
};
__global__ __launch_bounds__(256) void kd_ends(const u64 *cand, KeyFmt kf, const u64 *bitmap, const u32 *wrank, u32 junc_limit, u32 *ends,
                                               u32 *cand_rank, ContigStats *cs) {
    const u32 n = cs->n_cand;
    for (u32 p = blockIdx.x * 256 + threadIdx.x; p < n; p += gridDim.x * 256) {
        int32_t s, e;
        unpack_key(kf, cand[p], s, e);
        const u32 rs = start_rank(bitmap, wrank, s);
        cand_rank[p] = rs;
        if (rs >= junc_limit) {
            atomicOr(&cs->overflow, OVF_JUNC);
            continue;
        }
        u32 *slot = ends + (size_t)rs * DENSE_ENDS;
        const u32 ue = (u32)e;
        bool placed = false;
        for (int k = 0; k < DENSE_ENDS && !placed; k++) {
            const u32 cur = atomicCAS(&slot[k], DENSE_EMPTY, ue);
            placed = cur == DENSE_EMPTY || cur == ue;
        }
        if (!placed) atomicOr(&cs->overflow, OVF_DENSE);
    }
}
__global__ __launch_bounds__(256) void kd_rank_pages(const u64 *bitmap, const u32 *page_cnt, const u32 *page_rank, u32 *wrank, u32 n_pages, u32 n_words) {
    const u32 page = blockIdx.x * 4 + (threadIdx.x >> 6);
    if (page >= n_pages) return;
    if (page_cnt[page] == 0) return;
    const u32 w = (page << KD_PAGE_SHIFT) + (u32)lane_id();
    const u32 c = w < n_words ? (u32)__popcll(bitmap[w]) : 0u;
    const u32 inc = wave_iscan(c);
    if (w < n_words) wrank[w] = page_rank[page] + inc - c;
}
__global__ __launch_bounds__(256) void kd_reset(const u64 *cand, const u32 *cand_rank, KeyFmt kf, u32 junc_limit, const ContigStats *cs,
                                                u64 *bitmap, u32 *ends, u32 *page_cnt) {
    const u32 n = cs->n_cand;
    for (u32 p = blockIdx.x * 256 + threadIdx.x; p < n; p += gridDim.x * 256) {
        int32_t s, e;
        unpack_key(kf, cand[p], s, e);
        bitmap[(u32)s >> 6] = 0;
        page_cnt[(u32)s >> (6 + KD_PAGE_SHIFT)] = 0;
        const u32 rs = cand_rank[p];
        if (rs < junc_limit) {
            uint4 *q = reinterpret_cast<uint4 *>(ends + (size_t)rs * DENSE_ENDS);
            q[0] = q[1] = make_uint4(DENSE_EMPTY, DENSE_EMPTY, DENSE_EMPTY, DENSE_EMPTY);
        }
    }
}
struct EndsCountFn {
    const u32 *ends;
    __device__ u64 operator()(u64 rs) const {
        const uint4 *q = reinterpret_cast<const uint4 *>(ends + rs * DENSE_ENDS);
        const uint4 a = q[0], b = q[1];
        return (u64)((a.x != DENSE_EMPTY) + (a.y != DENSE_EMPTY) + (a.z != DENSE_EMPTY) + (a.w != DENSE_EMPTY) + (b.x != DENSE_EMPTY) +
                     (b.y != DENSE_EMPTY) + (b.z != DENSE_EMPTY) + (b.w != DENSE_EMPTY));
    }
};
struct FirstIdSink {
    u32 *first_id;
    int32_t *anc_l, *anc_r;
    __device__ void operator()(u64 i, u64, u64 ex) const {
        first_id[i] = (u32)ex;
        anc_l[i] = INT32_MAX;
        anc_r[i] = INT32_MIN;
    }
};
__device__ __forceinline__ u32 ends_below(const u32 *ends, u32 rs, u32 ue) {
    const uint4 *q = reinterpret_cast<const uint4 *>(ends + (size_t)rs * DENSE_ENDS);
    const uint4 a = q[0], b = q[1];
    return (a.x < ue) + (a.y < ue) + (a.z < ue) + (a.w < ue) + (b.x < ue) + (b.y < ue) + (b.z < ue) + (b.w < ue);
}
__device__ __forceinline__ void anchors_fold(bool valid, u32 j, int32_t l, int32_t r, int32_t *anc_l, int32_t *anc_r) {
    const u32 lk = (u32)l ^ 0x80000000u, rk = (u32)r ^ 0x80000000u;
    u64 todo = __ballot(valid);
    while (todo) {
        const int first = __ffsll((long long)todo) - 1;
        const u32 jc = (u32)__builtin_amdgcn_readlane((int)j, first);
        const bool mine = valid && j == jc;
        const u64 m = __ballot(mine);
        const int32_t lo = (int32_t)(wave_total<DppMin>(mine ? lk : 0xffffffffu) ^ 0x80000000u);
        const int32_t hi = (int32_t)(wave_total<DppMax>(mine ? rk : 0u) ^ 0x80000000u);
        if (lane_id() == first) {
            if (lo < __hip_atomic_load(&anc_l[jc], __ATOMIC_RELAXED, __HIP_MEMORY_SCOPE_AGENT)) atomicMin(&anc_l[jc], lo);
            if (hi > __hip_atomic_load(&anc_r[jc], __ATOMIC_RELAXED, __HIP_MEMORY_SCOPE_AGENT)) atomicMax(&anc_r[jc], hi);
        }
        todo &= ~m;
    }
// ... 554 lines not shown
            if (qPos < 0 || qPos + l > clen) {
                S.err = PJB_ERR_QUERY_RANGE;
                return S;
            }
        }
        if (cRef) rPos += ln;
        if (cQry) qPos += ln;
    }
    const int32_t q_start = position > start ? position : start;
    const int32_t q_end = rPos <= end ? rPos - 1 : end;
    if (q_start - start < 0 || end - q_end < 0) {
        S.err = PJB_ERR_QREGION;
        return S;
    }
    const int32_t gsize = end - start + 1;
    rPos = r0;
    qPos = q0;
    bool qDone = false, gDone = false, diverged = false;
    int32_t qTot = 0, gTot = 0, mism = 0, first_mis = -1, last_mis = -1;
    for (u32 k = k0; k < n; k++) {
        const u32 op = cig[k], ty = op & 15u;
        const int32_t ln = (int32_t)(op >> 4);
        const bool cRef = op_consumes_ref(ty);
        const bool cQry = op_consumes_query(ty) && ty != OP_S;
        int32_t qEmit = 0, gEmit = 0;
        int qKind = 0, gKind = 0;
        if (!qDone && rPos >= start) {
            if ((rPos > end && ty != OP_I) || (ty == OP_N && rPos + ln > end)) qDone = true;
            else if (cQry) {
                qEmit = (rPos + ln > end && ty != OP_I) ? end - rPos + 1 : ln;
                qKind = 1;
            } else if (cRef) {
                qEmit = rPos + ln > end ? end - rPos + 1 : ln;
                qKind = 2;
            }
        }
        if (!gDone && rPos >= q_start) {
            if (rPos > q_end && ty != OP_I) gDone = true;
            else if (cRef) {
                const int32_t so = rPos - start;
                gEmit = rPos + ln > q_end ? q_end - rPos + 1 : ln;
                if (so < 0 || so + gEmit > gsize) {
                    S.err = PJB_ERR_GENOME_RANGE;
                    return S;
                }
                gKind = 1;
            } else if (cQry) {
                gEmit = ln;
                gKind = 2;
            }
        }
        if (qEmit != gEmit) diverged = true;
        if (!diverged && qEmit > 0) {
            if (qKind == 1 && gKind == 1 && gcodes != nullptr && rPos >= 0 && rPos + qEmit <= glen) {
                cmp_words<GENERIC_NW, true>(reinterpret_cast<const u32 *>(seq), dS + qPos, q_limit, gcodes, rPos, (glen + 7) / 8 + 1, qEmit, qTot,
                                      mism, first_mis, last_mis);
            } else if (qKind == 1 && gKind == 1) {
                const int32_t qb = dS + qPos;
                for (int32_t t = 0; t < qEmit; t++) {
                    const int32_t qi = qb + t;
                    const u32 byte = gload(seq + (qi >> 1));
                    const u32 code = (qi & 1) ? (byte & 15u) : (byte >> 4);
                    const int32_t gi = rPos + t;
                    const u32 gc = (gi >= 0 && gi < glen) ? (u32)gload(genome + gi) : 0u;
                    if (nt16_ascii(code) != gc) {
                        mism++;
                        if (first_mis < 0) first_mis = qTot + t;
                        last_mis = qTot + t;
                    }
                }
            } else if (qKind == 1) {
                mism += qEmit;
                if (first_mis < 0) first_mis = qTot;
                last_mis = qTot + qEmit - 1;
            } else if (!genome_has_x) {
                mism += qEmit;
                if (first_mis < 0) first_mis = qTot;
                last_mis = qTot + qEmit - 1;
            } else {
                for (int32_t t = 0; t < qEmit; t++) {
                    const int32_t gi = rPos + t;
                    const u32 gc = (gi >= 0 && gi < glen) ? (u32)gload(genome + gi) : 0u;
                    if (gc != (u32)'X') {
                        mism++;
                        if (first_mis < 0) first_mis = qTot + t;
                        last_mis = qTot + t;
                    }
                }
            }
        }
        qTot += qEmit;
        gTot += gEmit;
        if (cRef) rPos += ln;
        if (cQry) qPos += ln;
        if (qDone && gDone) break;
    }
    if (qTot != gTot || qTot == 0) {
        S.err = PJB_ERR_ANCHOR_MISMATCH;
        return S;
    }
    if (diverged) {
        S.err = PJB_ERR_DIVERGENT;
        return S;
    }
    S.len = qTot;
    S.mism = mism;
    S.first_mis = first_mis;
    S.last_mis = last_mis;
    return S;
}

__device__ __forceinline__ u64 pair_stats_generic(const OpsView cig, u32 nc, int32_t pos, int32_t aligned, const uint8_t *seq,
                                                  int32_t lq, const uint8_t *genome, int32_t glen, bool has_x, const u32 *gcodes,
                                                  int32_t left, int32_t istart, int32_t iend, int32_t right, u32 g, u64 *err, u32 opi,
                                                  int32_t qN, int32_t q_limit) {
    if (lq <= 1) {
        const u32 totUp = (u32)((istart - 1) - left + 1);
        const u32 totDown = (u32)(right - (iend + 1) + 1);
        return pack_res(0, totUp < totDown ? totUp : totDown, 0);
    }
    u32 kL = opi, kR = 0;
    int32_t rL = istart, qL = qN, rR = pos, qR = 0;
    while (kL > 0) {
        const u32 op = cig[kL - 1], ty = op & 15u;
        const int32_t ln = (int32_t)(op >> 4);
        const int32_t rp = rL - (op_consumes_ref(ty) ? ln : 0);
        if (rp < left) break;
        kL--;
        rL = rp;
        if (op_consumes_query(ty) && ty != OP_S) qL -= ln;
    }
    const int32_t after = istart + (int32_t)(cig[opi] >> 4);
    if (after == iend + 1) {
        kR = opi + 1;
        rR = after;
        qR = qN;
    }
    const Side L = anchor_side(cig, nc, pos, aligned, seq, lq, genome, glen, has_x, gcodes, left, istart - 1, kL, rL, qL, q_limit);
    if (L.err) {
        set_error(err, g, L.err);
        return 0;
    }
    const Side R = anchor_side(cig, nc, pos, aligned, seq, lq, genome, glen, has_x, gcodes, iend + 1, right, kR, rR, qR, q_limit);
    if (R.err) {
        set_error(err, g, R.err);
        return 0;
    }
    const u32 upM = L.last_mis < 0 ? (u32)L.len : (u32)(L.len - 1 - L.last_mis);
    const u32 downM = R.first_mis < 0 ? (u32)R.len : (u32)R.first_mis;
    const u32 tu = (u32)(L.len - L.mism), td = (u32)(R.len - R.mism);
    return pack_res(upM < downM ? upM : downM, tu < td ? tu : td, (u32)(L.mism + R.mism));
}

__device__ __forceinline__ const DevBatch &find_batch(const DevBatch *batches, int n_batches, u32 g) {
    int lo = 0, hi = n_batches - 1;
    while (lo < hi) {
        const int mid = (lo + hi + 1) >> 1;
        if (batches[mid].base <= g) lo = mid;
        else hi = mid - 1;
    }
    return batches[lo];
}

__global__ __launch_bounds__(256) void k4b_generic(const u64 *list, const u32 *gen_cnt, u32 cap, const u64 *key, PairRec *rec, const u32 *jid_bam,
                                                    KeyFmt kf, const DevBatch *batches, int n_batches, const int32_t *anc_l, const int32_t *anc_r,
                                                    GroupTab G, int genome_has_x, int use_codes, u64 *err, const ContigStats *cs, u32 pack_nn) {
    __shared__ u32 s_ops[OPS_LDS][256];
    __shared__ u32 s_first[2 * GEN_SHARDS + 1];
    __shared__ u32 s_wsum[4];
    if (cs->P == 0) return;
    {
        const u32 i0 = threadIdx.x * 2;
        const u32 c0 = gen_cnt[(i0 % GEN_SHARDS) * GEN_CNT_STRIDE + (i0 / GEN_SHARDS) * 2];
        const u32 c1 = gen_cnt[((i0 + 1) % GEN_SHARDS) * GEN_CNT_STRIDE + ((i0 + 1) / GEN_SHARDS) * 2];
        const u32 n0 = c0 < cap ? c0 : cap, n1 = c1 < cap ? c1 : cap;
        u32 total;
        const u32 ex = block_escan<4>(n0 + n1, s_wsum, &total);
        s_first[i0] = ex;
        s_first[i0 + 1] = ex + n0;
        if (threadIdx.x == 255) s_first[2 * GEN_SHARDS] = total;
        __syncthreads();
    }
    static_assert(GEN_SHARDS == 256, "two sub-lists per thread of the block");
    const u32 n_items = s_first[2 * GEN_SHARDS];
    for (u32 item0 = blockIdx.x * 256; item0 < n_items; item0 += gridDim.x * 256) {
    const u32 item = item0 + threadIdx.x;
    if (item >= n_items) continue;
    u32 sub = 0;
#pragma unroll
    for (u32 step = GEN_SHARDS; step > 0; step >>= 1)
        if (sub + step < 2 * GEN_SHARDS && s_first[sub + step] <= item) sub += step;
    const bool check_only = sub >= GEN_SHARDS;
    const u64 entry = list[(size_t)sub * cap + (item - s_first[sub])];
    const u32 p0 = (u32)(entry >> 32);
    const u32 g = check_only && pack_nn ? (u32)entry & 0x0fffffffu : (u32)entry;
    if (check_only) {
        const u32 code = pack_nn ? (u32)entry >> 28 : 15u;
        const u32 nN = code < 15u ? code : (reinterpret_cast<const uint4 *>(rec + p0)[1].w >> 16) + 1u;
        bool ok = true;
        int32_t prev_istart = 0, is, ie;
        unpack_key(kf, key[p0], is, ie);
        for (u32 k = 0; k < nN; k++) {
            const u32 j = jid_bam[p0 + k];
            int32_t nis = 0, nie = 0;
            if (k + 1 < nN) unpack_key(kf, key[p0 + k + 1], nis, nie);
            if (k > 0 && prev_istart >= anc_l[j]) ok = false;
            if (k + 1 < nN && nie + 1 <= anc_r[j]) ok = false;
            prev_istart = is;
            is = nis;
            ie = nie;
        }
        if (ok) continue;
    }
    const DevBatch &b = find_batch(batches, n_batches, g);
    const u32 r = g - b.base;
    const u32 *cig_off = b.cig_off;
    const u32 c0 = gload(cig_off + r), c1 = gload(cig_off + r + 1);
    const u32 nc = c1 - c0;
    OpsView cig;
    cig.g = b.cigar + c0;
    cig.lds = &s_ops[0][threadIdx.x];
#pragma unroll
    for (int k = 0; k < OPS_LDS; k++) {
        const bool has = (u32)k < nc;
        const u32 v = gload(has ? cig.g + k : cig_off);
        s_ops[k][threadIdx.x] = has ? v : 0u;
    }
    const uint4 rb = reinterpret_cast<const uint4 *>(rec + p0)[1];
    const int32_t vpos = (int32_t)rb.x, aend = (int32_t)rb.y;
    const Member M = member_of(G, vpos);
    const int32_t pos = vpos - M.voff;
    const int32_t lq = gload(b.l_qseq + r);
    const u32 so0 = gload(b.seq_off + r), words = gload(b.seq_off + r + 1) - so0;
    if (lq > 1 && (u64)words * 8ull < (u64)lq) {
        set_error(err, g, PJB_ERR_NO_SEQ);
        continue;
    }
    const uint8_t *seq = b.seq4 + (size_t)so0 * 4;
    const int32_t q_limit = (int32_t)min(gload(b.seq_off + b.n) - 1u - so0, 0x7fffffffu);
    u32 k = 0;
    int32_t qsum = 0;
    for (u32 i = 0; i < nc; i++) {
        const u32 op = cig[i], ty = op & 15u;
        if (ty == OP_N) {
            const u32 p = p0 + k;
            const u32 j = jid_bam[p];
            int32_t istart, iend;
            unpack_key(kf, key[p], istart, iend);
            const u64 res = pair_stats_generic(cig, nc, pos, aend - vpos + 1, seq, lq, M.d, M.len, genome_has_x != 0, use_codes ? M.codes : (const u32 *)nullptr,
                                               anc_l[j] - M.voff, istart - M.voff, iend - M.voff, anc_r[j] - M.voff, g, err, i, qsum, q_limit);
            *reinterpret_cast<u64 *>(rec + p) = res;
            k++;
        }
        if (op_consumes_query(ty) && ty != OP_S) qsum += (int32_t)(op >> 4);
    }
    }
}

__global__ __launch_bounds__(256) void k4_pairs(const u32 *sidx, const u32 *jid_of, const PairRec *rec, const u64 *jkey, KeyFmt kf, const u32 *np,
                                                 u32 *frag, int32_t *frag_j, u64 *head_mask, u64 *run_mask, const ContigStats *cs_chk, u64 *err_chk) {
    const u32 n = *np;
    if (blockIdx.x * 256u >= n) return;
    const u32 i = blockIdx.x * 256 + threadIdx.x;
    const bool valid = i < n;
    const int lane = lane_id();
    const u32 ic = valid ? i : n - 1;
    const u32 p = sidx[ic];
    const u32 jv = jid_of[ic];
#ifdef PJB_SELFCHECK
    {
        const u32 Jc = cs_chk->J;
        const u32 jb = ic ? jid_of[ic - 1] : jv;
        int bad = 0;
        if (p >= n) bad = 1;
        else if (jv >= Jc) bad = 2;
        else if (jv != jb && jv != jb + 1) bad = 3;
        else if (ic == 0 && jv != 0) bad = 4;
        else if (ic == n - 1 && jv != Jc - 1) bad = 5;
        else if (jv + (ic >> 6) + 1 >= cs_chk->n_slots) bad = 6;
        else if ((ic >> 6) >= cs_chk->n_slices) bad = 7;
        else if (cs_chk->n_slots != Jc + (n + 63) / 64) bad = 8;
        if (__ballot(bad != 0)) {
            if (bad) set_error(err_chk, 0xffffe000u + (u32)bad, PJB_ERR_HIP);
            return;
        }
    }
#endif
    const PairRec Rc = rec_load(rec + p);
    const u64 jk = jkey[jv];
    u32 jprev_v = __shfl_up(jv, 1, 64);
    int32_t pos_prev = __shfl_up(Rc.pos, 1, 64), aend_prev = __shfl_up(Rc.aend, 1, 64);
    if (lane == 0 && valid && i > 0) {
        jprev_v = jid_of[i - 1];
        const uint4 q = reinterpret_cast<const uint4 *>(rec + sidx[i - 1])[1];
        pos_prev = (int32_t)q.x;
        aend_prev = (int32_t)q.y;
    }
    u32 j = 0xffffffffu;
    u32 cnt[4] = {0, 0, 0, 0}, jadp[5] = {0, 0, 0, 0, 0}, mx[5] = {0, 0, 0, 0, 0};
    u32 first_mis = 100000000u;
    u64 mism64 = 0;
    if (valid) {
        j = jv;
        int32_t istart, iend;
        unpack_key(kf, jk, istart, iend);
        const u64 rs = Rc.aux;
        const u32 minMatch = (u32)(rs & 0xfffffu), mmes = (u32)((rs >> 20) & 0xfffffu), nbMis = (u32)(rs >> 40);
        const u32 meta = Rc.meta;
        const u32 cat = meta & META_CAT_MASK;
        const u32 xs = (meta >> META_XS_SHIFT) & 3u;
        const bool dist_head = i == 0 || jprev_v != j || pos_prev != Rc.pos || aend_prev != Rc.aend;
        cnt[0] = 1u | ((u32)(cat == 0) << 8) | ((u32)(cat == 1) << 16) | ((u32)(cat == 2) << 24);
        cnt[1] = (u32)(cat == 3) | ((u32)((meta & META_MULTI) != 0) << 8) | ((u32)(xs == 1) << 16) | ((u32)(xs == 2) << 24);
        cnt[2] = (u32)((meta & META_UM) != 0) | ((u32)((meta & META_BPP) != 0) << 8) | ((u32)((meta & META_PPP) != 0) << 16) |
                 ((u32)((meta & META_REL) != 0) << 24);
        cnt[3] = (u32)dist_head;
#pragma unroll
        for (int w = 0; w < 5; w++)
            jadp[w] = (u32)((u32)(4 * w) < minMatch) | ((u32)((u32)(4 * w + 1) < minMatch) << 8) |
                      ((u32)((u32)(4 * w + 2) < minMatch) << 16) | ((u32)((u32)(4 * w + 3) < minMatch) << 24);
        const int32_t la = istart - Rc.lstart, ra = Rc.rend - iend;
        mx[0] = (u32)(la < ra ? la : ra);
        mx[1] = Rc.updown & 0xffffu;
        mx[2] = Rc.updown >> 16;
        mx[3] = mmes;
        mx[4] = minMatch;
        first_mis = minMatch > 0 ? minMatch : 100000000u;
        mism64 = nbMis;
        if (lane == 0 && i > 0 && jprev_v != j) frag_j[j + (i >> 6) - 1] = -1;
        if (i == n - 1) frag_j[j + (i >> 6) + 1] = -1;
    }
    if (head_mask) {
        const bool hj = valid && (i == 0 || jprev_v != j);
        const bool hr = valid && (hj || pos_prev != Rc.pos);
        const u64 mj = __ballot(hj), mr = __ballot(hr);
        if (lane == 0 && i < n) {
            head_mask[i >> 6] = mj;
            run_mask[i >> 6] = mr;
        }
    }
    auto store_fragment = [&](u32 hi_word) {
        const u32 slot = j + (i >> 6);
        u32 vals[F_WORDS];
#pragma unroll
        for (int k = 0; k < F_WORDS; k++) vals[k] = 0;
#pragma unroll
        for (int k = 0; k < 13; k++) vals[F_N + k] = (cnt[k >> 2] >> (8 * (k & 3))) & 0xffu;
        vals[F_MAXMINANC] = mx[0];
        vals[F_UP] = mx[1];
        vals[F_DOWN] = mx[2];
        vals[F_MAXMMES] = mx[3];
        vals[F_MAXMINMATCH] = mx[4];
        vals[F_FIRSTMIS] = first_mis;
        vals[F_MISM_LO] = (u32)mism64;
        vals[F_MISM_HI] = hi_word;
#pragma unroll
        for (int k = 0; k < 20; k++) vals[F_JAD0 + k] = (jadp[k >> 2] >> (8 * (k & 3))) & 0xffu;
        uint4 *dst = reinterpret_cast<uint4 *>(frag + (size_t)slot * F_WORDS);
#pragma unroll
        for (int k = 0; k < F_WORDS / 4; k++) dst[k] = make_uint4(vals[4 * k], vals[4 * k + 1], vals[4 * k + 2], vals[4 * k + 3]);
        frag_j[slot] = (int32_t)j;
    };
    const u32 j0 = (u32)__builtin_amdgcn_readfirstlane((int)j);
    if (__ballot(valid && j != j0) == 0) {
#pragma unroll
        for (int w = 0; w < 4; w++) cnt[w] = wave_total<DppAdd>(cnt[w]);
#pragma unroll
        for (int w = 0; w < 5; w++) jadp[w] = wave_total<DppAdd>(jadp[w]);
#pragma unroll
        for (int w = 0; w < 5; w++) mx[w] = wave_total<DppMax>(mx[w]);
        first_mis = wave_total<DppMin>(first_mis);
        mism64 = (u64)wave_total<DppAdd>((u32)mism64);
        if (valid && lane == 0) store_fragment(0u);
        return;
    }
    u32 take = 0;
#pragma unroll
    for (int sft = 0; sft < 6; sft++) {
        const int o = 1 << sft;
        const u32 kk = __shfl_down(j, o, 64);
        if (lane + o < 64 && kk == j) take |= 1u << sft;
    }
    auto red_add = [&](u32 v) {
#pragma unroll
        for (int sft = 0; sft < 6; sft++) {
            const u32 t = __shfl_down(v, 1 << sft, 64);
            if ((take >> sft) & 1u) v += t;
        }
        return v;
    };
    auto red_max = [&](u32 v) {
#pragma unroll
// ... 344 lines not shown
```

Baseline: 28.13 billion reads/s.

## Skip anchor check-only entries for reads whose junction windows cannot overlap

k1_count now records the maximum exon span per read (aligned length minus intron lengths), and k1_scan_tiles reduces it into ContigStats. k1_generic uses it to mark closed reads whose adjacent junctions cannot reach each other's anchor window, so they skip the k4b check-only list. k4b_generic now takes per-read metadata from the compact spl_idx/spl_rec records instead of re-reading cig_off, l_qseq and seq_off. It also caches per-batch tables in LDS and fetches CIGAR words with two 16-byte loads. The gain is fewer k4b items and fewer scattered global loads, at the cost of extra reductions in the count and scan kernels and a span bound that must be correct.

```diff
diff --git a/portcullis_amd/csrc/pjb_api.hip b/portcullis_amd/csrc/pjb_api.hip
--- a/portcullis_amd/csrc/pjb_api.hip
+++ b/portcullis_amd/csrc/pjb_api.hip
@@ -665,7 +665,7 @@
     if ((rc = ensure(c, S.ent, (size_t)PL * 8 + 16))) return rc;
     const u32 pair_blocks = std::max<u32>(1, (PL + 255) / 256);
     const u32 gen_cap = lim.list_cap ? lim.list_cap : (c->list_cap_forced ? c->list_cap_forced : gen_list_cap(PL));
-    const u32 pack_nn = (u64)f.n_reads < (1ull << 28) ? 1u : 0u;
+    const u32 pack_nn = (u64)n_tiles * K1_TILE < (1ull << 28) ? 1u : 0u;
     if ((rc = ensure(c, S.genlist, (size_t)gen_cap * GEN_SHARDS * 8 * 3))) return rc;
     if ((rc = ensure(c, S.gencount, GEN_SHARDS * GEN_CNT_STRIDE * 4))) return rc;
     const u32 slots_lim = JL + (PL + 63) / 64 + 1;
@@ -783,7 +783,7 @@
         }
         LAUNCH(c, "k1_scan_tiles", k1_scan_tiles, dim3(c->k1s_blocks_forced ? (u32)c->k1s_blocks_forced : k1s_blocks(n_tiles)), dim3(K1S_THREADS), (u32 *)S.tile_cnt.p, (const TileStats *)S.tile_stats.p,
                n_tiles, d_cs, PL, kf, group ? INT32_MAX - 1 : ref_len, (const u64 *)nullptr, (u32 *)S.tile_soff.p, (u32 *)S.chunk_tile.p,
-               (ScanPart *)S.scan_parts.p, ++S.scan_epoch);
+               (ScanPart *)S.scan_parts.p, ++S.scan_epoch, c->window_skip ? 1u : 0u);
         EmitLists el;
         el.cand = lim.dense ? (u64 *)S.key[1].p : (u64 *)nullptr;
         el.bitmap = lim.dense ? (u64 *)S.bitmap.p : (u64 *)nullptr;
@@ -824,7 +824,7 @@
     auto launch_k4b = [&]() -> int {
         LAUNCH(c, "k4b_generic", k4b_generic, dim3(gen_grid), dim3(256), (const u64 *)S.genlist.p, (const u32 *)d_gen_cnt, gen_cap, (const u64 *)pr.key,
                pr.rec, (const u32 *)S.jidbam.p, kf, (const DevBatch *)S.batches.p, (int)batches.size(), (const int32_t *)S.ancl.p, (const int32_t *)S.ancr.p,
-               GT, any_x ? 1 : 0, any_x ? 0 : 1, d_err, (const ContigStats *)d_cs, pack_nn);
+               GT, any_x ? 1 : 0, any_x ? 0 : 1, d_err, (const ContigStats *)d_cs, pack_nn, (const u32 *)S.splidx.p, (const uint4 *)S.splrec.p);
         return PJB_OK;
     };
     auto fork_k4b = [&]() -> int {
@@ -1652,6 +1652,7 @@
     else if (n == "dense_ids") c->dense_ids = value != 0;
     else if (n == "extra_dense") c->extra_dense_only = value != 0;
     else if (n == "sort_floor") c->sort_floor = (u32)std::max<int64_t>(1, std::min<int64_t>(value, 1 << 30));
+    else if (n == "window_skip") c->window_skip = value != 0;
     else if (n == "list_cap") c->list_cap_forced = (u32)std::max<int64_t>(0, std::min<int64_t>(value, 1 << 30));
     else return fail(c, PJB_ERR_ARG, "set_option: unknown option '%s'", name);
     return PJB_OK;
diff --git a/portcullis_amd/csrc/pjb_device.hip.h b/portcullis_amd/csrc/pjb_device.hip.h
--- a/portcullis_amd/csrc/pjb_device.hip.h
+++ b/portcullis_amd/csrc/pjb_device.hip.h
@@ -44,8 +44,9 @@
     int32_t max_end;
     int32_t max_nlen;
     int32_t min_pos;
-    int32_t _pad;
-};
+    u32 max_span;
+};
+static_assert(sizeof(TileStats) == 40, "TileStats layout");
 
 enum : u32 { OVF_PAIRS = 1u, OVF_KEYFMT = 2u, OVF_JUNC = 4u, OVF_DENSE = 8u, OVF_LISTS = 16u };
 struct ContigStats {
@@ -63,7 +64,13 @@
     u32 n_cand;
     u32 n_slices;
     u32 list_need;
-};
+    u32 max_span;
+};
+static_assert(sizeof(ContigStats) == 112, "ContigStats layout");
+__device__ __forceinline__ bool window_reach(u32 blk, u32 nl_prev, u32 nl_next, u32 B) {
+    const u32 l = __builtin_elementwise_add_sat(blk, nl_prev), r = __builtin_elementwise_add_sat(__builtin_elementwise_add_sat(blk, nl_next), 1u);
+    return l <= B || r <= B;
+}
 
 struct __attribute__((aligned(16))) PairRec {
     u64 aux;
diff --git a/portcullis_amd/csrc/pjb_host.hip.h b/portcullis_amd/csrc/pjb_host.hip.h
--- a/portcullis_amd/csrc/pjb_host.hip.h
+++ b/portcullis_amd/csrc/pjb_host.hip.h
@@ -247,6 +247,7 @@
     int radix_max_bits = 11;
     double junc_per_read = 0;
     u32 sort_floor = 1u << 16;
+    bool window_skip = true;
     u32 list_cap_forced = 0;
     bool k1_serial = true;
     hipEvent_t last_k1_ev = nullptr;
diff --git a/portcullis_amd/csrc/pjb_kernels.hip.h b/portcullis_amd/csrc/pjb_kernels.hip.h
--- a/portcullis_amd/csrc/pjb_kernels.hip.h
+++ b/portcullis_amd/csrc/pjb_kernels.hip.h
@@ -148,6 +148,9 @@
 __device__ __forceinline__ u32 spl_nlq(u32 n, bool seq_ok, int32_t lq) {
     return (n < 0x7fffu ? n : 0x7fffu) | (seq_ok ? 0x8000u : 0u) | ((u32)lq < 0xffffu ? (u32)lq << 16 : 0xffff0000u);
 }
+__device__ __forceinline__ u32 read_span(int32_t aligned, u32 nsum) {
+    return aligned < 0 || nsum > (u32)aligned ? 0xffffffffu : (u32)aligned - nsum;
+}
 #ifndef K1C_T
 #define K1C_T 256
 #endif
@@ -231,6 +234,7 @@
     u64 sum = 0;
     int32_t mn = INT32_MAX, mx = 0, max_end = 0, max_nlen = 0, min_pos = INT32_MAX;
     u32 cN[4], nlq[4];
+    u32 mspan = 0;
     u32 xspan = 0, xgapmax = 0;
     bool xmany = false;
 #pragma unroll
@@ -246,7 +250,7 @@
         const u32 n = c[i + 1] - c[i];
         nlq[i] = spl_nlq(n, (u64)(so[i + 1] - so[i]) * 8ull >= (u64)(int64_t)lenv, lenv);
         const u32 *ops = s_ops + (c[i] - cA + shift);
-        u32 cc = 0, ngap = 0, gmax = 0;
+        u32 cc = 0, ngap = 0, gmax = 0, nsum = 0;
         int32_t al = 0;
         auto count_op = [&](u32 op) {
             const u32 ty = op & 15u;
@@ -255,6 +259,7 @@
             if (ty == OP_N) {
                 cc++;
                 max_nlen = ln > max_nlen ? ln : max_nlen;
+                nsum = __builtin_elementwise_add_sat(nsum, (u32)ln);
             }
             if (EXTRA && ty == OP_D && ln) {
                 ngap++;
@@ -273,6 +278,7 @@
             const int32_t e = p + al;
             max_end = e > max_end ? e : max_end;
             min_pos = p < min_pos ? p : min_pos;
+            mspan = max(mspan, read_span(al, nsum));
         } else
             uns++;
         cN[i] = cc;
@@ -338,7 +344,9 @@
     max_end = smax(max_end);
     max_nlen = smax(max_nlen);
     min_pos = smin(min_pos);
+    mspan = wave_total<DppMax>(mspan);
     if (lane_id() == 0) {
+        r32[w][5] = (int32_t)mspan;
         r64[w][0] = ((u64)w_cnt << 32) | w_su;
         r64[w][1] = sum;
         r32[w][0] = mn;
@@ -352,8 +360,9 @@
         u64 pk = 0;
         TileStats ts;
         ts.sum_len = 0;
-        ts.min_len = INT32_MAX, ts.max_len = 0, ts.max_end = 0, ts.max_nlen = 0, ts.min_pos = INT32_MAX;
+        ts.min_len = INT32_MAX, ts.max_len = 0, ts.max_end = 0, ts.max_nlen = 0, ts.min_pos = INT32_MAX, ts.max_span = 0;
         for (int i = 0; i < NW; i++) {
+            ts.max_span = max(ts.max_span, (u32)r32[i][5]);
             pk += r64[i][0];
             ts.sum_len += r64[i][1];
             ts.min_len = min(ts.min_len, r32[i][0]);
@@ -365,7 +374,6 @@
         ts.spliced = (u32)((pk >> 16) & 0xffff);
         ts.unspliced = (u32)(pk & 0xffff);
         if (chk_ref_len > 0 && ts.max_end > chk_ref_len) ts.max_end = INT32_MAX;
-        ts._pad = 0;
         tile_stats[blockIdx.x] = ts;
         tile_cnt[blockIdx.x] = (u32)(pk >> 32);
     }
@@ -391,6 +399,7 @@
     u32 cnt = 0, spl = 0, uns = 0;
     u64 sum = 0;
     int32_t mn = INT32_MAX, mx = 0, max_end = 0, max_nlen = 0, min_pos = INT32_MAX;
+    u32 mspan = 0;
     constexpr int K1_OPS = 4;
     u32 c0[RPT], nop[RPT], ops[RPT][K1_OPS];
     int32_t pos4[RPT];
@@ -440,7 +449,7 @@
             const int32_t p = pos4[it];
             if (bad & (1u << it)) set_error(err, b.base + (u32)r, PJB_ERR_UNSORTED);
             if (bad & (16u << it)) set_error(err, b.base + (u32)r, PJB_ERR_BAD_XS);
-            u32 c = 0, ngap = 0, gmax = 0;
+            u32 c = 0, ngap = 0, gmax = 0, nsum = 0;
             int32_t al = 0;
             auto count_op = [&](u32 op) {
                 const u32 ty = op & 15u;
@@ -449,6 +458,7 @@
                 if (ty == OP_N) {
                     c++;
                     max_nlen = ln > max_nlen ? ln : max_nlen;
+                    nsum = __builtin_elementwise_add_sat(nsum, (u32)ln);
                 }
                 if (EXTRA && ty == OP_D && ln) {
                     ngap++;
@@ -464,6 +474,7 @@
                 int32_t e = p + al;
                 max_end = e > max_end ? e : max_end;
                 min_pos = p < min_pos ? p : min_pos;
+                mspan = max(mspan, read_span(al, nsum));
             } else
                 uns++;
             cthis = c;
@@ -533,6 +544,7 @@
     max_end = smax(max_end);
     max_nlen = smax(max_nlen);
     min_pos = smin(min_pos);
+    mspan = wave_total<DppMax>(mspan);
     int w = threadIdx.x >> 6;
     __shared__ u64 smp[NW];
     if (lane_id() == 0) {
@@ -543,14 +555,16 @@
         smi[w][2] = max_end;
         smi[w][3] = max_nlen;
         smi[w][4] = min_pos;
+        smi[w][5] = (int32_t)mspan;
     }
     __syncthreads();
     if (threadIdx.x == 0) {
         u64 p = 0;
         TileStats t;
         t.sum_len = 0;
-        t.min_len = INT32_MAX, t.max_len = 0, t.max_end = 0, t.max_nlen = 0, t.min_pos = INT32_MAX;
+        t.min_len = INT32_MAX, t.max_len = 0, t.max_end = 0, t.max_nlen = 0, t.min_pos = INT32_MAX, t.max_span = 0;
         for (int i = 0; i < NW; i++) {
+            t.max_span = max(t.max_span, (u32)smi[i][5]);
             p += smp[i];
             t.sum_len += sm64[i];
             t.min_len = min(t.min_len, smi[i][0]);
@@ -562,7 +576,6 @@
         t.spliced = (u32)((p >> 16) & 0xffff);
         t.unspliced = (u32)(p & 0xffff);
         if (chk_ref_len > 0 && t.max_end > chk_ref_len) t.max_end = INT32_MAX;
-        t._pad = 0;
         tile_stats[blockIdx.x] = t;
         tile_cnt[blockIdx.x] = (u32)(p >> 32);
     }
@@ -573,7 +586,7 @@
     u64 pairs, spl, uns, sum;
     int32_t mn, mx, max_end, max_nlen, min_pos;
     u32 flag;
-    u32 _pad[2];
+    u32 max_span, _pad;
 };
 static_assert(sizeof(ScanPart) == 64, "ScanPart layout");
 __host__ __device__ inline u32 k1s_blocks(u32 n_tiles) {
@@ -582,14 +595,14 @@
 }
 __global__ __launch_bounds__(K1S_THREADS) void k1_scan_tiles(u32 *tile_cnt, const TileStats *ts, u32 n_tiles, ContigStats *out, u32 pair_limit,
                                                               KeyFmt kf, int32_t ref_len, const u64 *tile_desc, u32 *tile_soff, u32 *chunk_tile,
-                                                              ScanPart *parts, u32 epoch) {
+                                                              ScanPart *parts, u32 epoch, u32 window_skip) {
     constexpr int NW = K1S_THREADS / 64;
     __shared__ u64 wsum[NW];
     __shared__ u32 wsum2[NW];
     __shared__ u32 carry2_s;
     __shared__ u64 carry_s;
     __shared__ u64 r_pairs[NW], r_spl[NW], r_uns[NW], r_sum[NW];
-    __shared__ int32_t r_i[NW][5];
+    __shared__ int32_t r_i[NW][6];
     __shared__ ScanPart total_s;
     const u32 nblk = gridDim.x, blk = blockIdx.x;
     const u32 per_blk = ((n_tiles + nblk - 1) / nblk + (u32)K1S_PER - 1) / (u32)K1S_PER * (u32)K1S_PER;
@@ -597,6 +610,7 @@
     const int w = threadIdx.x >> 6;
     u64 pairs = 0, spl = 0, uns = 0, sum = 0;
     int32_t mn = INT32_MAX, mx = 0, max_end = 0, max_nlen = 0, min_pos = INT32_MAX;
+    u32 max_span = 0;
     for (u32 base = lo; base < hi; base += K1S_THREADS * K1S_PER) {
         const u32 i0 = base + K1S_PER * threadIdx.x;
 #pragma unroll 4
@@ -614,6 +628,7 @@
                 max_end = max(max_end, t.max_end);
                 max_nlen = max(max_nlen, t.max_nlen);
                 min_pos = min(min_pos, t.min_pos);
+                max_span = max(max_span, t.max_span);
             }
         }
     }
@@ -626,7 +641,9 @@
     max_end = wave_max(max_end);
     max_nlen = wave_max(max_nlen);
     min_pos = wave_min(min_pos);
+    max_span = wave_max(max_span);
     if (lane_id() == 0) {
+        r_i[w][5] = (int32_t)max_span;
         r_pairs[w] = pairs;
         r_spl[w] = spl;
         r_uns[w] = uns;
@@ -640,8 +657,9 @@
     __syncthreads();
     ScanPart mine;
     mine.pairs = mine.spl = mine.uns = mine.sum = 0;
-    mine.mn = INT32_MAX, mine.mx = 0, mine.max_end = 0, mine.max_nlen = 0, mine.min_pos = INT32_MAX;
+    mine.mn = INT32_MAX, mine.mx = 0, mine.max_end = 0, mine.max_nlen = 0, mine.min_pos = INT32_MAX, mine.max_span = 0;
     for (int k = 0; k < NW; k++) {
+        mine.max_span = max(mine.max_span, (u32)r_i[k][5]);
         mine.pairs += r_pairs[k];
         mine.spl += r_spl[k];
         mine.uns += r_uns[k];
@@ -663,13 +681,14 @@
         o->max_end = mine.max_end;
         o->max_nlen = mine.max_nlen;
         o->min_pos = mine.min_pos;
+        o->max_span = mine.max_span;
         __hip_atomic_store(&o->flag, epoch, __ATOMIC_RELEASE, __HIP_MEMORY_SCOPE_AGENT);
     }
     if (w == 0) {
         const u32 l = lane_id();
         ScanPart b;
         b.pairs = b.spl = b.uns = b.sum = 0;
-        b.mn = INT32_MAX, b.mx = 0, b.max_end = 0, b.max_nlen = 0, b.min_pos = INT32_MAX;
+        b.mn = INT32_MAX, b.mx = 0, b.max_end = 0, b.max_nlen = 0, b.min_pos = INT32_MAX, b.max_span = 0;
         if (l < blk) {
             const ScanPart *o = parts + l;
             while (__hip_atomic_load(&o->flag, __ATOMIC_ACQUIRE, __HIP_MEMORY_SCOPE_AGENT) != epoch) __builtin_amdgcn_s_sleep(1);
@@ -683,6 +702,7 @@
                 b.max_end = __hip_atomic_load(&o->max_end, __ATOMIC_RELAXED, __HIP_MEMORY_SCOPE_AGENT);
                 b.max_nlen = __hip_atomic_load(&o->max_nlen, __ATOMIC_RELAXED, __HIP_MEMORY_SCOPE_AGENT);
                 b.min_pos = __hip_atomic_load(&o->min_pos, __ATOMIC_RELAXED, __HIP_MEMORY_SCOPE_AGENT);
+                b.max_span = __hip_atomic_load(&o->max_span, __ATOMIC_RELAXED, __HIP_MEMORY_SCOPE_AGENT);
             }
         }
         b.pairs = wave_sum(b.pairs);
@@ -695,6 +715,7 @@
             b.max_end = wave_max(b.max_end);
             b.max_nlen = wave_max(b.max_nlen);
             b.min_pos = wave_min(b.min_pos);
+            b.max_span = wave_max(b.max_span);
         }
         if (l == 0) {
             carry_s = b.pairs;
@@ -795,6 +816,7 @@
         out->n_junc = out->n_runs = 0;
         out->list_need = 0;
         out->n_cand = 0;
+        out->max_span = window_skip ? max(b.max_span, mine.max_span) : 0xffffffffu;
     }
 }
 
@@ -907,6 +929,58 @@
     __device__ __forceinline__ u32 operator[](u32 k) const { return k < (u32)NLDS ? lds[k * STRIDE] : gload(g + k); }
 };
 typedef OpsViewT<256, OPS_LDS> OpsView;
+__device__ __forceinline__ void fetch_ops8(const PJB_GLOBAL u32 *cigar, u32 c0, u32 cig_words, u32 (&w)[OPS_LDS]) {
+    static_assert(OPS_LDS == 8, "two 16-byte loads");
+    if (cig_words >= (u32)OPS_LDS) {
+        const u32 c0c = c0 + (u32)OPS_LDS <= cig_words ? c0 : cig_words - (u32)OPS_LDS;
+        const Words4 lo4 = gload_as<Words4>(cigar + c0c), hi4 = gload_as<Words4>(cigar + c0c + 4);
+        w[0] = lo4.x, w[1] = lo4.y, w[2] = lo4.z, w[3] = lo4.w, w[4] = hi4.x, w[5] = hi4.y, w[6] = hi4.z, w[7] = hi4.w;
+        if (c0c != c0) {
+            const u32 sh = c0 - c0c;
+#pragma unroll
+            for (int q = 0; q < OPS_LDS; q++) {
+                u32 v = 0;
+#pragma unroll
+                for (int j = q; j < OPS_LDS; j++) v = (u32)(j - q) == sh ? w[j] : v;
+                w[q] = v;
+            }
+        }
+    } else {
+#pragma unroll
+        for (int q = 0; q < OPS_LDS; q++) w[q] = c0 + (u32)q < cig_words ? cigar[c0 + (u32)q] : 0u;
+    }
+}
+constexpr int GEN_MAXB = 256;
+struct BatchTab {
+    u32 tbase[GEN_MAXB], seqw[GEN_MAXB], cigw[GEN_MAXB];
+    __device__ __forceinline__ void fill(const DevBatch *batches, int n_batches) {
+        if ((int)threadIdx.x < n_batches && threadIdx.x < (u32)GEN_MAXB) {
+            const PJB_GLOBAL DevBatch *d = as_global(batches + threadIdx.x);
+            tbase[threadIdx.x] = d->tile_base;
+            seqw[threadIdx.x] = as_global(d->seq_off)[d->n];
+            cigw[threadIdx.x] = as_global(d->cig_off)[d->n];
+        }
+    }
+    __device__ __forceinline__ int find(const DevBatch *batches, int n_batches, u32 tile) const {
+        int lo = 0, hi = n_batches - 1;
+        if (n_batches <= GEN_MAXB) {
+            while (lo < hi) {
+                const int mid = (lo + hi + 1) >> 1;
+                if (tbase[mid] <= tile) lo = mid;
+                else hi = mid - 1;
+            }
+        } else {
+            while (lo < hi) {
+                const int mid = (lo + hi + 1) >> 1;
+                if (gload(&batches[mid].tile_base) <= tile) lo = mid;
+                else hi = mid - 1;
+            }
+        }
+        return lo;
+    }
+    __device__ __forceinline__ u32 seq_words(const DevBatch &b, int bi) const { return bi < GEN_MAXB ? seqw[bi] : gload(b.seq_off + b.n); }
+    __device__ __forceinline__ u32 cig_words(const DevBatch &b, int bi) const { return bi < GEN_MAXB ? cigw[bi] : gload(b.cig_off + b.n); }
+};
 
 struct NCursor {
     u32 i;
@@ -1299,6 +1373,7 @@
     __shared__ u32 s_seqw[K1E_MAXB], s_cigw[K1E_MAXB], s_tbase[K1E_MAXB];
     __shared__ u32 s_wsum[4];
     if (cs->P == 0) return;
+    const u32 max_span = cs->max_span;
     K1E_T0();
     const bool want_g = P.g != nullptr;
     const bool want_cand = E.cand != nullptr;
@@ -1404,27 +1479,7 @@
             if (b.seq2 != nullptr) O.excw = b.seq_exc[r >> 5];
             O.lq = (int32_t)(R.sr.w >> 16);
             if (O.lq == 0xffff) O.lq = b.l_qseq[r];
-            static_assert(OPS_LDS == 8, "two 16-byte loads");
-            if (cig_words >= (u32)OPS_LDS) {
-                const u32 c0c = c0 + (u32)OPS_LDS <= cig_words ? c0 : cig_words - (u32)OPS_LDS;
-                const Words4 lo4 = gload_as<Words4>(b.cigar + c0c), hi4 = gload_as<Words4>(b.cigar + c0c + 4);
-                u32 w[OPS_LDS] = {lo4.x, lo4.y, lo4.z, lo4.w, hi4.x, hi4.y, hi4.z, hi4.w};
-                if (c0c != c0) {
-                    const u32 sh = c0 - c0c;
-#pragma unroll
-                    for (int q = 0; q < OPS_LDS; q++) {
-                        u32 v = 0;
-#pragma unroll
-                        for (int j = q; j < OPS_LDS; j++) v = (u32)(j - q) == sh ? w[j] : v;
-                        w[q] = v;
-                    }
-                }
-#pragma unroll
-                for (int q = 0; q < OPS_LDS; q++) O.op[q] = w[q];
-            } else {
-#pragma unroll
-                for (int q = 0; q < OPS_LDS; q++) O.op[q] = c0 + (u32)q < cig_words ? b.cigar[c0 + (u32)q] : 0u;
-            }
+            fetch_ops8(b.cigar, c0, cig_words, O.op);
         }
         return O;
     };
@@ -1452,7 +1507,7 @@
         const bool on = R.on;
         const u32 so = R.sr.z;
         const int32_t pos = (int32_t)R.sr.y, lq = O.lq;
-        bool generic = false, simple = false, two = false;
+        bool generic = false, simple = false, two = false, chk2 = false;
         u32 dS = 0, a = 0, nl = 0, b2 = 0, nl2 = 0, b3 = 0, meta = 0, off = 0, g = 0;
         if (on) {
             const u32 n = O.n;
@@ -1486,10 +1541,11 @@
                 }
             }
             two = two && simple;
+            chk2 = two && window_reach(b2, nl, nl2, max_span);
             generic = !simple;
         }
         const u32 shard = (chunk >> (8 - K1E_SHIFT)) % GEN_SHARDS;
-        const u32 base2 = ctx.list_reserve(2, two, 2u, shard), base3 = ctx.list_reserve(3, generic, 0u, shard);
+        const u32 base2 = ctx.list_reserve(2, chk2, 2u, shard), base3 = ctx.list_reserve(3, generic, 0u, shard);
         K1E_MARK(2);
         bool use2 = simple && gcodes2 != nullptr && !((O.excw >> (R.r & 31u)) & 1u) && pos >= 0 && (int64_t)pos + a + nl + b2 + nl2 + b3 <= (int64_t)ref_len &&
                     a <= (u32)C2_MAX_BLOCK && b2 <= (u32)C2_MAX_BLOCK && b3 <= (u32)C2_MAX_BLOCK;
@@ -1645,9 +1701,9 @@
                 if (want_cand) cand_insert(key, Q.lstart, Q.rend);
             }
         }
-        const u64 p1_entry = (u64)(E.pack_nn ? g | (2u << 28) : g) | ((u64)off << 32);
+        const u64 p1_entry = (u64)(E.pack_nn ? R.slot | (2u << 28) : R.slot) | ((u64)off << 32);
         K1E_MARK(7);
-        ctx.list_write(2, two, base2, p1_entry, shard);
+        ctx.list_write(2, chk2, base2, p1_entry, shard);
         ctx.list_write(3, generic, base3, (u64)R.slot | ((u64)off << 32), shard);
         K1E_MARK(8);
         if (!more) ctx.cand_flush(true);
@@ -1660,28 +1716,22 @@
     }
 }
 
-__device__ __forceinline__ const DevBatch &find_batch_by_tile(const DevBatch *batches, int n_batches, u32 tile) {
-    int lo = 0, hi = n_batches - 1;
-    while (lo < hi) {
-        const int mid = (lo + hi + 1) >> 1;
-        if (batches[mid].tile_base <= tile) lo = mid;
-        else hi = mid - 1;
-    }
-    return batches[lo];
-}
 __global__ __launch_bounds__(K1E_T) void k1_generic(const DevBatch *batches, int n_batches, const u32 *spl_idx, const uint4 *spl_rec, Pairs P, EmitLists E, KeyFmt kf,
                                                     GroupTab G, int use_codes, int orientation, u64 *err, ContigStats *cs) {
     __shared__ EmitShared sh;
     __shared__ u32 s_ops[OPS_LDS][K1E_T];
     __shared__ u32 s_first[GEN_SHARDS + 1];
     __shared__ u32 s_wsum[4];
+    __shared__ BatchTab s_bt;
     if (cs->P == 0) return;
+    const u32 max_span = cs->max_span;
     const bool want_cand = E.cand != nullptr;
     EmitCtx ctx{sh, E, kf, cs, want_cand};
     ctx.init();
     static_assert(GEN_SHARDS == K1E_T, "a sub-list per thread");
     {
         const u32 c = E.gen_cnt[threadIdx.x * GEN_CNT_STRIDE + 4];
+        s_bt.fill(batches, n_batches);
         u32 total;
         const u32 ex = block_escan<K1E_T / 64>(c < E.gen_cap ? c : E.gen_cap, s_wsum, &total);
         s_first[threadIdx.x] = ex;
@@ -1700,7 +1750,8 @@
                 if (sub + step < GEN_SHARDS && s_first[sub + step] <= item) sub += step;
             const u64 e3 = E.gen_list[((size_t)2 * GEN_SHARDS + sub) * E.gen_cap + (item - s_first[sub])];
             const u32 slot = (u32)e3;
-            const DevBatch &b = find_batch_by_tile(batches, n_batches, slot / (u32)K1_TILE);
+            const int bi = s_bt.find(batches, n_batches, slot / (u32)K1_TILE);
+            const DevBatch &b = batches[bi];
             const u32 r = spl_idx[slot];
             const uint4 sr = spl_rec[slot];
             const int m = b.member;
@@ -1720,17 +1771,25 @@
             OpsViewT<K1E_T, OPS_LDS> cig;
             cig.g = b.cigar + sr.x;
             cig.lds = &s_ops[0][threadIdx.x];
-#pragma unroll
-            for (int q = 0; q < OPS_LDS; q++) {
-                const bool has = (u32)q < R.n;
-                const u32 v = gload(has ? cig.g + q : b.cig_off);
-                s_ops[q][threadIdx.x] = has ? v : 0u;
+            {
+                u32 w[OPS_LDS];
+                fetch_ops8(as_global(b.cigar), sr.x, s_bt.cig_words(b, bi), w);
+#pragma unroll
+                for (int q = 0; q < OPS_LDS; q++) s_ops[q][threadIdx.x] = (u32)q < R.n ? w[q] : 0u;
             }
             u32 nN = 0, shape = 0;
             int32_t aligned = 0;
             int64_t qsum = 0, bsum = 0;
+            u32 bref = 0, nl_prev = 0;
+            bool reach = max_span == 0xffffffffu;
             for (u32 q = 0; q < R.n; q++) {
                 const u32 o = cig[q], ty = o & 15u, ln = o >> 4;
+                if (ty == OP_N) {
+                    if (nN > 0) reach = reach || window_reach(bref, nl_prev, ln, max_span);
+                    nl_prev = ln;
+                    bref = 0;
+                } else if (op_consumes_ref(ty))
+                    bref = __builtin_elementwise_add_sat(bref, ln);
                 nN += (ty == OP_N);
                 if (op_consumes_ref(ty)) aligned += (int32_t)ln;
                 if (op_consumes_query(ty)) qsum += ln;
@@ -1749,14 +1808,14 @@
             const bool closed = gcodes != nullptr && (shape == 1 || shape == 3) && nN > 0 && R.seq_ok && R.lq > 1 && qsum == (int64_t)R.lq &&
                                 R.pos >= voff && R.aend < vlen;
             R.closed_seqw = closed ? reinterpret_cast<const u32 *>(b.seq4) + sr.z : nullptr;
-            R.q_limit = (int32_t)min(gload(b.seq_off + b.n) - 1u - sr.z, 0x7fffffffu);
+            R.q_limit = (int32_t)min(s_bt.seq_words(b, bi) - 1u - sr.z, 0x7fffffffu);
             R.gcodes = gcodes;
             R.glen = ref_len;
             R.voff = voff;
             emit_read_pairs(cig, R, P, kf, vlen, err, [&](u64 key, int32_t lstart, int32_t rend) { ctx.cand_insert(key, lstart, rend); });
             gen_pairs = nN;
-            gen_kind = closed ? 2u : 1u;
-            gen_entry = (u64)(closed && E.pack_nn ? R.g | ((nN < 15u ? nN : 15u) << 28) : R.g) | ((u64)R.off << 32);
+            gen_kind = !closed ? 1u : reach ? 2u : 0u;
+            gen_entry = (u64)(closed && E.pack_nn ? slot | ((nN < 15u ? nN : 15u) << 28) : slot) | ((u64)R.off << 32);
         }
         const u32 shard = (item0 >> K1E_SHIFT) % GEN_SHARDS;
         ctx.list_append(1, gen_kind == 1, gen_pairs, gen_entry, shard);
@@ -2617,28 +2676,21 @@
     return pack_res(upM < downM ? upM : downM, tu < td ? tu : td, (u32)(L.mism + R.mism));
 }
 
-__device__ __forceinline__ const DevBatch &find_batch(const DevBatch *batches, int n_batches, u32 g) {
-    int lo = 0, hi = n_batches - 1;
-    while (lo < hi) {
-        const int mid = (lo + hi + 1) >> 1;
-        if (batches[mid].base <= g) lo = mid;
-        else hi = mid - 1;
-    }
-    return batches[lo];
-}
-
 __global__ __launch_bounds__(256) void k4b_generic(const u64 *list, const u32 *gen_cnt, u32 cap, const u64 *key, PairRec *rec, const u32 *jid_bam,
                                                     KeyFmt kf, const DevBatch *batches, int n_batches, const int32_t *anc_l, const int32_t *anc_r,
-                                                    GroupTab G, int genome_has_x, int use_codes, u64 *err, const ContigStats *cs, u32 pack_nn) {
+                                                    GroupTab G, int genome_has_x, int use_codes, u64 *err, const ContigStats *cs, u32 pack_nn,
+                                                    const u32 *spl_idx, const uint4 *spl_rec) {
     __shared__ u32 s_ops[OPS_LDS][256];
     __shared__ u32 s_first[2 * GEN_SHARDS + 1];
     __shared__ u32 s_wsum[4];
+    __shared__ BatchTab s_bt;
     if (cs->P == 0) return;
     {
         const u32 i0 = threadIdx.x * 2;
         const u32 c0 = gen_cnt[(i0 % GEN_SHARDS) * GEN_CNT_STRIDE + (i0 / GEN_SHARDS) * 2];
         const u32 c1 = gen_cnt[((i0 + 1) % GEN_SHARDS) * GEN_CNT_STRIDE + ((i0 + 1) / GEN_SHARDS) * 2];
         const u32 n0 = c0 < cap ? c0 : cap, n1 = c1 < cap ? c1 : cap;
+        s_bt.fill(batches, n_batches);
         u32 total;
         const u32 ex = block_escan<4>(n0 + n1, s_wsum, &total);
         s_first[i0] = ex;
@@ -2658,7 +2710,7 @@
     const bool check_only = sub >= GEN_SHARDS;
     const u64 entry = list[(size_t)sub * cap + (item - s_first[sub])];
     const u32 p0 = (u32)(entry >> 32);
-    const u32 g = check_only && pack_nn ? (u32)entry & 0x0fffffffu : (u32)entry;
+    const u32 slot = check_only && pack_nn ? (u32)entry & 0x0fffffffu : (u32)entry;
     if (check_only) {
         const u32 code = pack_nn ? (u32)entry >> 28 : 15u;
         const u32 nN = code < 15u ? code : (reinterpret_cast<const uint4 *>(rec + p0)[1].w >> 16) + 1u;
@@ -2677,32 +2729,36 @@
         }
         if (ok) continue;
     }
-    const DevBatch &b = find_batch(batches, n_batches, g);
-    const u32 r = g - b.base;
-    const u32 *cig_off = b.cig_off;
-    const u32 c0 = gload(cig_off + r), c1 = gload(cig_off + r + 1);
-    const u32 nc = c1 - c0;
+    const int bi = s_bt.find(batches, n_batches, slot / (u32)K1_TILE);
+    const DevBatch &b = batches[bi];
+    const u32 r = spl_idx[slot];
+    const uint4 sr = spl_rec[slot];
+    const u32 g = gload(&b.base) + r;
+    const u32 c0 = sr.x;
+    u32 nc = sr.w & 0x7fffu;
+    if (nc == 0x7fffu) nc = gload(b.cig_off + r + 1) - c0;
     OpsView cig;
     cig.g = b.cigar + c0;
     cig.lds = &s_ops[0][threadIdx.x];
-#pragma unroll
-    for (int k = 0; k < OPS_LDS; k++) {
-        const bool has = (u32)k < nc;
-        const u32 v = gload(has ? cig.g + k : cig_off);
-        s_ops[k][threadIdx.x] = has ? v : 0u;
+    {
+        u32 w[OPS_LDS];
+        fetch_ops8(as_global(b.cigar), c0, s_bt.cig_words(b, bi), w);
+#pragma unroll
+        for (int k = 0; k < OPS_LDS; k++) s_ops[k][threadIdx.x] = (u32)k < nc ? w[k] : 0u;
     }
     const uint4 rb = reinterpret_cast<const uint4 *>(rec + p0)[1];
     const int32_t vpos = (int32_t)rb.x, aend = (int32_t)rb.y;
     const Member M = member_of(G, vpos);
     const int32_t pos = vpos - M.voff;
-    const int32_t lq = gload(b.l_qseq + r);
-    const u32 so0 = gload(b.seq_off + r), words = gload(b.seq_off + r + 1) - so0;
-    if (lq > 1 && (u64)words * 8ull < (u64)lq) {
+    int32_t lq = (int32_t)(sr.w >> 16);
+    if (lq == 0xffff) lq = gload(b.l_qseq + r);
+    const u32 so0 = sr.z;
+    if (lq > 1 && !(sr.w & 0x8000u)) {
         set_error(err, g, PJB_ERR_NO_SEQ);
         continue;
     }
     const uint8_t *seq = b.seq4 + (size_t)so0 * 4;
-    const int32_t q_limit = (int32_t)min(gload(b.seq_off + b.n) - 1u - so0, 0x7fffffffu);
+    const int32_t q_limit = (int32_t)min(s_bt.seq_words(b, bi) - 1u - so0, 0x7fffffffu);
     u32 k = 0;
     int32_t qsum = 0;
     for (u32 i = 0; i < nc; i++) {
```

Result: faster. 29.14 billion reads/s, median of 6 (+3.6%).
